# AarambhDevHub/query-engine

Hardware: AMD Instinct MI355X
Metric: rows/sec filter->hash-join->group-by, 1B rows, 1/2/4/8 GPUs; % HBM roofline (higher is better)
Workload: dtype int64/f64

## Files before the change

### query-engine_amd/csrc/k_aggregate.hip

```cpp
#include <algorithm>
#include <cstdlib>
#include <cstring>
#include <string>
#include <memory>
#include <type_traits>

#include "agg.h"
#include "expr_device.h"
#include "fast_tile.h"
#include "ops.h"

namespace qeh {

constexpr int kAggR = 4;
constexpr int kAggTile = kBlock * kAggR;
constexpr size_t kLdsStateBudget = 48 * 1024;
constexpr int kFastTile = kBlock * kFastR;

enum GidMode { GM_ZERO = 0, GM_JOIN = 1, GM_GROUP = 2, GM_LDSHASH = 3 };
enum PredMode { PM_NONE = 0, PM_TERMS = 1, PM_PROG = 2 };

constexpr int64_t kEmptyKey = INT64_MIN;
struct GTable {
    int64_t *keys;
// ... 267 lines not shown
    if (tid < kBpP) pc[tid] = 0, fillp[tid] = kBpChunk, curc[tid] = 0;
    __syncthreads();
    const int64_t n_tiles = (n + kBpTile - 1) / kBpTile;
    const int64_t woff = (int64_t)wave * (64 * kFastR) + 2 * lane;
    FastTile<NTERMS, NACOL, NT> nx;
    if ((int64_t)blockIdx.x < n_tiles && ((int64_t)blockIdx.x + 1) * kBpTile <= n) nx.issue(in, (int64_t)blockIdx.x * kBpTile + woff);
    for (int64_t tile = blockIdx.x; tile < n_tiles; tile += gridDim.x) {
        const int64_t base = tile * kBpTile + woff;
        FastTile<NTERMS, NACOL, NT> ft;
        if ((tile + 1) * kBpTile <= n) {
            ft = nx;
            ft.eval(in, terms);
            const int64_t t2 = tile + gridDim.x;
            if (t2 < n_tiles && (t2 + 1) * kBpTile <= n) nx.issue(in, t2 * kBpTile + woff);
        } else {
            ft.issue_tail(in, base, n);
            ft.eval(in, terms);
            ft.sel &= FastTile<NTERMS, NACOL, NT>::tail_mask(base, n);
        }
        uint32_t part[kFastR], rk[kFastR];
#pragma unroll
        for (int r = 0; r < kFastR; ++r) {
            part[r] = (uint32_t)(hash64((uint64_t)ft.k(r)) >> (64 - kBpPBits));
            rk[r] = ((ft.sel >> r) & 1u) ? atomicAdd(&pc[part[r]], 1u) : 0u;
        }
        bp_barrier();
        if (tid < kBpP) {
            const uint32_t c = pc[tid];
            const uint32_t incl = wave_incl_scan(c);
            tstart[tid] = incl - c;
            if (tid == kBpP - 1) tot_s = incl;
            const uint32_t room = kBpChunk - fillp[tid];
            const uint32_t spill = c > room ? c - room : 0u;
            const uint32_t nnew = (spill + kBpChunk - 1) / kBpChunk;
            uint32_t b = 0;
            if (nnew) {
                b = atomicAdd(nchunk, nnew);
                for (uint32_t i = 0; i < nnew; ++i) tag[b + i] = (uint16_t)tid, ccnt[b + i] = (uint16_t)kBpChunk;
            }
            cbase[tid] = b;
        }
        bp_barrier();
#pragma unroll
        for (int r = 0; r < kFastR; ++r) {
            if (!((ft.sel >> r) & 1u)) continue;
            const uint32_t p = part[r], f = fillp[p], room = kBpChunk - f;
            uint32_t dst;
            if (rk[r] < room) {
                dst = curc[p] * kBpChunk + f + rk[r];
            } else {
                const uint32_t q = rk[r] - room;
                dst = (cbase[p] + q / kBpChunk) * kBpChunk + q % kBpChunk;
            }
            const uint32_t st = tstart[p] + rk[r];
            skey[st] = (uint64_t)ft.k(r);
            if (NACOL > 0) sval[st] = (uint64_t)ft.a(acs, r);
            sdst[st] = dst;
        }
        bp_barrier();
        const uint32_t tot = tot_s;
        for (uint32_t i = tid; i < tot; i += kBpBlock) {
            const uint32_t d = sdst[i];
            okey[d] = skey[i];
            if (NACOL > 0) oval[d] = sval[i];
        }
        if (tid < kBpP) {
            const uint32_t c = pc[tid], f = fillp[tid], room = kBpChunk - f;
            if (c <= room) {
                fillp[tid] = f + c;
            } else {
                const uint32_t q = c - room;
                curc[tid] = cbase[tid] + (q - 1) / kBpChunk;
                fillp[tid] = (q - 1) % kBpChunk + 1;
            }
            pc[tid] = 0;
        }
        bp_barrier();
    }
    if (tid < kBpP && fillp[tid] < kBpChunk) ccnt[curc[tid]] = (uint16_t)fillp[tid];
}

template <int NACOL>
__global__ __launch_bounds__(kBpBlock) void k_bp_probe(AggSpecs specs, FastIn in, HashTable t, int64_t G,
                                                       const uint32_t *__restrict__ sbase, const uint32_t *__restrict__ list,
                                                       const uint64_t *__restrict__ ikey, const uint64_t *__restrict__ ival,
                                                       uint64_t *__restrict__ gstates_all) {
    uint64_t *__restrict__ gstates = shard_states(gstates_all, specs, G);
    extern __shared__ __attribute__((aligned(16))) uint64_t lds[];
    {
        const int64_t words = (int64_t)specs.n_slots * G;
        for (int64_t i = threadIdx.x; i < words; i += blockDim.x) lds[i] = 0;
        __syncthreads();
        for (int a = 0; a < specs.n; ++a) {
            const AggSpec sp = specs.a[a];
            if (sp.kind == AK_MIN || sp.kind == AK_MAX)
                for (int64_t g = threadIdx.x; g < G; g += blockDim.x) lds[(int64_t)sp.val_slot * G + g] = (uint64_t)agg_init_value(sp.kind);
        }
        __syncthreads();
    }
    const int lane = threadIdx.x & 63, wave = threadIdx.x >> 6;
    const int x = blockIdx.x & 7;
    const uint32_t wi = blockIdx.x >> 3, nwg = gridDim.x >> 3;
    constexpr int U = 2;
    for (int p = x; p < kBpP; p += 8) {
        const uint32_t lo = sbase[p], hi = sbase[p + 1];
        const uint32_t stride = nwg * kBpWaves * U;
        uint32_t ent[U];
#pragma unroll
        for (int u = 0; u < U; ++u) {
            const uint32_t e = lo + (wi * kBpWaves + wave) * U + u;
            ent[u] = e < hi ? list[e] : 0xFFFFFFFFu;
        }
        for (uint32_t e0 = lo + (wi * kBpWaves + wave) * U; e0 < hi; e0 += stride) {
            int64_t key[U][4], val[U][4];
            uint32_t cn[U];
#pragma unroll
            for (int u = 0; u < U; ++u) {
                cn[u] = ent[u] == 0xFFFFFFFFu ? 0u : (ent[u] >> 24) + 1u;
                const uint64_t at = (uint64_t)(ent[u] & 0xFFFFFFu) * kBpChunk + lane * 4;
                if (cn[u]) {
                    const v2i64 k0 = __builtin_nontemporal_load((const v2i64 *)(ikey + at));
                    const v2i64 k1 = __builtin_nontemporal_load((const v2i64 *)(ikey + at + 2));
                    key[u][0] = k0[0], key[u][1] = k0[1], key[u][2] = k1[0], key[u][3] = k1[1];
                    if (NACOL > 0) {
                        const v2i64 v0 = __builtin_nontemporal_load((const v2i64 *)(ival + at));
                        const v2i64 v1 = __builtin_nontemporal_load((const v2i64 *)(ival + at + 2));
                        val[u][0] = v0[0], val[u][1] = v0[1], val[u][2] = v1[0], val[u][3] = v1[1];
                    }
                }
            }
#pragma unroll
            for (int u = 0; u < U; ++u) {
                const uint32_t e = e0 + stride + u;
                ent[u] = e < hi ? list[e] : 0xFFFFFFFFu;
            }
            uint32_t gid[U][4];
            uint32_t hit = 0;
#pragma unroll
            for (int u = 0; u < U; ++u)
#pragma unroll
                for (int q = 0; q < 4; ++q) {
                    gid[u][q] = 0;
                    if ((uint32_t)(lane * 4 + q) < cn[u] && probe_unique(t, key[u][q], gid[u][q])) hit |= 1u << (u * 4 + q);
                }
#pragma unroll
            for (int u = 0; u < U; ++u)
#pragma unroll
                for (int q = 0; q < 4; ++q)
                    if ((hit >> (u * 4 + q)) & 1u) atomicAdd((unsigned long long *)&lds[gid[u][q]], 1ull);
            for (int a = 0; a < specs.n; ++a) {
                const AggSpec sp = specs.a[a];
                if (sp.kind == AK_COUNT || in.agg_colslot[a] < 0) continue;
                uint64_t *st = lds + (int64_t)sp.val_slot * G;
#pragma unroll
                for (int u = 0; u < U; ++u)
#pragma unroll
                    for (int q = 0; q < 4; ++q)
                        if ((hit >> (u * 4 + q)) & 1u) {
                            const int64_t v = NACOL > 0 ? val[u][q] : 0;
                            if (sp.kind == AK_SUM_F) atomicAdd((double *)&st[gid[u][q]], as_f64(v));
                            else if (sp.kind == AK_SUM_I) atomicAdd((unsigned long long *)&st[gid[u][q]], (unsigned long long)v);
                            else agg_apply<true>(sp.kind, &st[gid[u][q]], agg_input(sp.kind, sp.in_type, v));
                        }
            }
        }
    }
    __syncthreads();
    for (int64_t g = threadIdx.x; g < G; g += blockDim.x) {
        uint64_t rows = lds[g];
        if (!rows) continue;
        atomicAdd((unsigned long long *)&gstates[g], (unsigned long long)rows);
        for (int a = 0; a < specs.n; ++a) {
            const AggSpec sp = specs.a[a];
            if (sp.kind != AK_COUNT)
                agg_merge_global(sp.kind, &gstates[(int64_t)sp.val_slot * G + g], lds[(int64_t)sp.val_slot * G + g]);
        }
    }
}

constexpr int kSliceBits = 16;
constexpr int kSliceKeys = 1 << kSliceBits;
constexpr int kSliceMaxF = 160;
constexpr int kSliceBlock = 1024;
constexpr int kSliceTile = kSliceBlock * kFastR;
constexpr int kSliceChunk = 32;
constexpr int kMaxSliceGrid = 512;
constexpr int kSliceStateWords = 3584;
constexpr int kGidSliceBits = 12;
constexpr int kGidStateWords = 16384;

__device__ __forceinline__ void lds_barrier() { asm volatile("s_waitcnt lgkmcnt(0)\n\ts_barrier" ::: "memory"); }

struct SliceRegions {
    uint16_t *key;
    int64_t *val;
    int64_t *val2;
    uint32_t *count;
    uint32_t *overflow;
    uint64_t cap;
    int32_t F;
    const uint64_t *rbase;
    int32_t pw;
    int32_t prank;
    int32_t pgrid;
    const uint16_t *okey;
    const int64_t *oval;
    uint64_t ocap;
};
__host__ __device__ __forceinline__ int part_slices(int F, int pw) { return (F + pw - 1) / pw; }
__host__ __device__ __forceinline__ uint64_t part_region(int b, int w, int F, int pw, int grid) {
    return ((uint64_t)(b % pw) * part_slices(F, pw) + (uint64_t)(b / pw)) * grid + w;
}


struct SlicePlan {
    int64_t kmin;
    uint64_t range;
    uint64_t cap;
    int32_t F;
    int32_t ok;
    int64_t src[6];
};
struct SlicePlanIn {
    uint64_t min_bytes;
    uint64_t alloc_items;
    int32_t grid;
    int32_t n_slots;
    int32_t sparse_ok;
    int32_t chunk;
    int32_t world;
};
__host__ __device__ inline SlicePlan plan_slices(const SlicePlanIn &pi, int64_t kmn, int64_t kmx, int64_t kcnt, int64_t gmn,
                                                 int64_t gmx, int64_t gcnt) {
    SlicePlan p{};
    p.src[0] = kmn, p.src[1] = kmx, p.src[2] = kcnt, p.src[3] = gmn, p.src[4] = gmx, p.src[5] = gcnt;
    if (kcnt <= 0) return p;
    const uint64_t gr = gcnt ? (uint64_t)gmx - (uint64_t)gmn + 1ull : 0;
    const int64_t g_bound = (gr == 0 || gr > (1ull << 20)) ? -1 : (int64_t)gr + 1;
    if (g_bound <= 0 || g_bound >= 0xFFFF || (int64_t)pi.n_slots * g_bound > kSliceStateWords) return p;
    const uint64_t range = (uint64_t)kmx - (uint64_t)kmn + 1ull;
    if (!direct_table_ok_with(range, (uint64_t)kcnt, (uint64_t)g_bound, pi.sparse_ok != 0)) return p;
    if (range * 2 < pi.min_bytes) return p;
    const uint64_t F = (range + kSliceKeys - 1) >> kSliceBits;
    if (F == 0 || F > (uint64_t)kSliceMaxF) return p;
    p.kmin = kmn;
    p.range = range;
    p.F = (int32_t)F;
    const uint64_t ch = pi.chunk > 0 ? (uint64_t)pi.chunk : (uint64_t)kSliceChunk;
    const uint64_t Fr = pi.world > 1 ? (F + pi.world - 1) / pi.world * pi.world : F;
    p.cap = pi.alloc_items / ((uint64_t)pi.grid * Fr) / ch * ch;
    p.ok = p.cap >= ch;
    return p;
}
__global__ void k_slice_plan(const MinMax *__restrict__ mm, SlicePlanIn pi, SlicePlan *out) {
    if (threadIdx.x == 0 && blockIdx.x == 0)
        *out = plan_slices(pi, mm[0].mn, mm[0].mx, (int64_t)mm[0].cnt, mm[1].mn, mm[1].mx, (int64_t)mm[1].cnt);
}
__global__ void k_slice_plan_stats(const int64_t *__restrict__ M, int world, int row_len, SlicePlanIn pi, SlicePlan *out) {
    if (threadIdx.x != 0 || blockIdx.x != 0) return;
    int64_t tot = 0, kmn = INT64_MAX, kmx = INT64_MIN, gmn = INT64_MAX, gmx = INT64_MIN, bitmap = 0;
    for (int r = 0; r < world; ++r) {
        const int64_t *m = M + (int64_t)r * row_len;
        bitmap |= m[5];
        if (m[0] <= 0) continue;
        tot += m[0];
        kmn = m[1] < kmn ? m[1] : kmn, kmx = m[2] > kmx ? m[2] : kmx;
        gmn = m[3] < gmn ? m[3] : gmn, gmx = m[4] > gmx ? m[4] : gmx;
    }
    SlicePlan p = plan_slices(pi, kmn, kmx, tot, gmn, gmx, tot);
    if (bitmap || kmn > kmx || gmn > gmx) p.ok = 0;
    *out = p;
}

struct FusedPlan {
    SlicePlan sp;
    int64_t gmin;
    int64_t ngroups;
    uint64_t dcap;
};
struct FusedPro {
    const int64_t *dk;
    ColRef dg;
    int64_t nd;
    uint32_t *ditems;
    uint32_t *dcount;
    uint32_t *status;
    void *gkeys;
    uint32_t *rep;
    int64_t G;
    int32_t as32;
    const FusedPlan *plan;
};
struct DimSlices {
    const uint32_t *items;
    const uint32_t *count;
    uint32_t *dup;
    const FusedPlan *plan;
    int32_t nreg;
    int32_t _pad;
    uint64_t rstride;
    const uint32_t *offs;
};

struct __attribute__((aligned(16))) SliceChunk {
    uint64_t g;
    int32_t soff;
    uint32_t pk;
};

#ifndef QEH_EARLY_PAIRS
#define QEH_EARLY_PAIRS 2
#endif
#ifndef QEH_SLICE_FLUSH_LATE
#define QEH_SLICE_FLUSH_LATE 1
#endif
#ifndef QEH_EARLY_CHUNK
#define QEH_EARLY_CHUNK 64
#endif
template <int NACOL, bool EARLY = false, int NTH = kSliceBlock>
struct SliceShape {
    static constexpr int P = NACOL > 1 ? 2 : (EARLY ? QEH_EARLY_PAIRS : kFastPairs);
    static constexpr int CH = NACOL > 1 ? 16 : (EARLY ? QEH_EARLY_CHUNK : kSliceChunk);
    static constexpr int TILE = NTH * 2 * P;
};

template <int NTH>
__device__ __attribute__((noinline)) void fused_prologue(const FusedPro &fp, int F, int64_t kmin, uint32_t *dcnt) {
    const int tid = threadIdx.x;
    const FusedPlan fpl = *fp.plan;
    for (int i = tid; i < F; i += NTH) dcnt[i] = 0;
    for (int64_t i = (int64_t)blockIdx.x * NTH + tid; i < fp.G; i += (int64_t)gridDim.x * NTH) {
        if (fp.as32) ((int32_t *)fp.gkeys)[i] = (int32_t)(fpl.gmin + i);
        else ((int64_t *)fp.gkeys)[i] = fpl.gmin + i;
        fp.rep[i] = (uint32_t)i;
    }
    __syncthreads();
    const int64_t chunk = (fp.nd + gridDim.x - 1) / gridDim.x;
    const int64_t lo = (int64_t)blockIdx.x * chunk, hi = lo + chunk < fp.nd ? lo + chunk : fp.nd;
    uint32_t *dreg = fp.ditems + (uint64_t)blockIdx.x * F * fpl.dcap;
    bool dovf = false;
    constexpr int DR = 8;
    for (int64_t i0 = lo + tid; i0 < hi; i0 += DR * NTH) {
        int64_t kk[DR], gg[DR];
#pragma unroll
        for (int q = 0; q < DR; ++q) {
            const int64_t i = i0 + (int64_t)q * NTH;
            kk[q] = i < hi ? fp.dk[i] : kmin;
            gg[q] = i < hi ? load_i64(fp.dg, i) : 0;
        }
#pragma unroll
        for (int q = 0; q < DR; ++q) {
            if (i0 + (int64_t)q * NTH >= hi) continue;
            const uint64_t o = (uint64_t)kk[q] - (uint64_t)kmin;
            const uint32_t b = (uint32_t)(o >> kSliceBits);
            const uint32_t r = atomicAdd(&dcnt[b], 1u);
            if (r < fpl.dcap)
                dreg[(uint64_t)b * fpl.dcap + r] =
                    ((uint32_t)(o & (kSliceKeys - 1)) << 16) | ((uint32_t)((uint64_t)gg[q] - (uint64_t)fpl.gmin) + 1u);
            else
                dovf = true;
        }
    }
    __syncthreads();
    if (fp.dcount)
        for (int i = tid; i < F; i += NTH) {
            fp.dcount[(uint64_t)blockIdx.x * F + i] = dcnt[i] < fpl.dcap ? dcnt[i] : (uint32_t)fpl.dcap;
            dovf |= dcnt[i] > fpl.dcap;
        }
    if (dovf) fp.status[1] = 1u;
}

#ifndef QEH_PA_STAMPS
#define QEH_PA_STAMPS 0
#endif
#if QEH_PA_STAMPS
constexpr int kPaStampWords = 16;
__device__ uint64_t qeh_pa_stamps[kMaxSliceGrid * 16 * kPaStampWords];
#define PA_STAMP(i)                                          \
    do {                                                     \
        const uint64_t t_ = __builtin_amdgcn_s_memtime();    \
        pa_acc[i] += t_ - pa_prev;                           \
        pa_prev = t_;                                        \
    } while (0)
#else
#define PA_STAMP(i) \
    do {            \
    } while (0)
#endif

template <int NTERMS, int NACOL, bool NT, int MODE = 0, bool EARLY = false, int NTH = kSliceBlock>
__global__ __launch_bounds__(NTH) void k_slice_partition(FastIn in, PredTerms terms, int64_t kmin, uint64_t range,
                                                                 int64_t n_tiles, SliceRegions rg, HashTable t,
                                                                 const SlicePlan *__restrict__ dplan = nullptr,
                                                                 int64_t tail_rows = 0, FusedPro fp = FusedPro{}) {
    using Shape = SliceShape<NACOL, EARLY, NTH>;
    constexpr int P = Shape::P, R = 2 * P, TILE = Shape::TILE, CH = Shape::CH;
    constexpr int MAXF = kSliceMaxF;
    if (dplan) {
        const SlicePlan pl = *dplan;
        if (!pl.ok) return;
        kmin = pl.kmin, range = pl.range;
        rg.F = pl.F, rg.cap = pl.cap;
    }
    constexpr int SB = MODE ? kGidSliceBits : kSliceBits;
    constexpr int VC = NACOL;
    constexpr int VS = VC > 0 ? VC : 1;
    __shared__ uint32_t cntb[2][MAXF], cnb[2][MAXF], posb[2][MAXF], lofsb[2][MAXF], mpre[MAXF], hd[MAXF];
    __shared__ uint64_t abase[MAXF];
    __shared__ uint32_t s_chunks;
    __shared__ SliceChunk cdesc[TILE / CH + MAXF];
    __shared__ uint16_t st_key[TILE];
    __shared__ int64_t st_v[VS][VC ? TILE : 1];
    __shared__ uint16_t c_key[MAXF * CH];
    __shared__ int64_t c_v[VS][VC ? MAXF * CH : 1];
    __shared__ uint8_t st_b[EARLY ? TILE : 1];
    int64_t *const vout[2] = {rg.val, rg.val2};
    const int F = rg.F;
    const uint64_t cap = rg.cap;
    const int tid = threadIdx.x, lane = tid & 63, wave = tid >> 6;
    const uint64_t region0 = (uint64_t)blockIdx.x * F;
    for (int i = tid; i < MAXF; i += NTH) {
        cntb[0][i] = 0, cntb[1][i] = 0, posb[0][i] = 0, hd[i] = 0, abase[i] = 0;
        if (i < F) {
            const uint64_t st = rg.rbase ? rg.rbase[(uint64_t)i * gridDim.x + blockIdx.x]
                                : rg.pw ? part_region(i, blockIdx.x, F, rg.pw, gridDim.x) * cap
                                        : (region0 + i) * cap;
            hd[i] = (uint32_t)(st % CH);
            abase[i] = st - hd[i];
        }
        cnb[0][i] = hd[i];
    }
    __syncthreads();
    bool ovf = false;
    auto flush = [&](uint32_t M) {
        const uint32_t xl = (tid & (CH / 2 - 1)) * 2;
        for (uint32_t c = tid / (CH / 2); c < M; c += NTH / (CH / 2)) {
            const SliceChunk d = cdesc[c];
            const uint32_t coff = (d.pk & 255u) * CH, clim = (d.pk >> 8) & 127u, lo = (d.pk >> 15) & 127u,
                           hi = (d.pk >> 22) & 127u;
            uint16_t kv[2];
            int64_t vv[VS][2] = {};
#pragma unroll
            for (int q = 0; q < 2; ++q) {
                const uint32_t x = xl + q;
                if (x < clim) {
                    kv[q] = c_key[coff + x];
#pragma unroll
                    for (int u = 0; u < VC; ++u) vv[u][q] = c_v[u][coff + x];
                } else {
                    kv[q] = st_key[d.soff + (int32_t)x];
#pragma unroll
                    for (int u = 0; u < VC; ++u) vv[u][q] = st_v[u][d.soff + (int32_t)x];
                }
            }
            const uint64_t o = d.g + xl;
            if (lo == 0 && hi == (uint32_t)CH) {
                const uint32_t kw = (uint32_t)kv[0] | ((uint32_t)kv[1] << 16);
                if constexpr (EARLY) __builtin_nontemporal_store(kw, (uint32_t *)(rg.key + o));
                else *(uint32_t *)(rg.key + o) = kw;
#pragma unroll
                for (int u = 0; u < VC; ++u) {
                    v2i64 w;
                    w[0] = vv[u][0], w[1] = vv[u][1];
                    __builtin_nontemporal_store(w, (v2i64 *)(vout[u] + o));
                }
            } else {
#pragma unroll
                for (int q = 0; q < 2; ++q) {
                    if (xl + q < lo || xl + q >= hi) continue;
                    rg.key[o + q] = kv[q];
#pragma unroll
                    for (int u = 0; u < VC; ++u) __builtin_nontemporal_store(vv[u][q], vout[u] + o + q);
                }
            }
        }
    };
    auto carry = [&](const uint32_t *cn_o, const uint32_t *cnt_o, const uint32_t *lofs_o, int p0, int stride) {
        if constexpr (EARLY) {
            const uint32_t total = lofs_o[F - 1] + cnt_o[F - 1];
            for (uint32_t si = (uint32_t)p0; si < total; si += (uint32_t)stride) {
                const int b = st_b[si];
                const uint32_t cb = cn_o[b], nb = cnt_o[b], T = cb + nb, L = T % CH, j = si - lofs_o[b];
                int dst = -1;
                if (T < CH) dst = (int)(cb + j);
                else if (j >= nb - L) dst = (int)(j - (nb - L));
                if (dst >= 0) {
                    c_key[b * CH + dst] = st_key[si];
#pragma unroll
                    for (int u = 0; u < VC; ++u) c_v[u][b * CH + dst] = st_v[u][si];
                }
            }
            return;
        }
        for (int p = p0; p < F * CH; p += stride) {
            const int b = p / CH, kx = p % CH;
            const uint32_t cb = cn_o[b], nb = cnt_o[b], T = cb + nb, L = T % CH;
            int src = -1;
            if (T < CH) {
                if (kx >= (int)cb && kx < (int)T) src = (int)(lofs_o[b] + kx - cb);
            } else if (kx < (int)L) {
                src = (int)(lofs_o[b] + nb - L + kx);
            }
            if (src >= 0) {
                c_key[b * CH + kx] = st_key[src];
#pragma unroll
                for (int u = 0; u < VC; ++u) c_v[u][b * CH + kx] = st_v[u][src];
            }
        }
    };
    FastTile<NTERMS, NACOL, NT, P> ft;
    int64_t tile = blockIdx.x;
    int par = 0;
    uint32_t m_prev = 0;
    bool have_prev = false;
    const int64_t n_all = n_tiles + (EARLY && tail_rows > 0 ? 1 : 0), lim = n_tiles * TILE + tail_rows;
    auto issue_tile = [&](int64_t tl) {
        const int64_t b = tl * TILE + (int64_t)wave * (64 * R) + 2 * lane;
        if (!EARLY || tl < n_tiles) ft.issue(in, b);
        else ft.issue_tail(in, b, lim);
    };
    if constexpr (EARLY) {
        __shared__ uint32_t dcnt[MAXF];
        fused_prologue<NTH>(fp, F, kmin, dcnt);
    }
    if (tile < n_all) issue_tile(tile);
#if QEH_PA_STAMPS
    uint64_t pa_acc[10] = {};
    const uint64_t pa_t0 = __builtin_amdgcn_s_memtime(), pa_r0 = __builtin_amdgcn_s_memrealtime();
    uint64_t pa_prev = pa_t0;
#endif
    for (; tile < n_all; tile += gridDim.x) {
        uint32_t *cnt = cntb[par], *cn = cnb[par], *pos = posb[par], *lofs = lofsb[par];
        const int pq = par ^ 1;
        if (!QEH_SLICE_FLUSH_LATE && have_prev) flush(m_prev);
#if QEH_PA_STAMPS
        PA_STAMP(9);
        asm volatile("s_waitcnt vmcnt(0)" ::: "memory");
        PA_STAMP(0);
#endif
        ft.eval(in, terms);
        uint32_t sel = ft.sel, off[R], rk[R];
        if (EARLY && tile >= n_tiles) sel &= decltype(ft)::tail_mask(tile * TILE + (int64_t)wave * (64 * R) + 2 * lane, lim);
        if constexpr (MODE == 1) {
#pragma unroll
            for (int r = 0; r < R; ++r) {
                off[r] = 0;
                if (((sel >> r) & 1) && !probe_unique(t, ft.k(r), off[r])) sel &= ~(1u << r);
            }
#pragma unroll
            for (int r = 0; r < R; ++r) {
                rk[r] = 0;
                if ((sel >> r) & 1) rk[r] = atomicAdd(&cnt[off[r] >> SB], 1u);
            }
        } else {
#pragma unroll
            for (int r = 0; r < R; ++r) {
                const uint64_t o = (uint64_t)ft.k(r) - (uint64_t)kmin;
                off[r] = (uint32_t)o;
                rk[r] = 0;
                if (((sel >> r) & 1) && o < range) rk[r] = atomicAdd(&cnt[(uint32_t)o >> kSliceBits], 1u);
                else sel &= ~(1u << r);
            }
        }
        int64_t vcur[VS][R];
#pragma unroll
        for (int u = 0; u < VS; ++u)
#pragma unroll
            for (int r = 0; r < R; ++r) vcur[u][r] = VC ? ft.a(u, r) : 0;
        PA_STAMP(1);
        if (EARLY && tile + gridDim.x < n_all) issue_tile(tile + gridDim.x);
        if (QEH_SLICE_FLUSH_LATE && have_prev) flush(m_prev);
        PA_STAMP(2);
        lds_barrier();
        PA_STAMP(3);
        if (wave == 0) {
            uint32_t n3[3], m3[3], ns = 0, ms = 0;
#pragma unroll
            for (int q = 0; q < 3; ++q) {
                const int b = lane * 3 + q;
                n3[q] = b < F ? cnt[b] : 0u;
                m3[q] = b < F ? (cn[b] + n3[q]) / CH : 0u;
                ns += n3[q];
                ms += m3[q];
            }
            uint32_t ni = ns, mi = ms;
#pragma unroll
            for (int d = 1; d < 64; d <<= 1) {
                const uint32_t a = __shfl_up(ni, d, 64), c = __shfl_up(mi, d, 64);
                if (lane >= d) ni += a, mi += c;
            }
            uint32_t no = ni - ns, mo = mi - ms;
#pragma unroll
            for (int q = 0; q < 3; ++q) {
                const int b = lane * 3 + q;
                if (b < MAXF) lofs[b] = no, mpre[b] = mo;
                no += n3[q];
                mo += m3[q];
            }
            if (lane == 63) s_chunks = mi;
        } else if (have_prev) {
            carry(cnb[pq], cntb[pq], lofsb[pq], tid - 64, NTH - 64);
        }
        PA_STAMP(4);
        lds_barrier();
        PA_STAMP(5);
#pragma unroll
        for (int r = 0; r < R; ++r) {
            if (!((sel >> r) & 1)) continue;
            const uint32_t s = lofs[off[r] >> SB] + rk[r];
            st_key[s] = (uint16_t)(off[r] & ((1u << SB) - 1u));
            if constexpr (EARLY) st_b[s] = (uint8_t)(off[r] >> SB);
#pragma unroll
            for (int u = 0; u < VC; ++u) st_v[u][s] = vcur[u][r];
        }
        if (tid < F) {
            const uint32_t cb = cn[tid], T = cb + cnt[tid], m = T / CH, m0 = mpre[tid];
            const uint32_t lo0 = lofs[tid];
            const uint64_t p0 = pos[tid], h = hd[tid], gb = abase[tid] + p0;
            for (uint32_t j = 0; j < m; ++j) {
                const uint64_t ds = p0 + (uint64_t)j * CH;
                const uint32_t lo = h > ds ? (uint32_t)std::min<uint64_t>(h - ds, CH) : 0u;
                const uint32_t hi = cap > ds ? (uint32_t)std::min<uint64_t>(cap - ds, CH) : 0u;
                if (hi < (uint32_t)CH) ovf = true;
                const uint32_t clim = j == 0 ? cb : 0u;
                SliceChunk d;
                d.g = gb + (uint64_t)j * CH;
                d.soff = (int32_t)lo0 + (int32_t)(j * CH) - (int32_t)cb;
                d.pk = (uint32_t)tid | (clim << 8) | (lo << 15) | (hi << 22);
                cdesc[m0 + j] = d;
            }
            posb[pq][tid] = (uint32_t)(p0 + (uint64_t)m * CH);
            cnb[pq][tid] = T % CH;
            cntb[pq][tid] = 0;
        }
        if (!EARLY && tile + gridDim.x < n_all) issue_tile(tile + gridDim.x);
        PA_STAMP(6);
        lds_barrier();
        PA_STAMP(7);
        m_prev = s_chunks;
        have_prev = true;
        par = pq;
#if QEH_PA_STAMPS
        pa_acc[8] += 1;
#endif
    }
#if QEH_PA_STAMPS
    if (EARLY && lane == 0) {
        uint64_t *o = qeh_pa_stamps + ((uint64_t)blockIdx.x * (NTH / 64) + wave) * kPaStampWords;
        for (int i = 0; i < 10; ++i) o[i] = pa_acc[i];
        o[10] = __builtin_amdgcn_s_memtime() - pa_t0;
        o[11] = __builtin_amdgcn_s_memrealtime() - pa_r0;
    }
#endif
    if (have_prev) {
        flush(m_prev);
        lds_barrier();
        const int pq = par ^ 1;
        carry(cnb[pq], cntb[pq], lofsb[pq], tid, NTH);
        lds_barrier();
    }
    const uint32_t *cn = cnb[par], *pos = posb[par];
    for (int p = tid; p < F * CH; p += NTH) {
        const int b = p / CH, kx = p % CH;
        if (kx >= (int)cn[b]) continue;
        const uint64_t dst = (uint64_t)pos[b] + kx;
        if (dst < hd[b]) continue;
        if (dst < cap) {
            const uint64_t o = abase[b] + dst;
            rg.key[o] = c_key[b * CH + kx];
#pragma unroll
            for (int u = 0; u < VC; ++u) vout[u][o] = c_v[u][b * CH + kx];
        } else {
            ovf = true;
        }
    }
    if (ovf) *rg.overflow = 1u;
    for (int b = tid; b < F; b += NTH) {
        const uint64_t n = (uint64_t)pos[b] + cn[b];
        rg.count[rg.pw ? part_region(b, blockIdx.x, F, rg.pw, gridDim.x) : region0 + b] =
            (uint32_t)((n < cap ? n : cap) - hd[b]);
    }
}

__device__ __forceinline__ void slice_states_flush(const uint64_t *lst, int64_t stride, int64_t g0, int64_t ng,
                                                   const AggSpecs &specs, int64_t G, uint64_t *__restrict__ gstates) {
    const uint32_t *lcnt = (const uint32_t *)lst;
    for (int64_t i = threadIdx.x; i < ng; i += blockDim.x) {
        const uint64_t rows = lcnt[i];
        if (!rows) continue;
        const int64_t g = g0 + i;
        atomicAdd((unsigned long long *)&gstates[g], (unsigned long long)rows);
        for (int a = 0; a < specs.n; ++a) {
            const AggSpec sp = specs.a[a];
            if (sp.kind != AK_COUNT)
                agg_merge_global(sp.kind, &gstates[(int64_t)sp.val_slot * G + g], lst[(int64_t)sp.val_slot * stride + i]);
        }
    }
}

__device__ __forceinline__ void slice_states_init(uint64_t *lst, int64_t stride, const AggSpecs &specs) {
    const int64_t words = (int64_t)specs.n_slots * stride;
    for (int64_t i = threadIdx.x; i < words; i += blockDim.x) lst[i] = 0;
    __syncthreads();
    for (int a = 0; a < specs.n; ++a) {
        const AggSpec sp = specs.a[a];
        if (sp.kind == AK_MIN || sp.kind == AK_MAX)
            for (int64_t g = threadIdx.x; g < stride; g += blockDim.x)
                lst[(int64_t)sp.val_slot * stride + g] = (uint64_t)agg_init_value(sp.kind);
    }
}

template <int NACOL, bool IDENT = false, bool PF = false, bool PV = false, bool DIM = false>
__global__ __launch_bounds__(kSliceBlock) void k_slice_probe(SliceRegions rg, int nreg, int splits, HashTable t, FastIn in,
                                                             AggSpecs specs, int64_t G, uint64_t *__restrict__ gstates_all,
                                                             DimSlices dim = DimSlices{}) {
    constexpr int VC = NACOL > 0 ? 1 : 0;
    __shared__ __attribute__((aligned(16))) uint16_t tslice[IDENT ? 8 : kSliceKeys];
    __shared__ uint64_t lst[IDENT ? kGidStateWords : kSliceStateWords];
    __shared__ uint32_t rcnt[DIM ? kMaxSliceGrid : 1];
    __shared__ uint32_t rbase[DIM ? kMaxSliceGrid : 1];
    uint32_t *lcnt = (uint32_t *)lst;
    uint64_t dcap = 0;
    int Fg = 0;
    if constexpr (DIM) {
        const FusedPlan pl = *dim.plan;
        if (!pl.sp.ok) return;
        Fg = pl.sp.F;
        rg.F = rg.pw ? part_slices(pl.sp.F, rg.pw) : pl.sp.F, rg.cap = pl.sp.cap;
        dcap = pl.dcap;
    }
    uint64_t *__restrict__ gstates = shard_states(gstates_all, specs, G);
    const int tid = threadIdx.x, lane = tid & 63, wave = tid >> 6;
    constexpr int W = kSliceBlock / 64;
    const int64_t stride = IDENT ? (1 << kGidSliceBits) : G;
    slice_states_init(lst, stride, specs);
    const int F = rg.F;
    const int64_t T = (int64_t)F * nreg;
    const int64_t units = splits ? (int64_t)F * splits : (int64_t)gridDim.x;
    int cur_b = -1;
    for (int64_t u = blockIdx.x; u < units; u += gridDim.x) {
    int64_t s0, s1;
    if (splits) {
        const int64_t ub = u / splits, sp = u % splits;
        s0 = ub * nreg + sp * nreg / splits;
        s1 = ub * nreg + (sp + 1) * nreg / splits;
    } else {
        s0 = u * T / gridDim.x;
        s1 = (u + 1) * T / gridDim.x;
    }
    for (int64_t sb = s0; sb < s1;) {
        const int b = (int)(sb / nreg);
        const int64_t se = std::min<int64_t>(s1, (int64_t)(b + 1) * nreg);
        __syncthreads();
        if (IDENT && b != cur_b) {
            if (cur_b >= 0) {
                const int64_t g0 = (int64_t)cur_b << kGidSliceBits;
                slice_states_flush(lst, stride, g0, std::min<int64_t>(stride, G - g0), specs, G, gstates);
                __syncthreads();
                slice_states_init(lst, stride, specs);
            }
            cur_b = b;
        }
        if (DIM && b != cur_b) {
            cur_b = b;
            uint32_t *tw = (uint32_t *)tslice;
            for (int i = tid; i < kSliceKeys / 2; i += kSliceBlock) tw[i] = 0u;
            const int dn = dim.nreg ? dim.nreg : nreg;
            const int bg = rg.pw ? b * rg.pw + rg.prank : b;
            for (int r = tid; r < dn; r += kSliceBlock) {
                if (bg >= Fg) {
                    rcnt[r] = 0u, rbase[r] = 0u;
                } else if (dim.nreg) {
                    const uint32_t *o = dim.offs + (uint64_t)r * 2 * (kSliceMaxF + 1);
                    rcnt[r] = o[kSliceMaxF + 1 + bg];
                    rbase[r] = (uint32_t)((uint64_t)r * dim.rstride + o[bg]);
                } else {
                    rcnt[r] = dim.count[(uint64_t)r * F + b];
                    rbase[r] = (uint32_t)(((uint64_t)r * F + b) * dcap);
                }
            }
            __syncthreads();
            uint32_t dup = 0;
            for (int r0 = wave * 8; r0 < dn; r0 += W * 8) {
                v4u32 w[8];
                uint32_t cq[8];
#pragma unroll
                for (int q = 0; q < 8; ++q) {
                    const int r = r0 + q;
                    cq[q] = r < dn ? rcnt[r] : 0u;
                    w[q] = (uint32_t)lane * 4 < cq[q] ? *(const v4u32 *)(dim.items + (uint64_t)rbase[r] + lane * 4)
                                                      : v4u32{0u, 0u, 0u, 0u};
                }
#pragma unroll
                for (int q = 0; q < 8; ++q)
#pragma unroll
                    for (int e = 0; e < 4; ++e) {
                        if ((uint32_t)lane * 4 + e >= cq[q]) break;
                        const uint32_t it = w[q][e];
                        const uint32_t off = it >> 16, sh = (off & 1u) * 16u;
                        dup |= (atomicOr(&tw[off >> 1], (it & 0xFFFFu) << sh) >> sh) & 0xFFFFu;
                    }
#pragma unroll
                for (int q = 0; q < 8; ++q) {
                    const int r = r0 + q;
                    const uint32_t c = r < dn ? rcnt[r] : 0u;
                    for (uint32_t i = 256 + (uint32_t)lane * 4; i < c; i += 256) {
                        const v4u32 x = *(const v4u32 *)(dim.items + (uint64_t)rbase[r] + i);
#pragma unroll
                        for (int e = 0; e < 4; ++e) {
                            if (i + e >= c) break;
                            const uint32_t off = x[e] >> 16, sh = (off & 1u) * 16u;
                            dup |= (atomicOr(&tw[off >> 1], (x[e] & 0xFFFFu) << sh) >> sh) & 0xFFFFu;
                        }
                    }
                }
            }
            if (dup) *dim.dup = 1u;
        } else if (!DIM && !IDENT && b != cur_b) {
            cur_b = b;
            const uint64_t k0 = (uint64_t)b << kSliceBits;
            const uint64_t nk = t.range - k0 < (uint64_t)kSliceKeys ? t.range - k0 : (uint64_t)kSliceKeys;
            for (int i = tid * 8; i < kSliceKeys; i += kSliceBlock * 8) {
                v4u32 w = {0u, 0u, 0u, 0u};
                if ((uint64_t)i + 8 <= nk) {
                    w = *(const v4u32 *)(t.payload16 + k0 + i);
                } else {
                    for (int q = 0; q < 8; ++q)
                        if ((uint64_t)(i + q) < nk) w[q >> 1] |= (uint32_t)t.payload16[k0 + i + q] << ((q & 1) * 16);
                }
                *(v4u32 *)&tslice[i] = w;
            }
        }
        __syncthreads();
        for (int64_t s = sb + wave; s < se; s += W) {
            uint64_t reg, rb;
            const uint16_t *kbase = rg.key;
            const int64_t *vbase = rg.val;
            if (rg.pw) {
                const int64_t r = s - (int64_t)b * nreg, q = r / rg.pgrid;
                reg = ((uint64_t)q * F + b) * rg.pgrid + (uint64_t)(r - q * rg.pgrid);
                if (rg.okey && q == rg.prank) {
                    kbase = rg.okey, vbase = rg.oval;
                    rb = reg * rg.ocap;
                } else {
                    rb = rg.rbase[reg];
                }
            } else {
                reg = (uint64_t)(s - (int64_t)b * nreg) * F + b;
                rb = reg * rg.cap;
            }
            const uint32_t n_r = rg.count[reg];
            const uint16_t *kp = kbase + rb;
            const int64_t *vp = VC ? vbase + rb : nullptr;
            const int64_t *vp2 = NACOL > 1 ? rg.val2 + rb : nullptr;
            uint32_t en[8];
            int64_t vn[8], vn2[NACOL > 1 ? 8 : 1];
            auto item = [&](uint32_t i0, int j) -> uint32_t {
                return PV ? i0 + (uint32_t)(j >> 1) * 128 + 2 * lane + (uint32_t)(j & 1) : i0 + (uint32_t)j * 64 + lane;
            };
            auto ld = [&](uint32_t i0) {
                if constexpr (PV) {
#pragma unroll
                    for (int j = 0; j < 4; ++j) {
                        const uint32_t i = item(i0, 2 * j);
                        const uint32_t ii = i < n_r ? i : 0u;
                        const uint32_t kk = __builtin_nontemporal_load((const uint32_t *)(kp + ii));
                        en[2 * j] = kk & 0xFFFFu, en[2 * j + 1] = kk >> 16;
                        if (VC) {
                            const v2i64 w = __builtin_nontemporal_load((const v2i64 *)(vp + ii));
                            vn[2 * j] = w[0], vn[2 * j + 1] = w[1];
                        } else {
                            vn[2 * j] = vn[2 * j + 1] = 0;
                        }
                    }
                } else {
#pragma unroll
                    for (int j = 0; j < 8; ++j) {
                        const uint32_t i = item(i0, j);
                        const uint32_t ii = i < n_r ? i : 0u;
                        en[j] = __builtin_nontemporal_load(kp + ii);
                        vn[j] = VC ? __builtin_nontemporal_load(vp + ii) : 0;
                        if constexpr (NACOL > 1) vn2[j] = __builtin_nontemporal_load(vp2 + ii);
                    }
                }
            };
            if (PF && n_r) ld(0);
            for (uint32_t i0 = 0; i0 < n_r; i0 += 64 * 8) {
                uint32_t e[8];
                int64_t v[8], v2[NACOL > 1 ? 8 : 1];
                if (!PF) ld(i0);
#pragma unroll
                for (int j = 0; j < 8; ++j) e[j] = en[j], v[j] = vn[j];
                if constexpr (NACOL > 1) {
#pragma unroll
                    for (int j = 0; j < 8; ++j) v2[j] = vn2[j];
                }
                if (PF && i0 + 64 * 8 < n_r) ld(i0 + 64 * 8);
#pragma unroll
                for (int j = 0; j < 8; ++j)
                    e[j] = (item(i0, j) < n_r) ? (IDENT ? e[j] + 1u : (uint32_t)tslice[e[j]]) : 0u;

#pragma unroll
                for (int j = 0; j < 8; ++j)
                    if (e[j]) atomicAdd(lcnt + (e[j] - 1u), 1u);
                for (int a = 0; a < specs.n; ++a) {
                    const AggSpec sp = specs.a[a];
                    uint64_t *st = lst + (int64_t)sp.val_slot * stride - 1;
                    const bool second = NACOL > 1 && in.agg_colslot[a] == 1;
                    auto val = [&](int j) -> int64_t {
                        if constexpr (NACOL > 1) return second ? v2[j] : v[j];
                        return v[j];
                    };
                    switch (sp.kind) {
                        case AK_SUM_F:
#pragma unroll
                            for (int j = 0; j < 8; ++j)
                                if (e[j]) atomicAdd((double *)&st[e[j]], as_f64(val(j)));
                            break;
                        case AK_SUM_I:
#pragma unroll
                            for (int j = 0; j < 8; ++j)
                                if (e[j]) atomicAdd((unsigned long long *)&st[e[j]], (unsigned long long)val(j));
                            break;
                        case AK_MIN:
                        case AK_MAX:
#pragma unroll
                            for (int j = 0; j < 8; ++j)
                                if (e[j]) agg_apply<true>(sp.kind, &st[e[j]], agg_input(sp.kind, sp.in_type, val(j)));
                            break;
                        default: break;
                    }
                }
            }
        }
        sb = se;
    }
    }
    __syncthreads();
    if (IDENT) {
        if (cur_b >= 0) {
            const int64_t g0 = (int64_t)cur_b << kGidSliceBits;
            slice_states_flush(lst, stride, g0, std::min<int64_t>(stride, G - g0), specs, G, gstates);
        }
    } else {
        slice_states_flush(lst, stride, 0, G, specs, G, gstates);
    }
}

constexpr int kKeyAggWords = 20480;
template <int NACOL, bool C16 = false>
__global__ __launch_bounds__(kSliceBlock) void k_slice_keyagg(SliceRegions rg, int nreg, HashTable t, AggSpecs specs,
                                                              int64_t G, uint64_t *__restrict__ gstates_all, int nw, int ws,
                                                              int full, int tparts) {
    __shared__ uint64_t lbuf[kKeyAggWords];
    uint32_t *lcnt = (uint32_t *)lbuf;
    uint64_t *lval = lbuf + (C16 ? ((uint32_t)ws + 3u) / 4u : ((uint32_t)ws + 1u) / 2u);
    bool ovf = false;
    uint64_t *__restrict__ gstates = shard_states(gstates_all, specs, G);
    const int tid = threadIdx.x, lane = tid & 63, wave = tid >> 6;
    constexpr int W = kSliceBlock / 64;
    const int gpx = (int)gridDim.x / 8 / nw;
    const int xcd = (int)blockIdx.x & 7, x = (int)blockIdx.x >> 3;
    const int grp = xcd * gpx + x / nw, ngrp = 8 * gpx;
    const uint32_t lo = (uint32_t)(x % nw) * (uint32_t)ws;
    auto init = [&]() {
        for (int i = tid; i < (C16 ? (ws + 1) / 2 : ws); i += kSliceBlock) lcnt[i] = 0u;
        for (int a = 0; a < specs.n; ++a) {
            const AggSpec sp = specs.a[a];
            if (sp.kind == AK_COUNT) continue;
            const uint64_t v0 = (uint64_t)agg_init_value(sp.kind);
            for (int i = tid; i < ws; i += kSliceBlock) lval[(int64_t)(sp.val_slot - 1) * ws + i] = v0;
        }
    };
    init();
    const int units = full + (rg.F - full) * tparts;
    for (int u = grp; u < units; u += ngrp) {
        const int tu = u - full;
        const int b = tu < 0 ? u : full + tu / tparts, parts = tu < 0 ? 1 : tparts, part = tu < 0 ? 0 : tu % tparts;
        const int r0 = part * nreg / parts, r1 = (part + 1) * nreg / parts;
        __syncthreads();
        for (int r = r0 + wave; r < r1; r += W) {
            const uint64_t reg = (uint64_t)r * rg.F + b;
            const uint32_t n_r = rg.count[reg];
            const uint16_t *kp = rg.key + reg * rg.cap;
            const int64_t *vp = NACOL ? rg.val + reg * rg.cap : nullptr;
            for (uint32_t i0 = 0; i0 < n_r; i0 += 64 * 8) {
                uint32_t e[8];
                int64_t v[8];
#pragma unroll
                for (int j = 0; j < 8; ++j) {
                    const uint32_t i = i0 + (uint32_t)j * 64 + lane;
                    const uint32_t ii = i < n_r ? i : 0u;
                    const uint32_t k = (uint32_t)kp[ii] - lo;
                    v[j] = NACOL ? vp[ii] : 0;
                    e[j] = (i < n_r && k < (uint32_t)ws) ? k + 1u : 0u;
                }
#pragma unroll
                for (int j = 0; j < 8; ++j) {
                    if (!e[j]) continue;
                    if constexpr (C16) {
                        const uint32_t sh = ((e[j] - 1u) & 1u) * 16u;
                        const uint32_t old = atomicAdd(lcnt + ((e[j] - 1u) >> 1), 1u << sh);
                        ovf |= ((old >> sh) & 0xFFFFu) == 0xFFFFu;
                    } else {
                        atomicAdd(lcnt + (e[j] - 1u), 1u);
                    }
                }
                for (int a = 0; a < specs.n; ++a) {
                    const AggSpec sp = specs.a[a];
                    if (sp.kind == AK_COUNT) continue;
                    uint64_t *st = lval + (int64_t)(sp.val_slot - 1) * ws - 1;
                    switch (sp.kind) {
                        case AK_SUM_F:
#pragma unroll
                            for (int j = 0; j < 8; ++j)
                                if (e[j]) atomicAdd((double *)&st[e[j]], as_f64(v[j]));
                            break;
                        case AK_SUM_I:
#pragma unroll
                            for (int j = 0; j < 8; ++j)
                                if (e[j]) atomicAdd((unsigned long long *)&st[e[j]], (unsigned long long)v[j]);
                            break;
                        default:
#pragma unroll
                            for (int j = 0; j < 8; ++j)
                                if (e[j]) agg_apply<true>(sp.kind, &st[e[j]], agg_input(sp.kind, sp.in_type, v[j]));
                            break;
                    }
                }
            }
        }
        __syncthreads();
        const uint64_t k0 = ((uint64_t)b << kSliceBits) + lo;
        for (int i = tid; i < ws; i += kSliceBlock) {
            const uint64_t rows = C16 ? (lcnt[i >> 1] >> ((i & 1) * 16)) & 0xFFFFu : lcnt[i];
            if (!rows || k0 + i >= t.range) continue;
            const uint32_t ent = t.payload16 ? (uint32_t)t.payload16[k0 + i] : t.payload[k0 + i];
            if (!ent) continue;
            const int64_t g = (int64_t)ent - 1;
            atomicAdd((unsigned long long *)&gstates[g], (unsigned long long)rows);
            for (int a = 0; a < specs.n; ++a) {
                const AggSpec sp = specs.a[a];
                if (sp.kind != AK_COUNT)
                    agg_merge_global(sp.kind, &gstates[(int64_t)sp.val_slot * G + g], lval[(int64_t)(sp.val_slot - 1) * ws + i]);
            }
        }
        __syncthreads();
        init();
    }
    if (C16 && ovf) *rg.overflow = 1u;
}

__global__ __launch_bounds__(1024) void k_fused_plan(const MinMax *__restrict__ part, int nb, SlicePlanIn pi, int64_t g_cap,
                                                     int64_t nd, uint64_t dim_items, FusedPlan *out, uint32_t *__restrict__ st,
                                                     uint64_t *__restrict__ states, int64_t G, AggSpecs specs) {
    const int64_t words = (int64_t)specs.shards * specs.n_slots * G;
    for (int64_t i = (int64_t)blockIdx.x * blockDim.x + threadIdx.x; i < words; i += (int64_t)gridDim.x * blockDim.x) {
        const int64_t slot = (i / G) % specs.n_slots;
        uint64_t v = 0;
        for (int a = 0; a < specs.n; ++a)
            if (specs.a[a].val_slot == slot) v = (uint64_t)agg_init_value(specs.a[a].kind);
        states[i] = v;
    }
    if (blockIdx.x != 0) return;
    __shared__ MinMax sm[2][16];
    const int lane = threadIdx.x & 63, wave = threadIdx.x >> 6;
    for (int c = 0; c < 2; ++c) {
        int64_t mn = INT64_MAX, mx = INT64_MIN;
        uint64_t cnt = 0;
        uint32_t bad = 0;
        for (int i = threadIdx.x; i < nb; i += blockDim.x) {
            const MinMax q = part[(int64_t)c * nb + i];
            mn = q.mn < mn ? q.mn : mn;
            mx = q.mx > mx ? q.mx : mx;
            cnt += q.cnt;
            bad |= q.bad;
        }
#pragma unroll
        for (int d = 32; d >= 1; d >>= 1) {
            const int64_t a = __shfl_xor(mn, d, 64), b2 = __shfl_xor(mx, d, 64);
            const uint64_t cc = __shfl_xor(cnt, d, 64);
            const uint32_t bb = __shfl_xor(bad, d, 64);
            mn = a < mn ? a : mn;
            mx = b2 > mx ? b2 : mx;
            cnt += cc;
            bad |= bb;
        }
        if (lane == 0) sm[c][wave] = MinMax{mn, mx, cnt, bad};
    }
    __syncthreads();
    if (threadIdx.x != 0) return;
    MinMax mm[2];
    for (int c = 0; c < 2; ++c) {
        mm[c] = sm[c][0];
        for (int w = 1; w < (int)(blockDim.x >> 6); ++w) {
            const MinMax q = sm[c][w];
            mm[c].mn = q.mn < mm[c].mn ? q.mn : mm[c].mn;
            mm[c].mx = q.mx > mm[c].mx ? q.mx : mm[c].mx;
            mm[c].cnt += q.cnt;
            mm[c].bad |= q.bad;
        }
    }
    FusedPlan p{};
    p.sp = plan_slices(pi, mm[0].mn, mm[0].mx, (int64_t)mm[0].cnt, mm[1].mn, mm[1].mx, (int64_t)mm[1].cnt);
    const bool full = (int64_t)mm[0].cnt == nd && (int64_t)mm[1].cnt == nd && !mm[0].bad && !mm[1].bad;
    p.gmin = mm[1].mn;
    p.ngroups = full ? (int64_t)((uint64_t)mm[1].mx - (uint64_t)mm[1].mn + 1ull) : 0;
    p.dcap = p.sp.F > 0 ? dim_items / ((uint64_t)pi.grid * p.sp.F) / 4 * 4 : 0;
    p.sp.ok = p.sp.ok && full && p.ngroups >= 1 && p.ngroups <= g_cap && p.ngroups < 0xFFFF && p.dcap >= 4;
    *out = p;
    for (int i = 0; i < 8; ++i) st[i] = 0u;
    st[5] = p.sp.ok ? 1u : 0u;
}

__device__ __forceinline__ void emit_matches(const uint32_t *e, const int64_t *v, const bool *live, int64_t amin,
                                             uint64_t *base, int64_t *__restrict__ out_v, int64_t *__restrict__ out_a) {
    uint64_t b = *base;
#pragma unroll
    for (int j = 0; j < 8; ++j) {
        const bool m = live[j] && e[j] != 0u;
        const uint64_t mask = __ballot(m);
        if (m) {
            const uint64_t pos = b + mbcnt(mask);
            out_v[pos] = v[j];
            out_a[pos] = (int64_t)(e[j] - 1u) + amin;
        }
        b += popc64(mask);
    }
    *base = b;
}

__device__ __forceinline__ void load_slice(uint16_t *tslice, const HashTable &t, int b, int tid) {
    const uint64_t k0 = (uint64_t)b << kSliceBits;
    const uint64_t nk = t.range - k0 < (uint64_t)kSliceKeys ? t.range - k0 : (uint64_t)kSliceKeys;
    for (int i = tid * 8; i < kSliceKeys; i += kSliceBlock * 8) {
        v4u32 w = {0u, 0u, 0u, 0u};
        if ((uint64_t)i + 8 <= nk) {
            w = *(const v4u32 *)(t.payload16 + k0 + i);
        } else {
            for (int q = 0; q < 8; ++q)
                if ((uint64_t)(i + q) < nk) w[q >> 1] |= (uint32_t)t.payload16[k0 + i + q] << ((q & 1) * 16);
        }
        *(v4u32 *)&tslice[i] = w;
    }
}

template <bool EMIT>
__global__ __launch_bounds__(kSliceBlock) void k_slice_join_b(SliceRegions rg, int nreg, HashTable t, int64_t amin,
                                                              uint32_t *__restrict__ counts, const uint64_t *__restrict__ bases,
                                                              int64_t *__restrict__ out_v, int64_t *__restrict__ out_a) {
    __shared__ __attribute__((aligned(16))) uint16_t tslice[kSliceKeys];
    const int tid = threadIdx.x, lane = tid & 63, wave = tid >> 6;
    constexpr int W = kSliceBlock / 64;
    const int F = rg.F;
    const int64_t T = (int64_t)F * nreg;
    const int64_t s0 = (int64_t)blockIdx.x * T / gridDim.x, s1 = (int64_t)(blockIdx.x + 1) * T / gridDim.x;
    for (int64_t sb = s0; sb < s1;) {
        const int b = (int)(sb / nreg);
        const int64_t se = std::min<int64_t>(s1, (int64_t)(b + 1) * nreg);
        __syncthreads();
        load_slice(tslice, t, b, tid);
        __syncthreads();
        for (int64_t s = sb + wave; s < se; s += W) {
            const uint64_t reg = (uint64_t)(s - (int64_t)b * nreg) * F + b;
            const uint32_t n_r = rg.count[reg];
            const uint64_t rb = rg.rbase ? rg.rbase[s] : reg * rg.cap;
            const uint16_t *kp = rg.key + rb;
            const int64_t *vp = rg.val + rb;
            uint64_t base = EMIT ? bases[s] : 0;
            uint32_t matches = 0;
            for (uint32_t i0 = 0; i0 < n_r; i0 += 64 * 8) {
                uint32_t e[8];
                int64_t v[8];
                bool live[8];
#pragma unroll
                for (int j = 0; j < 8; ++j) {
                    const uint32_t i = i0 + j * 64 + lane;
                    live[j] = i < n_r;
                    const uint32_t ii = live[j] ? i : 0u;
                    e[j] = __builtin_nontemporal_load(kp + ii);
                    v[j] = EMIT ? __builtin_nontemporal_load(vp + ii) : 0;
                }
#pragma unroll
                for (int j = 0; j < 8; ++j) e[j] = live[j] ? (uint32_t)tslice[e[j]] : 0u;
                if (EMIT) {
                    emit_matches(e, v, live, amin, &base, out_v, out_a);
                } else {
#pragma unroll
                    for (int j = 0; j < 8; ++j) matches += (uint32_t)popc64(__ballot(live[j] && e[j] != 0u));
                }
            }
            if (!EMIT && lane == 0) counts[s] = matches;
        }
        sb = se;
    }
}

__global__ __launch_bounds__(kSliceBlock) void k_slice_count(const int64_t *__restrict__ key, int64_t kmin, uint64_t range,
                                                             int64_t n_tiles, int F, uint32_t *__restrict__ counts) {
    constexpr int W = kSliceBlock / 64;
    __shared__ uint32_t cnt[W][kSliceMaxF];
    const int tid = threadIdx.x, wave = tid >> 6;
    for (int i = tid; i < W * kSliceMaxF; i += kSliceBlock) (&cnt[0][0])[i] = 0;
    __syncthreads();
    for (int64_t tile = blockIdx.x; tile < n_tiles; tile += gridDim.x) {
        const int64_t base = tile * kSliceTile;
        v2i64 kk[kSliceTile / (2 * kSliceBlock)];
#pragma unroll
        for (int q = 0; q < kSliceTile / (2 * kSliceBlock); ++q)
            kk[q] = __builtin_nontemporal_load((const v2i64 *)(key + base + 2 * ((int64_t)q * kSliceBlock + tid)));
#pragma unroll
        for (int q = 0; q < kSliceTile / (2 * kSliceBlock); ++q)
#pragma unroll
            for (int x = 0; x < 2; ++x) {
                const uint64_t o = (uint64_t)kk[q][x] - (uint64_t)kmin;
                if (o < range) atomicAdd(&cnt[wave][(uint32_t)(o >> kSliceBits)], 1u);
            }
    }
    __syncthreads();
    for (int b = tid; b < F; b += kSliceBlock) {
        uint32_t c = 0;
#pragma unroll
        for (int w = 0; w < W; ++w) c += cnt[w][b];
        counts[(uint64_t)b * gridDim.x + blockIdx.x] = c;
    }
}

__global__ __launch_bounds__(kSliceBlock) void k_slice_join_inplace(SliceRegions rg, int nreg, HashTable t, int64_t amin,
                                                                    int64_t *__restrict__ out_a,
                                                                    unsigned long long *__restrict__ misses) {
    __shared__ __attribute__((aligned(16))) uint16_t tslice[kSliceKeys];
    const int tid = threadIdx.x, lane = tid & 63, wave = tid >> 6;
    constexpr int W = kSliceBlock / 64;
    const int F = rg.F;
    const int64_t T = (int64_t)F * nreg;
    const int64_t s0 = (int64_t)blockIdx.x * T / gridDim.x, s1 = (int64_t)(blockIdx.x + 1) * T / gridDim.x;
    uint32_t miss = 0;
    for (int64_t sb = s0; sb < s1;) {
        const int b = (int)(sb / nreg);
        const int64_t se = std::min<int64_t>(s1, (int64_t)(b + 1) * nreg);
        __syncthreads();
        load_slice(tslice, t, b, tid);
        __syncthreads();
        for (int64_t s = sb + wave; s < se; s += W) {
            const uint64_t reg = (uint64_t)(s - (int64_t)b * nreg) * F + b;
            const uint32_t n_r = rg.count[reg];
            const uint64_t rb = rg.rbase[s];
            const uint16_t *kp = rg.key + rb;
            int64_t *ap = out_a + rb;
            uint32_t e[16];
#pragma unroll
            for (int j = 0; j < 16; ++j) {
                const uint32_t i = j * 64 + lane;
                e[j] = __builtin_nontemporal_load(kp + (i < n_r ? i : 0u));
            }
            for (uint32_t i0 = 0; i0 < n_r; i0 += 64 * 16) {
                uint32_t en[16];
                const uint32_t i1 = i0 + 64 * 16;
#pragma unroll
                for (int j = 0; j < 16; ++j) {
                    const uint32_t i = i1 + j * 64 + lane;
                    en[j] = __builtin_nontemporal_load(kp + (i < n_r ? i : 0u));
                }
#pragma unroll
                for (int j = 0; j < 16; ++j) {
                    const uint32_t i = i0 + j * 64 + lane;
                    if (i < n_r) {
                        const uint32_t x = tslice[e[j]];
                        miss += x == 0u;
                        __builtin_nontemporal_store((int64_t)(x - 1u) + amin, ap + i);
                    }
                }
#pragma unroll
                for (int j = 0; j < 16; ++j) e[j] = en[j];
            }
        }
        sb = se;
    }
    const uint64_t m = wave_sum_u64(miss);
    if (lane == 0 && m) atomicAdd(misses, (unsigned long long)m);
}

__global__ __launch_bounds__(kBlock) void k_slice_join_tail(const int64_t *__restrict__ key, const int64_t *__restrict__ val,
                                                            int64_t n, HashTable t, int64_t amin, int64_t *__restrict__ out_v,
                                                            int64_t *__restrict__ out_a, unsigned long long *counter) {
    const int lane = threadIdx.x & 63;
    for (int64_t i0 = (int64_t)blockIdx.x * blockDim.x * 8 + (threadIdx.x & ~63) * 8; i0 < n;
         i0 += (int64_t)gridDim.x * blockDim.x * 8) {
        uint32_t e[8];
        int64_t v[8];
        bool live[8];
        uint32_t total = 0;
#pragma unroll
        for (int j = 0; j < 8; ++j) {
            const int64_t i = i0 + j * 64 + lane;
            live[j] = i < n;
            e[j] = 0u;
            v[j] = 0;
            if (live[j]) {
                const uint64_t o = (uint64_t)key[i] - (uint64_t)t.kmin;
                if (o < t.range) e[j] = t.payload16[o];
                v[j] = val[i];
            }
            total += (uint32_t)popc64(__ballot(live[j] && e[j] != 0u));
        }
        unsigned long long b = 0;
        if (lane == 0 && total) b = atomicAdd(counter, (unsigned long long)total);
        uint64_t base = __shfl(b, 0, 64);
        emit_matches(e, v, live, amin, &base, out_v, out_a);
    }
}

__device__ __forceinline__ int64_t gt_slot(const GTable &g, int64_t key) {
    uint64_t h = hash64((uint64_t)key) & g.mask;
    for (uint64_t p = 0; p <= g.mask; ++p) {
        const long long cur = __hip_atomic_load((long long *)&g.keys[h], __ATOMIC_RELAXED, __HIP_MEMORY_SCOPE_AGENT);
        if (cur == key) return (int64_t)h;
        if (cur == kEmptyKey) {
            const unsigned long long old =
                atomicCAS((unsigned long long *)&g.keys[h], (unsigned long long)kEmptyKey, (unsigned long long)key);
            if ((long long)old == kEmptyKey || (long long)old == key) return (int64_t)h;
        }
        if (p > 4096) break;
        h = (h + 1) & g.mask;
    }
    *g.overflow = 1u;
    return -1;
}

template <int PM>
__global__ __launch_bounds__(kBlock) void k_groupby_lds(ColSet cols, int64_t n, PredTerms terms, DevProgram prog,
                                                        int key_col, GidSource src, AggSpecs specs, int64_t G,
                                                        uint64_t *__restrict__ gstates_all, uint32_t *__restrict__ errp) {
    uint64_t *__restrict__ gstates = shard_states(gstates_all, specs, G);
    extern __shared__ __attribute__((aligned(16))) uint64_t lds[];
    const int lcap = src.lcap;
    int64_t *lkeys = (int64_t *)lds;
    uint64_t *lst = lds + lcap;
    for (int i = threadIdx.x; i < lcap; i += blockDim.x) lkeys[i] = kEmptyKey;
    for (int64_t i = threadIdx.x; i < (int64_t)specs.n_slots * lcap; i += blockDim.x) lst[i] = 0;
    __syncthreads();
    for (int a = 0; a < specs.n; ++a) {
        const AggSpec sp = specs.a[a];
        if (sp.kind == AK_MIN || sp.kind == AK_MAX)
            for (int i = threadIdx.x; i < lcap; i += blockDim.x) lst[(int64_t)sp.val_slot * lcap + i] = (uint64_t)agg_init_value(sp.kind);
    }
    __syncthreads();
    const int64_t gcap = (int64_t)src.gt.mask + 1;
    const int lane = threadIdx.x & 63, wave = threadIdx.x >> 6;
    uint32_t err = 0;
    const int64_t ntiles = (n + kAggTile - 1) / kAggTile;
    for (int64_t tile = blockIdx.x; tile < ntiles; tile += gridDim.x) {
        const int64_t row0 = tile * kAggTile + (int64_t)wave * 64 * kAggR + lane;
        uint32_t sel;
        if (PM == PM_TERMS) {
            sel = eval_terms<kAggR>(terms, cols, row0, 64, n);
        } else if (PM == PM_PROG) {
            ExprRegs<kAggR> X;
            run_program<kAggR>(prog, cols, row0, 64, n, X, err);
            sel = program_true_mask<kAggR>(X);
        } else {
            sel = 0;
#pragma unroll
            for (int r = 0; r < kAggR; ++r)
                if (row0 + r * 64 < n) sel |= 1u << r;
        }
        int64_t kv[kAggR];
        uint32_t kvalid;
        load_rows<kAggR>(cols.c[key_col], row0, 64, n, kv, kvalid);
#pragma unroll
        for (int r = 0; r < kAggR; ++r) {
            if (!((sel >> r) & 1)) continue;
            const int64_t row = row0 + r * 64;
            const int64_t key = kv[r];
            uint64_t *st;
            int64_t stride, idx;
            bool local = false;
            int lslot = -1;
            if (((kvalid >> r) & 1) && key != kEmptyKey) {
                int h = (int)(hash64((uint64_t)key) & (uint64_t)(lcap - 1));
                for (int p = 0; p < 32; ++p) {
                    const int64_t cur = lkeys[h];
                    if (cur == key) { lslot = h; break; }
                    if (cur == kEmptyKey) {
                        const unsigned long long old = atomicCAS((unsigned long long *)&lkeys[h],
                                                                 (unsigned long long)kEmptyKey, (unsigned long long)key);
                        if ((long long)old == kEmptyKey || (long long)old == key) { lslot = h; break; }
                    }
                    h = (h + 1) & (lcap - 1);
                }
            }
            if (lslot >= 0) {
                local = true;
                st = lst;
                stride = lcap;
                idx = lslot;
            } else {
                st = gstates;
                stride = G;
                if (!((kvalid >> r) & 1)) idx = gcap;
                else if (key == kEmptyKey) idx = gcap + 1;
                else idx = gt_slot(src.gt, key);
                if (idx < 0) continue;
            }
            atomicAdd((unsigned long long *)&st[idx], 1ull);
            for (int a = 0; a < specs.n; ++a) {
                const AggSpec sp = specs.a[a];
                const ColRef &c = cols.c[sp.col];
                if (!col_valid(c, row)) continue;
                if (sp.cnt_slot) atomicAdd((unsigned long long *)&st[(int64_t)sp.cnt_slot * stride + idx], 1ull);
                if (sp.kind != AK_COUNT) {
                    const int64_t x = agg_input(sp.kind, sp.in_type, load_i64(c, row));
                    if (local) agg_apply<true>(sp.kind, &st[(int64_t)sp.val_slot * stride + idx], x);
                    else agg_apply<false>(sp.kind, &st[(int64_t)sp.val_slot * stride + idx], x);
                }
            }
        }
    }
    if (err) atomicOr(errp, err);
    __syncthreads();
    for (int i = threadIdx.x; i < lcap; i += blockDim.x) {
        const int64_t key = lkeys[i];
        if (key == kEmptyKey) continue;
        const int64_t g = gt_slot(src.gt, key);
        if (g < 0) continue;
        atomicAdd((unsigned long long *)&gstates[g], (unsigned long long)lst[i]);
        for (int a = 0; a < specs.n; ++a) {
            const AggSpec sp = specs.a[a];
            if (sp.cnt_slot) {
                const uint64_t c = lst[(int64_t)sp.cnt_slot * lcap + i];
                if (c) atomicAdd((unsigned long long *)&gstates[(int64_t)sp.cnt_slot * G + g], (unsigned long long)c);
            }
            if (sp.kind != AK_COUNT)
                agg_merge_global(sp.kind, &gstates[(int64_t)sp.val_slot * G + g], lst[(int64_t)sp.val_slot * lcap + i]);
        }
    }
}

__device__ __forceinline__ uint32_t lds_hash(int64_t key) {
    const uint32_t x = (uint32_t)key ^ (uint32_t)((uint64_t)key >> 32);
    return (x * 0x9E3779B1u) ^ ((x * 0x9E3779B1u) >> 15);
}

template <int NTERMS, int NACOL, bool NT, int BLOCK = kBlock>
__global__ __launch_bounds__(BLOCK) void k_group_agg_fast(FastIn in, PredTerms terms, AggSpecs specs, GTable gt,
                                                           int lcap, int64_t G, int64_t n_tiles,
                                                           uint64_t *__restrict__ gstates_all) {
    uint64_t *__restrict__ gstates = shard_states(gstates_all, specs, G);
    extern __shared__ __attribute__((aligned(16))) uint64_t lds[];
    int64_t *lkeys = (int64_t *)lds;
    uint64_t *lst = lds + lcap;
    for (int i = threadIdx.x; i < lcap; i += blockDim.x) lkeys[i] = kEmptyKey;
    for (int64_t i = threadIdx.x; i < (int64_t)specs.n_slots * lcap; i += blockDim.x) lst[i] = 0;
    __syncthreads();
    for (int a = 0; a < specs.n; ++a) {
        const AggSpec sp = specs.a[a];
        if (sp.kind == AK_MIN || sp.kind == AK_MAX)
            for (int i = threadIdx.x; i < lcap; i += blockDim.x) lst[(int64_t)sp.val_slot * lcap + i] = (uint64_t)agg_init_value(sp.kind);
    }
    __syncthreads();
    const int64_t gcap = (int64_t)gt.mask + 1;
    const int lane = threadIdx.x & 63, wave = threadIdx.x >> 6;
    for (int64_t tile = blockIdx.x; tile < n_tiles; tile += gridDim.x) {
        const int64_t base = tile * (BLOCK * kFastR) + (int64_t)wave * (64 * kFastR) + 2 * lane;
        FastTile<NTERMS, NACOL, NT> ft;
        ft.load(in, terms, base);
        const uint32_t sel = ft.sel;
        int slot[kFastR], h0[kFastR];
        int64_t first[kFastR];
#pragma unroll
        for (int r = 0; r < kFastR; ++r) {
            h0[r] = (int)(lds_hash(ft.k(r)) & (uint32_t)(lcap - 1));
            first[r] = lkeys[h0[r]];
        }
#pragma unroll
        for (int r = 0; r < kFastR; ++r) {
            const int64_t key = ft.k(r);
            slot[r] = (first[r] == key && key != kEmptyKey) ? h0[r] : -1;
            if (slot[r] >= 0 || !((sel >> r) & 1) || key == kEmptyKey) continue;
            int h = h0[r];
            for (int p = 0; p < 32; ++p) {
                const int64_t cur = lkeys[h];
                if (cur == key) { slot[r] = h; break; }
                if (cur == kEmptyKey) {
                    const unsigned long long old = atomicCAS((unsigned long long *)&lkeys[h], (unsigned long long)kEmptyKey,
                                                             (unsigned long long)key);
                    if ((long long)old == kEmptyKey || (long long)old == key) { slot[r] = h; break; }
                }
                h = (h + 1) & (lcap - 1);
            }
        }
        uint32_t in_lds = 0;
#pragma unroll
        for (int r = 0; r < kFastR; ++r) in_lds |= (((sel >> r) & 1) && slot[r] >= 0) ? 1u << r : 0u;
        lds_apply_rows(lst, lcap, specs, in, ft, in_lds, slot);
#pragma unroll
        for (int r = 0; r < kFastR; ++r) {
            if (!((sel >> r) & 1)) continue;
            if (slot[r] < 0) {
                const int64_t key = ft.k(r);
                const int64_t g = key == kEmptyKey ? gcap + 1 : gt_slot(gt, key);
                if (g < 0) continue;
                atomicAdd((unsigned long long *)&gstates[g], 1ull);
                for (int a = 0; a < specs.n; ++a) {
                    const AggSpec sp = specs.a[a];
                    if (sp.kind == AK_COUNT) continue;
                    agg_apply<false>(sp.kind, &gstates[(int64_t)sp.val_slot * G + g],
                                     agg_input(sp.kind, sp.in_type, ft.a(in.agg_colslot[a], r)));
                }
            }
        }
    }
    __syncthreads();
    for (int i = threadIdx.x; i < lcap; i += blockDim.x) {
        const int64_t key = lkeys[i];
        if (key == kEmptyKey) continue;
        const int64_t g = gt_slot(gt, key);
        if (g < 0) continue;
        atomicAdd((unsigned long long *)&gstates[g], (unsigned long long)lst[i]);
        for (int a = 0; a < specs.n; ++a) {
            const AggSpec sp = specs.a[a];
            if (sp.kind != AK_COUNT)
                agg_merge_global(sp.kind, &gstates[(int64_t)sp.val_slot * G + g], lst[(int64_t)sp.val_slot * lcap + i]);
        }
    }
}

__global__ void k_fill_i64(int64_t *p, int64_t n, int64_t v) {
    for (int64_t i = (int64_t)blockIdx.x * blockDim.x + threadIdx.x; i < n; i += (int64_t)gridDim.x * blockDim.x) p[i] = v;
}

__global__ void k_iota(uint32_t *p, int64_t n) {
    for (int64_t i = (int64_t)blockIdx.x * blockDim.x + threadIdx.x; i < n; i += (int64_t)gridDim.x * blockDim.x)
        p[i] = (uint32_t)i;
}

__global__ void k_states_init(uint64_t *states, int64_t G, AggSpecs specs) {
    const int64_t words = (int64_t)specs.shards * specs.n_slots * G;
    for (int64_t i = (int64_t)blockIdx.x * blockDim.x + threadIdx.x; i < words; i += (int64_t)gridDim.x * blockDim.x) {
        int64_t slot = (i / G) % specs.n_slots;
        uint64_t v = 0;
        for (int a = 0; a < specs.n; ++a)
            if (specs.a[a].val_slot == slot) v = (uint64_t)agg_init_value(specs.a[a].kind);
        states[i] = v;
    }
}

__global__ void k_states_reduce(uint64_t *states, int64_t G, AggSpecs specs) {
    const int64_t words = (int64_t)specs.n_slots * G;
    const int64_t stride = words;
    for (int64_t i = (int64_t)blockIdx.x * blockDim.x + threadIdx.x; i < words; i += (int64_t)gridDim.x * blockDim.x) {
        const int64_t slot = i / G;
        int kind = -1;
        for (int a = 0; a < specs.n; ++a)
            if (specs.a[a].val_slot == slot) kind = specs.a[a].kind;
        uint64_t acc = states[i];
        for (int sh = 1; sh < specs.shards; ++sh) {
            const uint64_t v = states[i + sh * stride];
            switch (kind) {
                case AK_SUM_F: acc = __builtin_bit_cast(uint64_t, as_f64(acc) + as_f64(v)); break;
                case AK_MIN: acc = (int64_t)v < (int64_t)acc ? v : acc; break;
                case AK_MAX: acc = (int64_t)v > (int64_t)acc ? v : acc; break;
                default: acc += v; break;
            }
        }
        states[i] = acc;
    }
}

__global__ __launch_bounds__(256) void k_states_fold(uint64_t *__restrict__ states, int64_t Gs, AggSpecs specs) {
    const int64_t words = (int64_t)specs.n_slots * Gs;
    const int64_t i = (int64_t)blockIdx.x * blockDim.x + threadIdx.x;
    if (i >= words) return;
    const int64_t slot = i / Gs;
    int kind = -1;
    for (int a = 0; a < specs.n; ++a)
        if (specs.a[a].val_slot == slot) kind = specs.a[a].kind;
    uint64_t acc = states[i];
    constexpr int B = 16;
    for (int sh0 = 1; sh0 < specs.shards; sh0 += B) {
        uint64_t v[B];
#pragma unroll
        for (int q = 0; q < B; ++q) v[q] = sh0 + q < specs.shards ? states[i + (sh0 + q) * words] : 0ull;
#pragma unroll
        for (int q = 0; q < B; ++q) {
            if (sh0 + q >= specs.shards) break;
            switch (kind) {
                case AK_SUM_F: acc = __builtin_bit_cast(uint64_t, as_f64(acc) + as_f64(v[q])); break;
                case AK_MIN: acc = (int64_t)v[q] < (int64_t)acc ? v[q] : acc; break;
                case AK_MAX: acc = (int64_t)v[q] > (int64_t)acc ? v[q] : acc; break;
                default: acc += v[q]; break;
            }
        }
    }
    states[i] = acc;
}

__global__ __launch_bounds__(256) void k_states_lanes(const uint64_t *__restrict__ states, int64_t Gs, int64_t G,
                                                      AggSpecs specs, double *__restrict__ lanes,
                                                      const uint32_t *__restrict__ status, int fused = 0) {
    const int64_t e = (int64_t)blockIdx.x * blockDim.x + threadIdx.x;
    if (e == 0 && status)
        lanes[(int64_t)(1 + specs.n) * G] =
            (status[0] | status[1] | (fused ? (status[4] | (status[5] ? 0u : 1u)) : 0u)) ? 1.0 : 0.0;
    if (e >= (int64_t)(1 + specs.n) * G) return;
    const int j = (int)(e / G) - 1;
    const int64_t g = e % G;
    const bool fsum = j >= 0 && specs.a[j].kind == AK_SUM_F;
    const int slot = j < 0 ? 0 : (fsum ? specs.a[j].val_slot : specs.a[j].cnt_slot);
    const int64_t words = (int64_t)specs.n_slots * Gs;
    const uint64_t *p = states + (int64_t)slot * Gs + g;
    constexpr int B = 16;
    double fv = 0.0;
    uint64_t uv = 0;
    for (int q0 = 0; q0 < specs.shards; q0 += B) {
        uint64_t v[B];
#pragma unroll
        for (int q = 0; q < B; ++q) v[q] = q0 + q < specs.shards ? p[(int64_t)(q0 + q) * words] : 0ull;
#pragma unroll
        for (int q = 0; q < B; ++q) {
            if (q0 + q >= specs.shards) break;
            if (fsum) fv += as_f64((int64_t)v[q]);
            else uv += v[q];
        }
    }
    lanes[e] = fsum ? fv : (double)uv;
}

constexpr int kCompactSmallG = 16384;
__global__ __launch_bounds__(1024) void k_states_compact_small(uint64_t *__restrict__ states, int64_t Gs, int64_t G,
                                                              AggSpecs specs, uint64_t *__restrict__ pos,
                                                              uint64_t *__restrict__ total) {
    __shared__ uint32_t wsum[16];
    const int t = threadIdx.x, lane = t & 63, wave = t >> 6;
    if (specs.shards > 1) {
        const int64_t words = (int64_t)specs.n_slots * Gs;
        for (int64_t i = t; i < words; i += 1024) {
            const int64_t slot = i / Gs;
            int kind = -1;
            for (int a = 0; a < specs.n; ++a)
                if (specs.a[a].val_slot == slot) kind = specs.a[a].kind;
            uint64_t acc = states[i];
            constexpr int B = 16;
            for (int sh0 = 1; sh0 < specs.shards; sh0 += B) {
                uint64_t v[B];
#pragma unroll
                for (int q = 0; q < B; ++q) v[q] = sh0 + q < specs.shards ? states[i + (sh0 + q) * words] : 0ull;
#pragma unroll
                for (int q = 0; q < B; ++q) {
                    if (sh0 + q >= specs.shards) break;
                    switch (kind) {
                        case AK_SUM_F: acc = __builtin_bit_cast(uint64_t, as_f64(acc) + as_f64(v[q])); break;
                        case AK_MIN: acc = (int64_t)v[q] < (int64_t)acc ? v[q] : acc; break;
                        case AK_MAX: acc = (int64_t)v[q] > (int64_t)acc ? v[q] : acc; break;
                        default: acc += v[q]; break;
                    }
                }
            }
            states[i] = acc;
        }
        __syncthreads();
    }
    const int64_t per = (G + 1023) / 1024, g0 = (int64_t)t * per, g1 = g0 + per < G ? g0 + per : G;
    uint32_t c = 0;
    for (int64_t g = g0; g < g1; ++g) c += states[g] != 0;
    const uint32_t incl = wave_incl_scan(c);
    if (lane == 63) wsum[wave] = incl;
    __syncthreads();
    uint32_t base = incl - c, all = 0;
    for (int w = 0; w < 16; ++w) {
        base += w < wave ? wsum[w] : 0u;
        all += wsum[w];
    }
    for (int64_t g = g0; g < g1; ++g) {
        pos[g] = base;
        base += states[g] != 0;
    }
    if (t == 0) *total = all;
}

__global__ void k_group_nonempty(const uint64_t *states, int64_t G, uint32_t *flags) {
    for (int64_t g = (int64_t)blockIdx.x * blockDim.x + threadIdx.x; g < G; g += (int64_t)gridDim.x * blockDim.x)
        flags[g] = states[g] != 0;
}

struct OutCol {
    void *values;
    uint32_t *validity;
    int32_t dtype;
    int32_t _pad;
};
struct OutCols {
    OutCol c[kMaxGroupKeys + kMaxAggs];
};

__device__ __forceinline__ void write_value(const OutCol &o, int64_t p, int64_t payload, bool valid) {
    if (o.validity && valid) atomicOr(&o.validity[p >> 5], 1u << (p & 31));
    switch (o.dtype) {
        case QEH_DT_BOOL:
            if (payload & 1) atomicOr(&((uint32_t *)o.values)[p >> 5], 1u << (p & 31));
            break;
        case QEH_DT_INT32: ((int32_t *)o.values)[p] = (int32_t)payload; break;
        case QEH_DT_FLOAT32: ((float *)o.values)[p] = (float)as_f64(payload); break;
        default: ((int64_t *)o.values)[p] = payload; break;
    }
}

__global__ void k_finalize(const uint64_t *__restrict__ states, int64_t G, const uint64_t *__restrict__ pos,
                           KeyCols keys, const uint32_t *__restrict__ rep_row, AggSpecs specs, OutCols outs) {
    for (int64_t g = (int64_t)blockIdx.x * blockDim.x + threadIdx.x; g < G; g += (int64_t)gridDim.x * blockDim.x) {
        const uint64_t rows = states[g];
        int64_t p;
        if (pos) {
            if (!rows) continue;
            p = (int64_t)pos[g];
        } else {
            p = g;
        }
        for (int k = 0; k < keys.n; ++k) {
            const int64_t r = rep_row[g];
            write_value(outs.c[k], p, load_i64(keys.c[k], r), col_valid(keys.c[k], r));
        }
        for (int a = 0; a < specs.n; ++a) {
            const AggSpec sp = specs.a[a];
            const uint64_t cnt = sp.cnt_slot ? states[(int64_t)sp.cnt_slot * G + g] : rows;
            const int64_t v = sp.kind == AK_COUNT ? 0 : (int64_t)states[(int64_t)sp.val_slot * G + g];
            const OutCol &o = outs.c[keys.n + a];
            const bool i32 = sp.in_type == QEH_DT_INT32;
            const bool flt = sp.in_type == QEH_DT_FLOAT32 || sp.in_type == QEH_DT_FLOAT64;
            switch (sp.func) {
                case QEH_AGG_COUNT: write_value(o, p, (int64_t)cnt, true); break;
                case QEH_AGG_SUM:
                    write_value(o, p, i32 ? (int64_t)(int32_t)v : v, cnt != 0);
                    break;
                case QEH_AGG_AVG: {
                    double s = flt ? as_f64(v) : (double)(i32 ? (int64_t)(int32_t)v : v);
                    write_value(o, p, f64_bits(cnt ? s / (double)cnt : 0.0), cnt != 0);
                    break;
                }
                default: {
                    int64_t out = flt ? f64_bits(f64_from_order_key(v)) : v;
                    write_value(o, p, out, cnt != 0);
                    break;
                }
            }
        }
    }
}

__global__ __launch_bounds__(1024) void k_fused_finish(const uint64_t *__restrict__ states, int64_t G, KeyCols keys,
                                                       const uint32_t *__restrict__ rep, AggSpecs specs, OutCols outs,
                                                       uint64_t *__restrict__ total) {
    __shared__ uint32_t pos[kSliceStateWords];
    __shared__ uint32_t vbits[kMaxGroupKeys + kMaxAggs][kSliceStateWords / 32];
    __shared__ uint32_t wsum[16];
    const int t = threadIdx.x, lane = t & 63, wave = t >> 6;
    const int nout = keys.n + specs.n;
    const int64_t vwords = (G + 31) / 32;
    for (int c = 0; c < nout; ++c)
        for (int64_t w = t; w < vwords; w += blockDim.x) vbits[c][w] = 0u;
    const int64_t per = (G + 1023) / 1024, g0 = (int64_t)t * per, g1 = g0 + per < G ? g0 + per : G;
    uint32_t c = 0;
    for (int64_t g = g0; g < g1; ++g) c += states[g] != 0;
    const uint32_t incl = wave_incl_scan(c);
    if (lane == 63) wsum[wave] = incl;
    __syncthreads();
    uint32_t base = incl - c, all = 0;
    for (int w = 0; w < 16; ++w) {
        base += w < wave ? wsum[w] : 0u;
        all += wsum[w];
    }
    for (int64_t g = g0; g < g1; ++g) {
        pos[g] = base;
        base += states[g] != 0;
    }
    if (t == 0) *total = all;
    __syncthreads();
    auto put = [&](int c, int64_t p, int64_t payload, bool valid) {
        OutCol o = outs.c[c];
        if (o.validity && valid) atomicOr(&vbits[c][p >> 5], 1u << (p & 31));
        o.validity = nullptr;
        write_value(o, p, payload, true);
    };
    for (int64_t g = t; g < G; g += blockDim.x) {
        const uint64_t rows = states[g];
        if (!rows) continue;
        const int64_t p = pos[g];
        for (int k = 0; k < keys.n; ++k) {
            const int64_t r = rep[g];
            put(k, p, load_i64(keys.c[k], r), col_valid(keys.c[k], r));
        }
        for (int a = 0; a < specs.n; ++a) {
            const AggSpec sp = specs.a[a];
            const uint64_t cnt = sp.cnt_slot ? states[(int64_t)sp.cnt_slot * G + g] : rows;
            const int64_t v = sp.kind == AK_COUNT ? 0 : (int64_t)states[(int64_t)sp.val_slot * G + g];
            const int o = keys.n + a;
            const bool i32 = sp.in_type == QEH_DT_INT32;
            const bool flt = sp.in_type == QEH_DT_FLOAT32 || sp.in_type == QEH_DT_FLOAT64;
            switch (sp.func) {
                case QEH_AGG_COUNT: put(o, p, (int64_t)cnt, true); break;
                case QEH_AGG_SUM: put(o, p, i32 ? (int64_t)(int32_t)v : v, cnt != 0); break;
                case QEH_AGG_AVG: {
                    double sm = flt ? as_f64(v) : (double)(i32 ? (int64_t)(int32_t)v : v);
                    put(o, p, f64_bits(cnt ? sm / (double)cnt : 0.0), cnt != 0);
                    break;
                }
                default: put(o, p, flt ? f64_bits(f64_from_order_key(v)) : v, cnt != 0); break;
            }
        }
    }
    __syncthreads();
    for (int c = 0; c < nout; ++c)
        if (outs.c[c].validity)
            for (int64_t w = t; w < vwords; w += blockDim.x) outs.c[c].validity[w] = vbits[c][w];
}

static int agg_output_type(int func, int in_type) {
    switch (func) {
        case QEH_AGG_COUNT: return QEH_DT_INT64;
        case QEH_AGG_SUM: return (in_type == QEH_DT_FLOAT32 || in_type == QEH_DT_FLOAT64) ? QEH_DT_FLOAT64 : QEH_DT_INT64;
        case QEH_AGG_AVG: return QEH_DT_FLOAT64;
        default: return in_type;
    }
}

static int plan_aggs(const qeh_agg *aggs, int n_aggs, const qeh_column *inputs, int n_inputs,
                     const int *colset_index, AggSpecs *out) {
    if (n_aggs > kMaxAggs) return fail(QEH_E_UNSUPPORTED, "too many aggregates for one device operator (max 8)");
    std::memset(out, 0, sizeof(*out));
    out->n = n_aggs;
    out->shards = 1;
    int slot = 1;
    for (int i = 0; i < n_aggs; ++i) {
        const qeh_agg &a = aggs[i];
        if (a.column < 0 || a.column >= n_inputs) return fail(QEH_E_INVALID, "aggregate input index out of range");
        const qeh_column &c = inputs[a.column];
        int t = c.dtype;
        AggSpec &s = out->a[i];
        s.func = a.func;
        s.col = colset_index[a.column];
        s.in_type = t;
        const bool numeric = t == QEH_DT_INT32 || t == QEH_DT_INT64 || t == QEH_DT_FLOAT32 || t == QEH_DT_FLOAT64;
        const bool flt = t == QEH_DT_FLOAT32 || t == QEH_DT_FLOAT64;
        switch (a.func) {
            case QEH_AGG_COUNT: s.kind = AK_COUNT; break;
            case QEH_AGG_SUM:
                if (!numeric) return fail(QEH_E_TYPE, "Unsupported type for SUM");
                s.kind = flt ? AK_SUM_F : AK_SUM_I;
                break;
            case QEH_AGG_AVG:
                if (!numeric) return fail(QEH_E_TYPE, "Unsupported type for AVG");
                s.kind = flt ? AK_SUM_F : AK_SUM_I;
                break;
            case QEH_AGG_MIN:
                if (!numeric) return fail(QEH_E_TYPE, "Unsupported type for MIN");
                s.kind = AK_MIN;
                break;
            case QEH_AGG_MAX:
                if (!numeric) return fail(QEH_E_TYPE, "Unsupported type for MAX");
                s.kind = AK_MAX;
                break;
            default: return fail(QEH_E_INVALID, "unknown aggregate function");
        }
        s.val_slot = s.kind == AK_COUNT ? -1 : slot++;
        const bool has_nulls = c.validity != nullptr && c.null_count != 0;
        s.cnt_slot = has_nulls ? slot++ : 0;
    }
    out->n_slots = slot;
    return QEH_OK;
}

struct PredPlan {
    int mode = PM_NONE;
    PredTerms terms{};
    DevProgram prog{};
};

static int plan_predicate(const qeh_expr *pred, const int32_t *dtypes, int n_cols, PredPlan *pp) {
    pp->mode = PM_NONE;
    if (!pred || pred->n_nodes == 0) return QEH_OK;
    QEH_TRY(compile_expr(pred, dtypes, n_cols, &pp->prog));
    if (pp->prog.result_type != QEH_DT_BOOL)
        return fail(QEH_E_TYPE, "Filter predicate must return boolean");
    pp->mode = lower_to_terms(pred, dtypes, n_cols, &pp->terms) ? PM_TERMS : PM_PROG;
    return QEH_OK;
}

template <int GM>
static void launch_agg_rows(qeh_ctx *ctx, int pm, bool lds, int grid, size_t shmem, const ColSet &cols, int64_t n,
                            const PredPlan &pp, const GidSource &src, const AggSpecs &specs, int64_t G,
                            uint64_t *states, uint32_t *err) {
#define QEH_LAUNCH(PMV, LDSV)                                                                                  \
    hipLaunchKernelGGL((k_agg_rows<GM, PMV, LDSV>), dim3(grid), dim3(kBlock), shmem, ctx->stream, cols, n, pp.terms, \
                       pp.prog, src, specs, G, states, err)
    if (pm == PM_NONE) { if (lds) QEH_LAUNCH(PM_NONE, true); else QEH_LAUNCH(PM_NONE, false); }
    else if (pm == PM_TERMS) { if (lds) QEH_LAUNCH(PM_TERMS, true); else QEH_LAUNCH(PM_TERMS, false); }
    else { if (lds) QEH_LAUNCH(PM_PROG, true); else QEH_LAUNCH(PM_PROG, false); }
#undef QEH_LAUNCH
}

static ColRef advance(ColRef c, int64_t rows) {
    size_t es = dtype_size(c.dtype);
    if (c.dtype != QEH_DT_BOOL && es) c.values = (const char *)c.values + (size_t)rows * es;
    c.vbit0 += rows;
    return c;
}

static bool fast_col_ok(const ColRef &c) {
    return (c.dtype == QEH_DT_INT64 || c.dtype == QEH_DT_FLOAT64) && c.validity == nullptr &&
           ((uintptr_t)c.values & 15) == 0;
}

static int fast_nt_mode() {
    static int m = -1;
    if (m < 0) {
        const char *e = std::getenv("QEH_NT_LOADS");
        m = (e && e[0] == '0') ? 0 : 1;
    }
    return m;
}

static bool fast_cols_eligible(const ColSet &cols, const PredPlan &pp, int key_col, const AggSpecs &specs,
                               FastIn *inp, int *nterms_out, int *nacol_out) {
    if (pp.mode == PM_PROG || (pp.mode == PM_TERMS && pp.terms.n > 2)) return false;
    if (!fast_col_ok(cols.c[key_col])) return false;
    FastIn &in = *inp;
    in = FastIn{};
    in.key = (const int64_t *)cols.c[key_col].values;
    const int nterms = pp.mode == PM_TERMS ? pp.terms.n : 0;
    for (int i = 0; i < nterms; ++i) {
        const ColRef &c = cols.c[pp.terms.t[i].col];
        if (!fast_col_ok(c)) return false;
        in.term[i] = (const int64_t *)c.values;
        in.term_dt[i] = c.dtype;
    }
    int nacol = 0;
    int acol_idx[2] = {-1, -1};
    for (int a = 0; a < specs.n; ++a) {
        const AggSpec &sp = specs.a[a];
        if (sp.cnt_slot != 0) return false;
        in.agg_colslot[a] = -1;
        if (sp.kind == AK_COUNT) continue;
        int slot = -1;
        for (int c = 0; c < nacol; ++c)
            if (acol_idx[c] == sp.col) slot = c;
        if (slot < 0) {
            if (nacol == 2) return false;
            if (!fast_col_ok(cols.c[sp.col])) return false;
            acol_idx[nacol] = sp.col;
            in.acol[nacol] = (const int64_t *)cols.c[sp.col].values;
            slot = nacol++;
        }
        in.agg_colslot[a] = slot;
    }
    *nterms_out = nterms;
    *nacol_out = nacol;
    return true;
}

static bool fast_eligible(const ColSet &cols, const PredPlan &pp, const GidSource &src, const AggSpecs &specs,
                          FastIn *inp, int *nterms_out, int *nacol_out) {
    if (!src.jt.unique) return false;
    if (cols.c[src.key_col].dtype != QEH_DT_INT64) return false;
    return fast_cols_eligible(cols, pp, src.key_col, specs, inp, nterms_out, nacol_out);
}

static void launch_tail(qeh_ctx *ctx, const ColSet &cols, int64_t n, int64_t done, const PredPlan &pp,
                        const GidSource &src, const AggSpecs &specs, int64_t G, uint64_t *states, uint32_t *err,
                        size_t lds_bytes) {
    if (done >= n) return;
    ColSet tail = cols;
    for (int i = 0; i < cols.n; ++i) tail.c[i] = advance(cols.c[i], done);
    const int grid = (int)std::min<int64_t>(16, (n - done + kAggTile - 1) / kAggTile);
    launch_agg_rows<GM_JOIN>(ctx, pp.mode, true, std::max(grid, 1), lds_bytes, tail, n - done, pp, src, specs, G, states,
                             err);
}

static uint64_t table_bytes(const HashTable &t);

static bool try_bucket_parts(qeh_ctx *ctx, const FastIn &in, const PredPlan &pp, int nterms, int nacol,
                             const AggSpecs &specs, const HashTable &t, int64_t G, int64_t n, uint64_t *states,
                             size_t lds_bytes) {
    if (t.kind != TK_BUCKET || nacol > 1 || !std::getenv("QEH_BUCKET_PARTS")) return false;
    if (lds_bytes > 64 * 1024) return false;
    const int cus = ctx->props.multiProcessorCount;
    const int64_t n_tiles = (n + kBpTile - 1) / kBpTile;
    const int grid1 = (int)std::max<int64_t>(1, std::min<int64_t>(2 * (int64_t)cus, n_tiles));
    const uint64_t max_chunks = (uint64_t)(n + kBpChunk - 1) / kBpChunk + (uint64_t)grid1 * kBpP;
    if (max_chunks >= (1ull << 24)) return false;
    DevBuf keys, vals, tags, cnts, lists, ctr;
    if (keys.alloc(ctx, max_chunks * kBpChunk * 8) != QEH_OK || (nacol && vals.alloc(ctx, max_chunks * kBpChunk * 8) != QEH_OK) ||
        tags.alloc(ctx, max_chunks * 2) != QEH_OK || cnts.alloc(ctx, max_chunks * 2) != QEH_OK ||
        lists.alloc(ctx, max_chunks * 4 + (kBpP + 1) * 4 + chunk_lists_work_words(kBpP) * 4) != QEH_OK ||
        ctr.alloc(ctx, 4) != QEH_OK)
        return false;
    if (hipMemsetAsync(tags.p, 0xFF, max_chunks * 2, ctx->stream) != hipSuccess ||
        hipMemsetAsync(ctr.p, 0, 4, ctx->stream) != hipSuccess)
        return false;
    const int acs = nacol ? 0 : -1;
    KernelTimer kt(ctx, "bucket_parts");
    const bool nt = fast_nt_mode() == 1;
#define QEH_BP(NTV, NAV, NTB)                                                                                            \
    hipLaunchKernelGGL((k_bp_part<NTV, NAV, NTB>), dim3(grid1), dim3(kBpBlock), 0, ctx->stream, in, pp.terms, n, acs,   \
                       keys.as<uint64_t>(), vals.as<uint64_t>(), tags.as<uint16_t>(), cnts.as<uint16_t>(), ctr.as<uint32_t>())
#define QEH_BP_NA(NTV, NTB)                  \
    if (nacol == 0) QEH_BP(NTV, 0, NTB);     \
    else QEH_BP(NTV, 1, NTB);
#define QEH_BP_NT(NTB)                           \
    if (nterms == 0) { QEH_BP_NA(0, NTB) }       \
    else if (nterms == 1) { QEH_BP_NA(1, NTB) }  \
    else { QEH_BP_NA(2, NTB) }
    if (nt) { QEH_BP_NT(true) } else { QEH_BP_NT(false) }
#undef QEH_BP_NT
#undef QEH_BP_NA
#undef QEH_BP
    uint32_t *sbase = lists.as<uint32_t>() + max_chunks;
    if (chunk_lists(ctx, tags.as<uint16_t>(), cnts.as<uint16_t>(), max_chunks, kBpP, sbase, lists.as<uint32_t>(),
                    sbase + kBpP + 1) != QEH_OK)
        return false;
    const int grid2 = std::max(8, (2 * cus + 7) / 8 * 8);
    if (nacol)
        hipLaunchKernelGGL(k_bp_probe<1>, dim3(grid2), dim3(kBpBlock), lds_bytes, ctx->stream, specs, in, t, G, sbase,
                           lists.as<uint32_t>(), keys.as<uint64_t>(), vals.as<uint64_t>(), states);
    else
        hipLaunchKernelGGL(k_bp_probe<0>, dim3(grid2), dim3(kBpBlock), lds_bytes, ctx->stream, specs, in, t, G, sbase,
                           lists.as<uint32_t>(), keys.as<uint64_t>(), vals.as<uint64_t>(), states);
    return hipStreamSynchronize(ctx->stream) == hipSuccess;
}

static bool try_fast_join(qeh_ctx *ctx, const ColSet &cols, int64_t n, const PredPlan &pp, const GidSource &src,
                          const AggSpecs &specs, int64_t G, uint64_t *states, uint32_t *err, size_t lds_bytes,
                          int per_cu) {
    if (std::getenv("QEH_NO_FAST")) return false;
    FastIn in;
    int nterms, nacol;
    if (!fast_eligible(cols, pp, src, specs, &in, &nterms, &nacol)) return false;
    if (try_bucket_parts(ctx, in, pp, nterms, nacol, specs, src.jt, G, n, states, lds_bytes)) return true;
    const int64_t n_tiles = n / kFastTile;
    if (n_tiles > 0) {
        const int grid = grid_for(ctx, n_tiles * kFastTile, kFastTile, per_cu);
        const bool nt = fast_nt_mode() == 1;
#define QEH_FAST(NTV, NAV, NTB)                                                                                    \
    hipLaunchKernelGGL((k_join_agg_fast<NTV, NAV, NTB>), dim3(grid), dim3(kBlock), lds_bytes, ctx->stream, in, pp.terms, \
                       specs, src.jt, G, n_tiles, states)
#define QEH_FAST_NA(NTV, NTB)                       \
    if (nacol == 0) QEH_FAST(NTV, 0, NTB);          \
    else if (nacol == 1) QEH_FAST(NTV, 1, NTB);     \
    else QEH_FAST(NTV, 2, NTB);
#define QEH_FAST_NT(NTB)                            \
    if (nterms == 0) { QEH_FAST_NA(0, NTB) }        \
    else if (nterms == 1) { QEH_FAST_NA(1, NTB) }   \
    else { QEH_FAST_NA(2, NTB) }
        if (nt) { QEH_FAST_NT(true) } else { QEH_FAST_NT(false) }
#undef QEH_FAST_NT
#undef QEH_FAST_NA
#undef QEH_FAST
    }
    launch_tail(ctx, cols, n, n_tiles * kFastTile, pp, src, specs, G, states, err, lds_bytes);
    return true;
}

static uint64_t table_bytes(const HashTable &t) {
    if (t.kind == TK_DIRECT) return t.range * (t.payload16 ? 2 : 4);
    if (t.kind == TK_PACKED) return (t.mask + 1) * 8;
    if (t.kind == TK_BUCKET) return t.nbkt * 64;
    return (t.mask + 1) * 16;
}

struct SlicePre {
    bool launched = false;
    int64_t kmin = 0;
    uint64_t range = 0;
    int grid = 0;
    int64_t n_tiles = 0;
    DevBuf kbuf, vbuf, cbuf, planbuf, vbuf2;
    SliceRegions rg{};
    hipEvent_t done = nullptr;
    bool dev_planned = false;
    hipEvent_t plan_copied = nullptr;
    ~SlicePre() {
        if (done) {
            (void)hipEventSynchronize(done);
            (void)hipEventDestroy(done);
        }
        if (plan_copied) {
            (void)hipEventSynchronize(plan_copied);
            (void)hipEventDestroy(plan_copied);
        }
    }
};

struct BuildRanges {
    int64_t mn[2], mx[2], cnt[2];
    bool operator==(const BuildRanges &o) const {
        return std::memcmp(mn, o.mn, sizeof mn) == 0 && std::memcmp(mx, o.mx, sizeof mx) == 0 &&
               std::memcmp(cnt, o.cnt, sizeof cnt) == 0;
    }
};

struct PendingSlice {
    SlicePre pre;
    std::vector<const void *> vals;
    std::vector<int64_t> offs, lens;
    std::vector<int32_t> dtypes;
    int key_idx = -1;
    std::vector<uint8_t> pred;
    std::vector<int32_t> agg_fc;
    BuildRanges br{};
    static std::vector<uint8_t> serialise(const qeh_expr *e);
    static std::vector<int32_t> agg_list(const qeh_agg *aggs, int n_aggs) {
        std::vector<int32_t> v;
        for (int i = 0; i < n_aggs; ++i) v.push_back(aggs[i].func), v.push_back(aggs[i].column);
        return v;
    }
    bool matches(const qeh_column *cols, int n_cols, int key, const qeh_expr *predicate, const qeh_agg *aggs,
                 int n_aggs) const {
        if (n_cols != (int)vals.size() || key != key_idx) return false;
// ... 1256 lines not shown
    if (probe_key_idx < 0 || probe_key_idx >= n_probe_cols) return fail(QEH_E_INVALID, "probe key index out of range");
    DeviceGuard dg(ctx->device);
    ctx->pending_slice.reset();
    if (n_aggs == 0 || std::getenv("QEH_NO_SLICES") || std::getenv("QEH_NO_OVERLAP") || slice_chunk_tiles() > 0) return QEH_OK;
    const int64_t n = probe_cols[0].length;
    for (int i = 0; i < n_probe_cols; ++i)
        if (probe_cols[i].length != n) return fail(QEH_E_INVALID, "probe columns have different lengths");
    if (probe_cols[probe_key_idx].dtype != QEH_DT_INT64) return QEH_OK;
    ColSet cols;
    QEH_TRY(make_colset(probe_cols, n_probe_cols, &cols));
    std::vector<int32_t> dts(n_probe_cols);
    std::vector<int> idx(n_probe_cols);
    for (int i = 0; i < n_probe_cols; ++i) {
        dts[i] = probe_cols[i].dtype;
        idx[i] = i;
    }
    PredPlan pp;
    QEH_TRY(plan_predicate(predicate, dts.data(), n_probe_cols, &pp));
    AggSpecs specs;
    QEH_TRY(plan_aggs(aggs, n_aggs, probe_cols, n_probe_cols, idx.data(), &specs));
    auto p = std::make_shared<PendingSlice>();
    SlicePlanIn pi;
    bool launched = false;
    QEH_TRY(slice_launch_dev(
        ctx, cols, n, pp, specs, probe_key_idx, &pi, &p->pre,
        [&](const SlicePlanIn &q, SlicePlan *out) {
            hipLaunchKernelGGL(k_slice_plan_stats, dim3(1), dim3(64), 0, ctx->stream, stats, world, row_len, q, out);
        },
        &launched));
    if (!launched) return QEH_OK;
    for (int i = 0; i < n_probe_cols; ++i) {
        p->vals.push_back(probe_cols[i].values);
        p->offs.push_back(probe_cols[i].offset);
        p->lens.push_back(probe_cols[i].length);
        p->dtypes.push_back(probe_cols[i].dtype);
    }
    p->key_idx = probe_key_idx;
    p->pred = PendingSlice::serialise(predicate);
    p->agg_fc = PendingSlice::agg_list(aggs, n_aggs);
    ctx->pending_slice = p;
    return QEH_OK;
}

struct DenseCols {
    const void *vals[kMaxAggs];
    int32_t dt[kMaxAggs];
    int32_t n;
};

__global__ void k_dense_scatter(ColRef key, int64_t n, DenseCols dc, int64_t kmin, int64_t range,
                                double *__restrict__ out) {
    for (int64_t i = (int64_t)blockIdx.x * blockDim.x + threadIdx.x; i < n; i += (int64_t)gridDim.x * blockDim.x) {
        const uint64_t o = (uint64_t)load_i64(key, i) - (uint64_t)kmin;
        if (o >= (uint64_t)range) continue;
        out[o] = 1.0;
        for (int j = 0; j < dc.n; ++j) {
            double v;
            if (dc.dt[j] == QEH_DT_FLOAT64) v = ((const double *)dc.vals[j])[i];
            else if (dc.dt[j] == QEH_DT_INT32) v = (double)((const int32_t *)dc.vals[j])[i];
            else v = (double)((const int64_t *)dc.vals[j])[i];
            out[(int64_t)(j + 1) * range + (int64_t)o] = v;
        }
    }
}

__global__ __launch_bounds__(1024) void k_dense_take(const double *__restrict__ in, int64_t kmin, int64_t range, int world,
                                                     int rank, int32_t key_dt, void *__restrict__ okeys, DenseCols oc,
                                                     int64_t *__restrict__ total, int with_status = 0) {
    __shared__ uint32_t wsum[16];
    const int t = threadIdx.x, lane = t & 63, wave = t >> 6;
    const int64_t owned = range > rank ? (range - rank + world - 1) / world : 0;
    const int64_t per = (owned + 1023) / 1024, q0 = (int64_t)t * per, q1 = q0 + per < owned ? q0 + per : owned;
    uint32_t c = 0;
    for (int64_t q = q0; q < q1; ++q) c += in[rank + q * world] > 0.0;
    const uint32_t incl = wave_incl_scan(c);
    if (lane == 63) wsum[wave] = incl;
    __syncthreads();
    uint32_t base = incl - c, all = 0;
    for (int w = 0; w < 16; ++w) {
        base += w < wave ? wsum[w] : 0u;
        all += wsum[w];
    }
    for (int64_t q = q0; q < q1; ++q) {
        const int64_t o = rank + q * world;
        if (!(in[o] > 0.0)) continue;
        const int64_t key = kmin + o;
        if (key_dt == QEH_DT_INT32) ((int32_t *)okeys)[base] = (int32_t)key;
        else ((int64_t *)okeys)[base] = key;
        for (int j = 0; j < oc.n; ++j) {
            const double v = in[(int64_t)(j + 1) * range + o];
            if (oc.dt[j] == QEH_DT_FLOAT64) ((double *)oc.vals[j])[base] = v;
            else ((int64_t *)oc.vals[j])[base] = (int64_t)v;
        }
        ++base;
    }
    if (t == 0) {
        total[0] = all;
        if (with_status) total[1] = __builtin_bit_cast(int64_t, in[(int64_t)(1 + oc.n) * range]);
    }
}

extern "C" int qeh_dense_states_f64(qeh_ctx *ctx, const qeh_column *keys, const qeh_column *vals, int n_vals,
                                    int64_t key_min, int64_t range, double *out) {
    if (!ctx || !keys || !out || n_vals < 0 || n_vals > kMaxAggs || (n_vals > 0 && !vals) || range <= 0)
        return fail(QEH_E_INVALID, "qeh_dense_states_f64: bad argument");
    QEH_TRY(check_column(*keys, "dense state key"));
    if (keys->dtype != QEH_DT_INT64 && keys->dtype != QEH_DT_INT32) return fail(QEH_E_UNSUPPORTED, "dense state keys must be Int32 / Int64");
    if (keys->validity && keys->null_count != 0) return fail(QEH_E_UNSUPPORTED, "dense state keys must be non-null");
    DenseCols dc{};
    dc.n = n_vals;
    for (int j = 0; j < n_vals; ++j) {
        QEH_TRY(check_column(vals[j], "dense state value"));
        if (vals[j].length != keys->length) return fail(QEH_E_INVALID, "dense state columns have different lengths");
        if ((vals[j].dtype != QEH_DT_INT64 && vals[j].dtype != QEH_DT_FLOAT64 && vals[j].dtype != QEH_DT_INT32) ||
            (vals[j].validity && vals[j].null_count != 0))
            return fail(QEH_E_UNSUPPORTED, "dense state values must be non-null Int32 / Int64 / Float64");
        dc.vals[j] = (const char *)vals[j].values + (size_t)vals[j].offset * dtype_size(vals[j].dtype);
        dc.dt[j] = vals[j].dtype;
    }
    DeviceGuard dg(ctx->device);
    const int64_t n = keys->length;
    if (n > 0)
        hipLaunchKernelGGL(k_dense_scatter, dim3(grid_for(ctx, n, kBlock, 8)), dim3(kBlock), 0, ctx->stream, make_colref(*keys),
                           n, dc, key_min, range, out);
    QEH_HIP(hipGetLastError());
    return QEH_OK;
}

static int dense_states_take(qeh_ctx *ctx, const double *in, int n_vals, int64_t key_min, int64_t range, int world,
                             int rank, int32_t key_dtype, const int32_t *out_dtypes, qeh_column *out_keys,
                             qeh_column *out_vals, int64_t *out_groups, double *status) {
    if (!ctx || !in || !out_keys || !out_groups || n_vals < 0 || n_vals > kMaxAggs || (n_vals > 0 && (!out_vals || !out_dtypes)) ||
        range <= 0 || world < 1 || rank < 0 || rank >= world || (key_dtype != QEH_DT_INT64 && key_dtype != QEH_DT_INT32))
        return fail(QEH_E_INVALID, "qeh_dense_states_take: bad argument");
    for (int j = 0; j < n_vals; ++j)
        if (out_dtypes[j] != QEH_DT_INT64 && out_dtypes[j] != QEH_DT_FLOAT64)
            return fail(QEH_E_UNSUPPORTED, "dense state outputs are Int64 / Float64");
    DeviceGuard dg(ctx->device);
    *out_groups = 0;
    const int64_t cap = std::max<int64_t>((range + world - 1) / world, 1);
    QEH_TRY(alloc_column(ctx, key_dtype, cap, false, out_keys));
    DenseCols oc{};
    oc.n = n_vals;
    int made = 0, s = QEH_OK;
    for (; made < n_vals; ++made) {
        if ((s = alloc_column(ctx, out_dtypes[made], cap, false, &out_vals[made])) != QEH_OK) break;
        oc.vals[made] = out_vals[made].values;
        oc.dt[made] = out_dtypes[made];
    }
    DevBuf tot;
    if (s == QEH_OK) s = tot.alloc(ctx, 16);
    int64_t g = 0, gs[2] = {0, 0};
    if (s == QEH_OK) {
        hipLaunchKernelGGL(k_dense_take, dim3(1), dim3(1024), 0, ctx->stream, in, key_min, range, world, rank, key_dtype,
                           out_keys->values, oc, tot.as<int64_t>(), status ? 1 : 0);
        s = hipGetLastError() == hipSuccess ? read_small(ctx, gs, tot.p, status ? 16 : 8)
                                            : fail(QEH_E_HIP, "dense take launch failed");
        g = gs[0];
        if (status) *status = __builtin_bit_cast(double, gs[1]);
    }
    if (s != QEH_OK) {
        qeh_column_release(ctx, out_keys);
        for (int j = 0; j < made; ++j) qeh_column_release(ctx, &out_vals[j]);
        return s;
    }
    out_keys->length = g;
    for (int j = 0; j < n_vals; ++j) out_vals[j].length = g;
    *out_groups = g;
    return QEH_OK;
}

extern "C" int qeh_dense_states_take(qeh_ctx *ctx, const double *in, int n_vals, int64_t key_min, int64_t range, int world,
                                     int rank, int32_t key_dtype, const int32_t *out_dtypes, qeh_column *out_keys,
                                     qeh_column *out_vals, int64_t *out_groups) {
    return dense_states_take(ctx, in, n_vals, key_min, range, world, rank, key_dtype, out_dtypes, out_keys, out_vals,
                             out_groups, nullptr);
}

extern "C" int qeh_dense_states_take_status(qeh_ctx *ctx, const double *in, int n_vals, int64_t key_min, int64_t range,
                                            int world, int rank, int32_t key_dtype, const int32_t *out_dtypes,
                                            qeh_column *out_keys, qeh_column *out_vals, int64_t *out_groups,
                                            double *status) {
    if (!status) return fail(QEH_E_INVALID, "qeh_dense_states_take_status: bad argument");
    return dense_states_take(ctx, in, n_vals, key_min, range, world, rank, key_dtype, out_dtypes, out_keys, out_vals,
                             out_groups, status);
}

__global__ void k_seq_i64(int64_t *p, int64_t n, int64_t base, int as32) {
    for (int64_t i = (int64_t)blockIdx.x * blockDim.x + threadIdx.x; i < n; i += (int64_t)gridDim.x * blockDim.x) {
        if (as32) ((int32_t *)p)[i] = (int32_t)(base + i);
        else p[i] = base + i;
    }
}

static int join_filter_aggregate_table(qeh_ctx *ctx, const qeh_column *probe_cols, int n_probe_cols, int probe_key_idx,
                                       const qeh_expr *predicate, const uint16_t *table, int64_t key_min,
                                       uint64_t key_range, int64_t group_min, int64_t n_groups, int32_t group_dtype,
                                       const qeh_agg *aggs, int n_aggs, qeh_column *out_keys, qeh_column *out_aggs,
                                       int64_t *out_groups, double *lanes, uint32_t *dev_status = nullptr) {
    if (!ctx || !out_groups || !table || key_range == 0 || key_range >= (1ull << 32) || n_groups < 1 ||
        n_groups >= 0xFFFE || (group_dtype != QEH_DT_INT64 && group_dtype != QEH_DT_INT32))
        return fail(QEH_E_INVALID, "qeh_join_filter_aggregate_table: bad argument");
    *out_groups = 0;
    if (n_aggs == 0) return QEH_OK;
    if (probe_key_idx < 0 || probe_key_idx >= n_probe_cols) return fail(QEH_E_INVALID, "probe key index out of range");
    const int64_t n = probe_cols[0].length;
    for (int i = 0; i < n_probe_cols; ++i)
        if (probe_cols[i].length != n) return fail(QEH_E_INVALID, "probe columns have different lengths");
    DeviceGuard dg(ctx->device);
    ColSet cols;
    QEH_TRY(make_colset(probe_cols, n_probe_cols, &cols));
    std::vector<int32_t> dts(n_probe_cols);
    std::vector<int> idx(n_probe_cols);
    for (int i = 0; i < n_probe_cols; ++i) {
        dts[i] = probe_cols[i].dtype;
        idx[i] = i;
    }
    PredPlan pp;
    QEH_TRY(plan_predicate(predicate, dts.data(), n_probe_cols, &pp));
    AggSpecs specs;
    QEH_TRY(plan_aggs(aggs, n_aggs, probe_cols, n_probe_cols, idx.data(), &specs));
    if (probe_cols[probe_key_idx].dtype != QEH_DT_INT64 && probe_cols[probe_key_idx].dtype != QEH_DT_INT32)
        return fail(QEH_E_UNSUPPORTED, "hash join keys must be Int32/Int64 on the device");
    SlicePre pre;
    std::shared_ptr<PendingSlice> pend = std::static_pointer_cast<PendingSlice>(ctx->pending_slice);
    ctx->pending_slice.reset();
    if (pend && pend->matches(probe_cols, n_probe_cols, probe_key_idx, predicate, aggs, n_aggs)) {
        if (pend->pre.dev_planned) QEH_TRY(resolve_dev_plan(ctx, &pend->pre, &pend->br));
        pend->take(&pre);
    }
    pend.reset();
    DevBuf gkeys, rep;
    QEH_TRY(gkeys.alloc(ctx, (size_t)n_groups * 8));
    QEH_TRY(rep.alloc(ctx, (size_t)n_groups * 4));
    const int g = grid_for(ctx, n_groups, kBlock, 1);
    hipLaunchKernelGGL(k_seq_i64, dim3(g), dim3(kBlock), 0, ctx->stream, gkeys.as<int64_t>(), n_groups, group_min,
                       group_dtype == QEH_DT_INT32 ? 1 : 0);
    hipLaunchKernelGGL(k_iota, dim3(g), dim3(kBlock), 0, ctx->stream, rep.as<uint32_t>(), n_groups);
    QEH_HIP(hipGetLastError());
    qeh_column kc{};
    kc.dtype = group_dtype;
    kc.length = n_groups;
    kc.values = gkeys.p;
    KeyCols keys{};
    keys.n = 1;
    keys.c[0] = make_colref(kc);
    GidSource src{};
    src.jt.kind = TK_DIRECT;
    src.jt.payload16 = const_cast<uint16_t *>(table);
    src.jt.kmin = key_min;
    src.jt.kmax = (int64_t)((uint64_t)key_min + key_range - 1ull);
    src.jt.range = key_range;
    src.jt.unique = 1;
    src.key_col = probe_key_idx;
    const int32_t kd = group_dtype;
    if (lanes)
        for (int a = 0; a < specs.n; ++a)
            if (!((specs.a[a].kind == AK_SUM_F && specs.a[a].func == QEH_AGG_SUM && specs.a[a].cnt_slot == 0) ||
                  (specs.a[a].kind == AK_COUNT && specs.a[a].func == QEH_AGG_COUNT)))
                return fail(QEH_E_UNSUPPORTED, "dense lanes carry COUNT and non-null float SUM aggregates only");
    return aggregate_rows(ctx, GM_JOIN, cols, n, pp, src, specs, n_groups, keys, &kd, rep.as<uint32_t>(), true,
                          "join_filter_aggregate", out_keys, out_aggs, out_groups, &pre, lanes, dev_status);
}

extern "C" int qeh_join_filter_aggregate_table(qeh_ctx *ctx, const qeh_column *probe_cols, int n_probe_cols,
                                               int probe_key_idx, const qeh_expr *predicate, const uint16_t *table,
                                               int64_t key_min, uint64_t key_range, int64_t group_min, int64_t n_groups,
                                               int32_t group_dtype, const qeh_agg *aggs, int n_aggs, qeh_column *out_keys,
                                               qeh_column *out_aggs, int64_t *out_groups) {
    return join_filter_aggregate_table(ctx, probe_cols, n_probe_cols, probe_key_idx, predicate, table, key_min, key_range,
                                       group_min, n_groups, group_dtype, aggs, n_aggs, out_keys, out_aggs, out_groups,
                                       nullptr);
}

extern "C" int qeh_join_filter_aggregate_table_lanes(qeh_ctx *ctx, const qeh_column *probe_cols, int n_probe_cols,
                                                     int probe_key_idx, const qeh_expr *predicate, const uint16_t *table,
                                                     int64_t key_min, uint64_t key_range, int64_t n_groups,
                                                     const qeh_agg *aggs, int n_aggs, double *lanes) {
    if (!lanes) return fail(QEH_E_INVALID, "qeh_join_filter_aggregate_table_lanes: bad argument");
    if (n_aggs == 0) return fail(QEH_E_INVALID, "qeh_join_filter_aggregate_table_lanes: no aggregates");
    int64_t g = 0;
    return join_filter_aggregate_table(ctx, probe_cols, n_probe_cols, probe_key_idx, predicate, table, key_min, key_range,
                                       0, n_groups, QEH_DT_INT64, aggs, n_aggs, nullptr, nullptr, &g, lanes);
}

extern "C" int qeh_join_filter_aggregate_table_lanes_async(qeh_ctx *ctx, const qeh_column *probe_cols, int n_probe_cols,
                                                           int probe_key_idx, const qeh_expr *predicate,
                                                           const uint16_t *table, int64_t key_min, uint64_t key_range,
                                                           int64_t n_groups, const qeh_agg *aggs, int n_aggs, double *lanes,
                                                           uint32_t *dev_status) {
    if (!lanes || !dev_status) return fail(QEH_E_INVALID, "qeh_join_filter_aggregate_table_lanes_async: bad argument");
    if (n_aggs == 0) return fail(QEH_E_INVALID, "qeh_join_filter_aggregate_table_lanes_async: no aggregates");
    int64_t g = 0;
    return join_filter_aggregate_table(ctx, probe_cols, n_probe_cols, probe_key_idx, predicate, table, key_min, key_range,
                                       0, n_groups, QEH_DT_INT64, aggs, n_aggs, nullptr, nullptr, &g, lanes, dev_status);
}

constexpr int kFusedNotEligible = -4;

static void launch_slice_partition_early(qeh_ctx *ctx, const FastIn &in, const PredPlan &pp, int nterms, int nacol,
                                         int64_t n_tiles, int64_t tail_rows, int grid, const SliceRegions &rg,
                                         const SlicePlan *dplan, const FusedPro &fp) {
    const bool nt = fast_nt_mode() == 1;
    KernelTimer kta(ctx, "slice_partition");
    const HashTable t{};
#define QEH_SE(NTV, NAV, NTB)                                                                                            \
    hipLaunchKernelGGL((k_slice_partition<NTV, NAV, NTB, 0, true>), dim3(grid), dim3(kSliceBlock), 0, ctx->stream, in,   \
                       pp.terms, 0, 0, n_tiles, rg, t, dplan, tail_rows, fp)
#define QEH_SE_NA(NTV, NTB)                      \
    if (nacol == 0) { QEH_SE(NTV, 0, NTB); }      \
    else if (nacol == 1) { QEH_SE(NTV, 1, NTB); } \
    else { QEH_SE(NTV, 2, NTB); }
#define QEH_SE_NT(NTB)                          \
    if (nterms == 0) { QEH_SE_NA(0, NTB) }      \
    else if (nterms == 1) { QEH_SE_NA(1, NTB) } \
    else { QEH_SE_NA(2, NTB) }
    if (nt) { QEH_SE_NT(true) } else { QEH_SE_NT(false) }
#undef QEH_SE_NT
#undef QEH_SE_NA
#undef QEH_SE
}

static int fused_join_filter_aggregate(qeh_ctx *ctx, const ColSet &cols, int64_t n, const PredPlan &pp,
                                       const AggSpecs &specs_in, int key_col, const qeh_column &bk, const qeh_column &gk,
                                       qeh_column *out_keys, qeh_column *out_aggs, int64_t *out_groups) {
    if (std::getenv("QEH_NO_FUSED") || std::getenv("QEH_NO_SLICES")) return kFusedNotEligible;
    const size_t timing_mark = ctx->timing_pending.size();
    const bool bk_nulls = bk.validity && bk.null_count != 0, gk_nulls = gk.validity && gk.null_count != 0;
    if (bk.dtype != QEH_DT_INT64 || bk_nulls || (gk.dtype != QEH_DT_INT64 && gk.dtype != QEH_DT_INT32) || gk_nulls)
        return kFusedNotEligible;
    const int64_t nd = bk.length;
    if (nd <= 0 || nd >= ((int64_t)1 << 32) || gk.length != nd) return kFusedNotEligible;
    FastIn in;
    int nterms, nacol;
    if (!fast_cols_eligible(cols, pp, key_col, specs_in, &in, &nterms, &nacol) || nacol > 2 ||
        (nacol == 2 && std::getenv("QEH_NO_FUSED_AGG2")))
        return kFusedNotEligible;
    const int64_t tile_rows = nacol == 2 ? (int64_t)SliceShape<2, true>::TILE
                                         : (nacol ? SliceShape<1, true>::TILE : SliceShape<0, true>::TILE);
    const int chunk = nacol == 2 ? SliceShape<2, true>::CH : (nacol ? SliceShape<1, true>::CH : SliceShape<0, true>::CH);
    const int64_t n_tiles = n / tile_rows, tail = n - n_tiles * tile_rows;
    if (n_tiles == 0) return kFusedNotEligible;
    AggSpecs specs = specs_in;
    const int64_t g_cap = std::min<int64_t>(kSliceStateWords / std::max(specs.n_slots, 1), 0xFFFE);
    const int64_t Gs = g_cap;
    specs.shards = 1;
    if (std::getenv("QEH_FUSED_SHARDS"))
        while (specs.shards < 64 && (size_t)specs.n_slots * Gs * 8 * specs.shards * 2 <= (8u << 20)) specs.shards *= 2;
    const int64_t n_all = n_tiles + (tail ? 1 : 0);
    const int grid = (int)std::min<int64_t>({(int64_t)ctx->props.multiProcessorCount, n_all,
                                             (int64_t)kMaxSliceGrid});
    const uint64_t tiles_per_wg = (uint64_t)((n_all + grid - 1) / grid);

    DevBuf mm, plan, ditems, dcount, kbuf, vbuf, vbuf2, cbuf, states, errw, gkeys, rep;
    SlicePlanIn pi{};
    pi.min_bytes = 6ull << 20;
    if (const char *e = std::getenv("QEH_SLICE_MIN_BYTES")) pi.min_bytes = std::strtoull(e, nullptr, 10);
    pi.grid = grid;
    pi.n_slots = specs.n_slots;
    pi.sparse_ok = direct_sparse_allowed() ? 1 : 0;
    pi.chunk = chunk;
    pi.alloc_items = tiles_per_wg * grid * (uint64_t)tile_rows * 5 / 4 + (uint64_t)grid * kSliceMaxF * (256 + 2 * chunk);
    const uint64_t dim_items = (uint64_t)nd * 5 / 4 + (uint64_t)grid * kSliceMaxF * 64;
    if (dim_items >= (1ull << 32)) return kFusedNotEligible;
    const uint64_t nreg_max = (uint64_t)grid * kSliceMaxF;
    QEH_TRY(mm.alloc(ctx, sizeof(MinMax) * 2 * (size_t)minmax_partials_max_blocks(ctx) + 16));
    QEH_TRY(plan.alloc(ctx, sizeof(FusedPlan)));
    QEH_TRY(ditems.alloc(ctx, dim_items * 4 + 64));
    QEH_TRY(dcount.alloc(ctx, nreg_max * 4 + 64));
    QEH_TRY(kbuf.alloc(ctx, pi.alloc_items * 2 + 64));
    if (nacol) QEH_TRY(vbuf.alloc(ctx, pi.alloc_items * 8 + 64));
    if (nacol > 1) QEH_TRY(vbuf2.alloc(ctx, pi.alloc_items * 8 + 64));
    QEH_TRY(cbuf.alloc(ctx, nreg_max * 4 + 64));
    QEH_TRY(states.alloc(ctx, (size_t)specs.shards * specs.n_slots * Gs * 8));
    QEH_TRY(errw.alloc(ctx, 32));
    QEH_TRY(gkeys.alloc(ctx, (size_t)Gs * 8));
    QEH_TRY(rep.alloc(ctx, (size_t)Gs * 4));
    uint32_t *st = errw.as<uint32_t>();
    SliceRegions rg{};
    rg.key = kbuf.as<uint16_t>();
    rg.val = nacol ? vbuf.as<int64_t>() : nullptr;
    rg.val2 = nacol > 1 ? vbuf2.as<int64_t>() : nullptr;
    rg.count = cbuf.as<uint32_t>();
    rg.overflow = st + 1;
    FusedPlan *dplan = plan.as<FusedPlan>();
    {
        KernelTimer kt(ctx, "fused_build");
        const qeh_column both[2] = {bk, gk};
        int nb = 0;
        QEH_TRY(columns_minmax_partials(ctx, both, 2, mm.as<MinMax>(), &nb));
        const int gp = (int)std::max<int64_t>(1, std::min<int64_t>(ctx->props.multiProcessorCount,
                                                                   (specs.shards * specs.n_slots * Gs + 4095) / 4096));
        hipLaunchKernelGGL(k_fused_plan, dim3(gp), dim3(1024), 0, ctx->stream, mm.as<MinMax>(), nb, pi, g_cap, nd, dim_items,
                           dplan, st, states.as<uint64_t>(), Gs, specs);
    }
    QEH_HIP(hipGetLastError());
    FusedPro fp{};
    fp.dk = (const int64_t *)bk.values + bk.offset;
    fp.dg = make_colref(gk);
    fp.nd = nd;
    fp.ditems = ditems.as<uint32_t>();
    fp.dcount = dcount.as<uint32_t>();
    fp.status = st;
    fp.gkeys = gkeys.p;
    fp.rep = rep.as<uint32_t>();
    fp.G = Gs;
    fp.as32 = gk.dtype == QEH_DT_INT32 ? 1 : 0;
    fp.plan = dplan;
    launch_slice_partition_early(ctx, in, pp, nterms, nacol, n_tiles, tail, grid, rg, &dplan->sp, fp);
    {
        KernelTimer ktb(ctx, "slice_probe");
        DimSlices dim{ditems.as<uint32_t>(), dcount.as<uint32_t>(), st + 4, dplan};
        const bool pf = slice_probe_prefetch();
        const int gridB = ctx->props.multiProcessorCount;
        const HashTable t{};
        static const bool pv = !(std::getenv("QEH_FUSED_PV") && std::atoi(std::getenv("QEH_FUSED_PV")) == 0);
#define QEH_SD(NAV, PFV, PVV)                                                                                              \
    hipLaunchKernelGGL((k_slice_probe<NAV, false, PFV, PVV, true>), dim3(gridB), dim3(kSliceBlock), 0, ctx->stream, rg,   \
                       grid, 0, t, in, specs, Gs, states.as<uint64_t>(), dim)
        if (nacol == 0) {
            if (pf) QEH_SD(0, true, false);
            else QEH_SD(0, false, false);
        } else if (nacol == 2) {
            if (pf) QEH_SD(2, true, false);
            else QEH_SD(2, false, false);
        } else if (pv) {
            if (pf) QEH_SD(1, true, true);
            else QEH_SD(1, false, true);
        } else {
            if (pf) QEH_SD(1, true, false);
            else QEH_SD(1, false, false);
        }
#undef QEH_SD
    }
    QEH_HIP(hipGetLastError());
    if (specs.shards > 1) {
        const int64_t words = (int64_t)specs.n_slots * Gs;
        hipLaunchKernelGGL(k_states_fold, dim3((unsigned)((words + 255) / 256)), dim3(256), 0, ctx->stream,
                           states.as<uint64_t>(), Gs, specs);
    }
    QEH_HIP(hipGetLastError());
    qeh_column kc{};
    kc.dtype = gk.dtype;
    kc.length = Gs;
    kc.values = gkeys.p;
    KeyCols keys{};
    keys.n = 1;
    keys.c[0] = make_colref(kc);
    OutCols oc{};
    int made = 0;
    auto cleanup = [&]() {
        for (int i = 0; i < made; ++i) qeh_column_release(ctx, i == 0 ? &out_keys[0] : &out_aggs[i - 1]);
        made = 0;
    };
    for (int i = 0; i < 1 + specs.n; ++i) {
        qeh_column *c = i == 0 ? &out_keys[0] : &out_aggs[i - 1];
        int dt;
        bool nullable;
        if (i == 0) {
            dt = gk.dtype;
            nullable = false;
        } else {
            const AggSpec &sp = specs.a[i - 1];
            dt = agg_output_type(sp.func, sp.in_type);
            nullable = sp.func != QEH_AGG_COUNT;
        }
        const int s = alloc_column(ctx, dt, Gs, nullable, c);
        if (s != QEH_OK) {
            cleanup();
            return s;
        }
        ++made;
        oc.c[i].values = c->values;
        oc.c[i].validity = (uint32_t *)c->validity;
        oc.c[i].dtype = dt;
    }
    {
        KernelTimer kt(ctx, "aggregate_finalize");
        hipLaunchKernelGGL(k_fused_finish, dim3(1), dim3(1024), 0, ctx->stream, states.as<uint64_t>(), Gs, keys,
                           rep.as<uint32_t>(), specs, oc, (uint64_t *)(st + 2));
    }
    uint32_t sw[8];
    int s = hipGetLastError() == hipSuccess ? QEH_OK : fail(QEH_E_HIP, "fused join-aggregate: launch failed");
    if (s == QEH_OK) s = read_small(ctx, sw, errw.p, 32);
    if (s == QEH_OK && !sw[0] && (!sw[5] || sw[1] || sw[4])) s = kFusedNotEligible;
    if (s == kFusedNotEligible && !sw[5]) {
        for (size_t i = timing_mark; i < ctx->timing_pending.size(); ++i) ctx->timing_pending[i].name += "_declined";
    }
    if (s == QEH_OK) s = kernel_error_status(sw[0], "aggregate");
    if (s != QEH_OK) {
        cleanup();
        return s;
    }
    const int64_t out_n = (int64_t)((uint64_t)sw[2] | ((uint64_t)sw[3] << 32));
    for (int i = 0; i < 1 + specs.n; ++i) {
        qeh_column *c = i == 0 ? &out_keys[0] : &out_aggs[i - 1];
        c->length = out_n;
        c->null_count = c->validity ? -1 : 0;
    }
    *out_groups = out_n;
    return QEH_OK;
}


__global__ __launch_bounds__(1024) void k_fused_plan_stats(const int64_t *__restrict__ M, int world, int row_len,
                                                           SlicePlanIn pi, int64_t g_cap, FusedPlan *out,
                                                           uint32_t *__restrict__ st, uint64_t *__restrict__ states,
                                                           int64_t G, AggSpecs specs) {
    const int64_t words = (int64_t)specs.shards * specs.n_slots * G;
    for (int64_t i = (int64_t)blockIdx.x * blockDim.x + threadIdx.x; i < words; i += (int64_t)gridDim.x * blockDim.x) {
        const int64_t slot = (i / G) % specs.n_slots;
        uint64_t v = 0;
        for (int a = 0; a < specs.n; ++a)
            if (specs.a[a].val_slot == slot) v = (uint64_t)agg_init_value(specs.a[a].kind);
        states[i] = v;
    }
    if (blockIdx.x != 0 || threadIdx.x != 0) return;
    int64_t tot = 0, kmn = INT64_MAX, kmx = INT64_MIN, gmn = INT64_MAX, gmx = INT64_MIN, bitmap = 0;
    for (int r = 0; r < world; ++r) {
        const int64_t *m = M + (int64_t)r * row_len;
        bitmap |= m[5];
        if (m[0] <= 0) continue;
        tot += m[0];
        kmn = m[1] < kmn ? m[1] : kmn, kmx = m[2] > kmx ? m[2] : kmx;
        gmn = m[3] < gmn ? m[3] : gmn, gmx = m[4] > gmx ? m[4] : gmx;
    }
    FusedPlan p{};
    p.sp = plan_slices(pi, kmn, kmx, tot, gmn, gmx, tot);
    const bool live = !bitmap && tot > 0 && kmn <= kmx && gmn <= gmx;
    p.gmin = gmn;
    p.ngroups = live ? (int64_t)((uint64_t)gmx - (uint64_t)gmn + 1ull) : 0;
    p.dcap = 0;
    p.sp.ok = p.sp.ok && live && p.ngroups >= 1 && p.ngroups <= g_cap && p.ngroups < 0xFFFF;
    *out = p;
    for (int i = 0; i < 8; ++i) st[i] = 0u;
    st[5] = p.sp.ok ? 1u : 0u;
}

__device__ __forceinline__ uint32_t dim_item(const FusedPlan &pl, int64_t k, int64_t g, uint32_t &it) {
    const uint64_t o = (uint64_t)k - (uint64_t)pl.sp.kmin;
    const uint64_t gs = (uint64_t)g - (uint64_t)pl.gmin;
    if (o >= pl.sp.range || gs >= (uint64_t)pl.ngroups) return 0xFFFFFFFFu;
    it = ((uint32_t)(o & (kSliceKeys - 1)) << 16) | ((uint32_t)gs + 1u);
    return (uint32_t)(o >> kSliceBits);
}
__global__ __launch_bounds__(1024) void k_dim_items(const int64_t *__restrict__ dk, ColRef dg, int64_t nd, uint64_t span,
                                                    const FusedPlan *__restrict__ plan, uint32_t *__restrict__ items,
                                                    uint32_t *__restrict__ offs, uint32_t *__restrict__ st) {
    constexpr int DR = 8, S = kSliceMaxF;
    __shared__ uint32_t lc[S], ls[S];
    const int tid = threadIdx.x;
    const FusedPlan pl = *plan;
    for (int i = tid; i < S; i += 1024) lc[i] = 0u;
    __syncthreads();
    const int64_t per = (nd + gridDim.x - 1) / gridDim.x;
    const int64_t lo = (int64_t)blockIdx.x * per, hi = lo + per < nd ? lo + per : nd;
    bool bad = false;
    auto pass = [&](bool place) {
        for (int64_t c0 = lo; c0 < hi; c0 += 1024 * DR) {
            int64_t kk[DR], gg[DR];
#pragma unroll
            for (int q = 0; q < DR; ++q) {
                const int64_t i = c0 + (int64_t)q * 1024 + tid;
                kk[q] = i < hi ? dk[i] : 0;
                gg[q] = i < hi ? load_i64(dg, i) : 0;
            }
#pragma unroll
            for (int q = 0; q < DR; ++q) {
                if (c0 + (int64_t)q * 1024 + tid >= hi) continue;
                uint32_t it;
                const uint32_t b = dim_item(pl, kk[q], gg[q], it);
                if (b == 0xFFFFFFFFu) bad = true;
                else if (place) items[(uint64_t)blockIdx.x * span + atomicAdd(&ls[b], 1u)] = it;
                else atomicAdd(&lc[b], 1u);
            }
        }
    };
    if (pl.sp.ok) pass(false);
    __syncthreads();
    uint32_t *o = offs + (uint64_t)blockIdx.x * 2 * (S + 1);
    if (tid < 64) {
        const int lane = tid;
        uint32_t c3[3], t = 0;
#pragma unroll
        for (int q = 0; q < 3; ++q) {
            const int b = lane * 3 + q;
            c3[q] = b < S ? (lc[b] + 3u) & ~3u : 0u;
            t += c3[q];
        }
        uint32_t incl = t;
#pragma unroll
        for (int d = 1; d < 64; d <<= 1) {
            const uint32_t a = __shfl_up(incl, d, 64);
            if (lane >= d) incl += a;
        }
        uint32_t run = incl - t;
#pragma unroll
        for (int q = 0; q < 3; ++q) {
            const int b = lane * 3 + q;
            if (b < S) ls[b] = run;
            run += c3[q];
        }
        if (lane == 63) o[S] = incl;
    }
    __syncthreads();
    for (int b = tid; b < S; b += 1024) o[b] = ls[b], o[S + 1 + b] = lc[b];
    __syncthreads();
    if (pl.sp.ok) pass(true);
    if (bad) st[1] = 1u;
}

struct FusedItems {
    DevBuf plan, kbuf, vbuf, cbuf, states, errw;
    SliceRegions rg{};
    FastIn in{};
    AggSpecs specs{};
    int nacol = 0, grid = 0;
    int64_t Gs = 0;
    int pw = 0, prank = 0, S = 0;
    uint64_t blockcap = 0, cap = 0;
    DevBuf pkey, pval, pcnt, prb, ptot, rrb, roff;
};

static int fused_items_begin(qeh_ctx *ctx, const qeh_column *probe_cols, int n_probe_cols, int probe_key_idx,
                             const qeh_expr *predicate, const qeh_agg *aggs, int n_aggs, const int64_t *stats_dev,
                             int world, int row_len, void **handle, bool check_only, int pw = 0, int prank = 0) {
    if (!ctx || (!check_only && (!handle || !stats_dev || world < 1 || row_len < 6)) || n_aggs < 1 || n_probe_cols < 1 ||
        probe_key_idx < 0 || probe_key_idx >= n_probe_cols)
        return fail(QEH_E_INVALID, "qeh_fused_items_begin: bad argument");
    if (handle) *handle = nullptr;
    DeviceGuard dg(ctx->device);
    const int64_t n = probe_cols[0].length;
    for (int i = 0; i < n_probe_cols; ++i)
        if (probe_cols[i].length != n) return fail(QEH_E_INVALID, "probe columns have different lengths");
    ColSet cols;
    QEH_TRY(make_colset(probe_cols, n_probe_cols, &cols));
    std::vector<int32_t> dts(n_probe_cols);
    std::vector<int> idx(n_probe_cols);
    for (int i = 0; i < n_probe_cols; ++i) dts[i] = probe_cols[i].dtype, idx[i] = i;
    PredPlan pp;
    QEH_TRY(plan_predicate(predicate, dts.data(), n_probe_cols, &pp));
    auto fi = std::make_unique<FusedItems>();
    QEH_TRY(plan_aggs(aggs, n_aggs, probe_cols, n_probe_cols, idx.data(), &fi->specs));
    for (int a = 0; a < fi->specs.n; ++a)
        if (!((fi->specs.a[a].kind == AK_SUM_F && fi->specs.a[a].func == QEH_AGG_SUM && fi->specs.a[a].cnt_slot == 0) ||
              (fi->specs.a[a].kind == AK_COUNT && fi->specs.a[a].func == QEH_AGG_COUNT)))
            return fail(QEH_E_UNSUPPORTED, "qeh_fused_items_begin: COUNT and non-null float SUM aggregates only");
    int nterms = 0;
    if (!fast_cols_eligible(cols, pp, probe_key_idx, fi->specs, &fi->in, &nterms, &fi->nacol) || fi->nacol > 1)
        return fail(QEH_E_UNSUPPORTED, "qeh_fused_items_begin: probe columns outside the fused pipeline's shapes");
    if (check_only) return QEH_OK;
    const int64_t tile_rows = fi->nacol ? SliceShape<1, true>::TILE : SliceShape<0, true>::TILE;
    const int chunk = fi->nacol ? SliceShape<1, true>::CH : SliceShape<0, true>::CH;
    const int64_t n_tiles = n / tile_rows, tail = n - n_tiles * tile_rows, n_all = n_tiles + (tail ? 1 : 0);
    AggSpecs &specs = fi->specs;
    specs.shards = 1;
    fi->Gs = std::min<int64_t>(kSliceStateWords / std::max(specs.n_slots, 1), 0xFFFE);
    fi->grid = pw > 1 ? (int)std::min<int64_t>(ctx->props.multiProcessorCount, kMaxSliceGrid)
                      : (int)std::max<int64_t>(1, std::min<int64_t>({(int64_t)ctx->props.multiProcessorCount, n_all,
                                                                     (int64_t)kMaxSliceGrid}));
    const uint64_t tiles_per_wg = (uint64_t)((n_all + fi->grid - 1) / fi->grid);
    SlicePlanIn pi{};
    pi.min_bytes = 6ull << 20;
    if (const char *e = std::getenv("QEH_SLICE_MIN_BYTES")) pi.min_bytes = std::strtoull(e, nullptr, 10);
    pi.grid = fi->grid;
    pi.n_slots = specs.n_slots;
    pi.sparse_ok = direct_sparse_allowed() ? 1 : 0;
    pi.chunk = chunk;
    pi.alloc_items = tiles_per_wg * fi->grid * (uint64_t)tile_rows * 5 / 4 + (uint64_t)fi->grid * kSliceMaxF * (256 + 2 * chunk);
    pi.world = pw;
    const uint64_t nreg_max = (uint64_t)fi->grid * (kSliceMaxF + (pw > 1 ? pw : 0));
    fi->pw = pw, fi->prank = prank;
    fi->rg.pw = pw, fi->rg.prank = prank;
    QEH_TRY(fi->plan.alloc(ctx, sizeof(FusedPlan)));
    QEH_TRY(fi->kbuf.alloc(ctx, pi.alloc_items * 2 + 64));
    if (fi->nacol) QEH_TRY(fi->vbuf.alloc(ctx, pi.alloc_items * 8 + 64));
    QEH_TRY(fi->cbuf.alloc(ctx, nreg_max * 4 + 64));
    QEH_TRY(fi->states.alloc(ctx, (size_t)specs.n_slots * fi->Gs * 8));
    QEH_TRY(fi->errw.alloc(ctx, 32));
    uint32_t *st = fi->errw.as<uint32_t>();
    fi->rg.key = fi->kbuf.as<uint16_t>();
    fi->rg.val = fi->nacol ? fi->vbuf.as<int64_t>() : nullptr;
    fi->rg.count = fi->cbuf.as<uint32_t>();
    fi->rg.overflow = st + 1;
    FusedPlan *dplan = fi->plan.as<FusedPlan>();
    {
        KernelTimer kt(ctx, "fused_build");
        const int gp = (int)std::max<int64_t>(1, std::min<int64_t>(ctx->props.multiProcessorCount,
                                                                   (specs.n_slots * fi->Gs + 4095) / 4096));
        hipLaunchKernelGGL(k_fused_plan_stats, dim3(gp), dim3(1024), 0, ctx->stream, stats_dev, world, row_len, pi, fi->Gs,
                           dplan, st, fi->states.as<uint64_t>(), fi->Gs, specs);
    }
    QEH_HIP(hipGetLastError());
    FusedPro fp{};
    fp.status = st;
    fp.plan = dplan;
    if (n_tiles > 0 || tail > 0)
        launch_slice_partition_early(ctx, fi->in, pp, nterms, fi->nacol, n_tiles, tail, fi->grid, fi->rg, &dplan->sp, fp);
    else
        QEH_HIP(hipMemsetAsync(fi->cbuf.p, 0, nreg_max * 4, ctx->stream));
    QEH_HIP(hipGetLastError());
    *handle = fi.release();
    return QEH_OK;
}

extern "C" int qeh_fused_items_begin(qeh_ctx *ctx, const qeh_column *probe_cols, int n_probe_cols, int probe_key_idx,
                                     const qeh_expr *predicate, const qeh_agg *aggs, int n_aggs, const int64_t *stats_dev,
                                     int world, int row_len, void **handle) {
    return fused_items_begin(ctx, probe_cols, n_probe_cols, probe_key_idx, predicate, aggs, n_aggs, stats_dev, world, row_len,
                             handle, false);
}

extern "C" int qeh_fused_items_check(qeh_ctx *ctx, const qeh_column *probe_cols, int n_probe_cols, int probe_key_idx,
                                     const qeh_expr *predicate, const qeh_agg *aggs, int n_aggs) {
    return fused_items_begin(ctx, probe_cols, n_probe_cols, probe_key_idx, predicate, aggs, n_aggs, nullptr, 0, 0, nullptr,
                             true);
}

extern "C" int qeh_fused_items_build(qeh_ctx *ctx, void *handle, const qeh_column *build_key, const qeh_column *group_key,
                                     int n_blocks, uint64_t span, uint32_t *items, uint32_t *offs) {
    if (!ctx || !handle || !build_key || !group_key || !offs || !items || n_blocks < 1 || n_blocks > kMaxSliceGrid ||
        (span & 3))
        return fail(QEH_E_INVALID, "qeh_fused_items_build: bad argument (1..512 blocks, span a multiple of 4)");
    FusedItems *fi = (FusedItems *)handle;
    DeviceGuard dg(ctx->device);
    if (build_key->dtype != QEH_DT_INT64 || (build_key->validity && build_key->null_count != 0) ||
        (group_key->dtype != QEH_DT_INT64 && group_key->dtype != QEH_DT_INT32) ||
        (group_key->validity && group_key->null_count != 0) || group_key->length != build_key->length)
        return fail(QEH_E_UNSUPPORTED, "qeh_fused_items_build: one non-null Int64 key and one non-null integer group key");
    const int64_t nd = build_key->length;
    if ((uint64_t)((nd + n_blocks - 1) / n_blocks) + 4ull * kSliceMaxF > span)
        return fail(QEH_E_INVALID, "qeh_fused_items_build: span below ceil(rows / n_blocks) + 640");
    KernelTimer kt(ctx, "fused_build");
    hipLaunchKernelGGL(k_dim_items, dim3(n_blocks), dim3(1024), 0, ctx->stream,
                       (const int64_t *)build_key->values + build_key->offset, make_colref(*group_key), nd, span,
                       fi->plan.as<FusedPlan>(), items, offs, fi->errw.as<uint32_t>());
    QEH_HIP(hipGetLastError());
    return QEH_OK;
}

extern "C" int qeh_fused_items_finish(qeh_ctx *ctx, void *handle, const uint32_t *items, uint64_t span,
                                      const uint32_t *offs, int n_regions, int64_t n_groups, double *lanes) {
    const int world = n_regions;
    if (!ctx || !handle || !offs || !lanes || world < 1 || world > kMaxSliceGrid || n_groups < 1 || (span & 3) ||
        (uint64_t)world * span >= (1ull << 32))
        return fail(QEH_E_INVALID, "qeh_fused_items_finish: bad argument");
    std::unique_ptr<FusedItems> fi((FusedItems *)handle);
    DeviceGuard dg(ctx->device);
    if (n_groups > fi->Gs) return fail(QEH_E_UNSUPPORTED, "qeh_fused_items_finish: more groups than the states hold");
    uint32_t *st = fi->errw.as<uint32_t>();
    {
        KernelTimer ktb(ctx, "slice_probe");
        DimSlices dim{items, nullptr, st + 4, fi->plan.as<FusedPlan>(), world, 0, span, offs};
        const int gridB = ctx->props.multiProcessorCount;
        const HashTable t{};
        const bool pf = slice_probe_prefetch();
        if (fi->nacol == 0) {
            if (pf) hipLaunchKernelGGL((k_slice_probe<0, false, true, false, true>), dim3(gridB), dim3(kSliceBlock), 0, ctx->stream,
                                       fi->rg, fi->grid, 0, t, fi->in, fi->specs, fi->Gs, fi->states.as<uint64_t>(), dim);
            else hipLaunchKernelGGL((k_slice_probe<0, false, false, false, true>), dim3(gridB), dim3(kSliceBlock), 0, ctx->stream,
                                    fi->rg, fi->grid, 0, t, fi->in, fi->specs, fi->Gs, fi->states.as<uint64_t>(), dim);
        } else {
            if (pf) hipLaunchKernelGGL((k_slice_probe<1, false, true, true, true>), dim3(gridB), dim3(kSliceBlock), 0, ctx->stream,
                                       fi->rg, fi->grid, 0, t, fi->in, fi->specs, fi->Gs, fi->states.as<uint64_t>(), dim);
            else hipLaunchKernelGGL((k_slice_probe<1, false, false, true, true>), dim3(gridB), dim3(kSliceBlock), 0, ctx->stream,
                                    fi->rg, fi->grid, 0, t, fi->in, fi->specs, fi->Gs, fi->states.as<uint64_t>(), dim);
        }
    }
    QEH_HIP(hipGetLastError());
    const int64_t ne = (int64_t)(1 + fi->specs.n) * n_groups;
    hipLaunchKernelGGL(k_states_lanes, dim3((unsigned)((ne + 255) / 256)), dim3(256), 0, ctx->stream,
                       (const uint64_t *)fi->states.as<uint64_t>(), fi->Gs, n_groups, fi->specs, lanes, (const uint32_t *)st, 1);
    QEH_HIP(hipGetLastError());
    return QEH_OK;
}

extern "C" int qeh_fused_items_abort(qeh_ctx *ctx, void *handle) {
    if (!ctx || !handle) return QEH_OK;
    DeviceGuard dg(ctx->device);
    std::unique_ptr<FusedItems> fi((FusedItems *)handle);
    QEH_HIP(hipStreamSynchronize(ctx->stream));
    return QEH_OK;
}


__global__ __launch_bounds__(1024) void k_region_scan(const uint32_t *__restrict__ cnt, int64_t E, const int64_t *bases,
                                                      uint64_t blockcap, int F, int pw, int grid,
// ... 278 lines not shown
```

### query-engine_amd/csrc/qeh_internal.h

```cpp
#pragma once

#include <hip/hip_runtime.h>

#include <cstdint>
#include <cstring>
#include <map>
#include <memory>
#include <mutex>
#include <string>
#include <unordered_map>
#include <vector>

#include "../../include/qeh.h"

namespace qeh {

void set_error(const std::string &msg);
int fail(int status, const std::string &msg);

#define QEH_HIP(expr)                                                                       \
    do {                                                                                    \
        hipError_t _e = (expr);                                                             \
        if (_e != hipSuccess)                                                               \
            return ::qeh::fail(QEH_E_HIP, std::string(#expr) + ": " + hipGetErrorString(_e)); \
    } while (0)

#define QEH_TRY(expr)               \
    do {                            \
        int _s = (expr);            \
        if (_s != QEH_OK) return _s; \
    } while (0)

class DevicePool {
  public:
    explicit DevicePool(int device) : device_(device) {}
    int device() const { return device_; }
    ~DevicePool();
    int alloc(size_t bytes, void **out);
    int free(void *p);
    void trim();
    size_t bytes_in_use() const { return in_use_; }

  private:
    static size_t size_class(size_t bytes);
    int device_;
    std::mutex mu_;
    std::multimap<size_t, void *> free_;
    std::unordered_map<void *, size_t> live_;
    size_t in_use_ = 0;
};

struct TimingRecord {
    std::string name;
    hipEvent_t start, stop;
};

}

namespace qeh {
struct SourceCache;
}

struct qeh_ctx {
    int device = 0;
    hipStream_t own_stream = nullptr;
    hipStream_t stream = nullptr;
    hipStream_t aux_stream = nullptr;
    qeh::DevicePool *pool = nullptr;
    hipDeviceProp_t props{};
    void *scratch = nullptr;
    size_t scratch_bytes = 0;
    void *pinned = nullptr;
    size_t pinned_bytes = 0;
    void *pinned_plan = nullptr;
    bool timing = false;
    std::vector<qeh::TimingRecord> timing_pending;
    std::vector<hipEvent_t> event_free;
    std::map<std::string, std::pair<double, int64_t>> timing_done;
    std::shared_ptr<qeh::SourceCache> source_cache;
    struct MinMaxMemoEntry {
        const void *values, *validity;
        int64_t offset, length;
        int32_t dtype;
        int64_t mn, mx, cnt;
    };
    bool mm_memo_on = false;
    int mm_memo_n = 0;
    MinMaxMemoEntry mm_memo[4];
    int64_t build_beside_rows = 0;
    std::shared_ptr<void> pending_slice;
};

namespace qeh {

struct DeviceGuard {
    int prev = -1;
    explicit DeviceGuard(int dev) {
        (void)hipGetDevice(&prev);
        if (prev != dev) (void)hipSetDevice(dev);
    }
    ~DeviceGuard() {
        int cur = -1;
        (void)hipGetDevice(&cur);
        if (prev >= 0 && cur != prev) (void)hipSetDevice(prev);
    }
};

struct MinMaxMemoScope {
    qeh_ctx *c;
    explicit MinMaxMemoScope(qeh_ctx *ctx) : c(ctx) { c->mm_memo_on = true, c->mm_memo_n = 0; }
    ~MinMaxMemoScope() { c->mm_memo_on = false, c->mm_memo_n = 0; }
};

struct DevBuf {
    qeh_ctx *ctx = nullptr;
    void *p = nullptr;
    size_t n = 0;
    DevBuf() = default;
    DevBuf(const DevBuf &) = delete;
    DevBuf &operator=(const DevBuf &) = delete;
    ~DevBuf() { reset(); }
    int alloc(qeh_ctx *c, size_t bytes) {
        reset();
        ctx = c;
        n = bytes;
        return c->pool->alloc(bytes ? bytes : 1, &p);
    }
    void reset() {
        if (p && ctx) ctx->pool->free(p);
        p = nullptr;
        n = 0;
    }
    void *release() {
        void *r = p;
        p = nullptr;
        return r;
    }
    template <class T>
    T *as() const { return reinterpret_cast<T *>(p); }
};

struct KernelTimer {
    qeh_ctx *ctx;
    const char *name;
    hipStream_t stream;
    hipEvent_t a = nullptr, b = nullptr;
    KernelTimer(qeh_ctx *c, const char *n, hipStream_t s = nullptr);
    ~KernelTimer();
};

hipStream_t aux_stream(qeh_ctx *ctx);

int read_small(qeh_ctx *ctx, void *host_dst, const void *dev_src, size_t bytes);
int scratch_zeroed(qeh_ctx *ctx, size_t bytes, void **out);

inline int grid_for(qeh_ctx *ctx, int64_t work_items, int items_per_block, int per_cu = 8) {
    int64_t want = (work_items + items_per_block - 1) / items_per_block;
    int64_t cap = (int64_t)ctx->props.multiProcessorCount * per_cu;
    if (want > cap) want = cap;
    if (want < 1) want = 1;
    return (int)want;
}

inline bool is_temporal(int dt) { return dt >= QEH_DT_DATE32 && dt <= QEH_DT_TIMESTAMP_NS; }
inline int physical_dtype(int dt) {
    if (dt == QEH_DT_DATE32) return QEH_DT_INT32;
    return is_temporal(dt) ? QEH_DT_INT64 : dt;
}
inline qeh_column physical_view(const qeh_column &c) {
    qeh_column v = c;
    v.dtype = physical_dtype(c.dtype);
    v.owned = 0;
    return v;
}

size_t dtype_size(int dt);
int alloc_column(qeh_ctx *ctx, int dtype, int64_t length, bool with_validity, qeh_column *out);

}
```

### query-engine_amd/csrc/runtime.cpp

```cpp
#include "qeh_internal.h"

#include <cstdio>

namespace qeh {

static thread_local std::string g_last_error;

void set_error(const std::string &msg) { g_last_error = msg; }

int fail(int status, const std::string &msg) {
    g_last_error = msg;
    return status;
}

size_t DevicePool::size_class(size_t bytes) {
    if (bytes <= 256) return 256;
    if (bytes >= (size_t(1) << 30)) return (bytes + 0xFFFFF) & ~size_t(0xFFFFF);
    size_t c = 256;
    while (c < bytes) c <<= 1;
    return c;
}

DevicePool::~DevicePool() { trim(); }

int DevicePool::alloc(size_t bytes, void **out) {
    size_t cls = size_class(bytes);
    {
        std::lock_guard<std::mutex> g(mu_);
        auto it = free_.find(cls);
        if (it != free_.end()) {
            void *p = it->second;
            free_.erase(it);
            live_[p] = cls;
            in_use_ += cls;
            *out = p;
            return QEH_OK;
        }
    }
    void *p = nullptr;
    hipError_t e = hipMalloc(&p, cls);
    if (e != hipSuccess) {
        (void)hipGetLastError();
        trim();
        e = hipMalloc(&p, cls);
        if (e != hipSuccess) {
            (void)hipGetLastError();
            return fail(QEH_E_OOM, "device allocation of " + std::to_string(bytes) + " bytes failed");
        }
    }
    std::lock_guard<std::mutex> g(mu_);
    live_[p] = cls;
    in_use_ += cls;
    *out = p;
    return QEH_OK;
}

int DevicePool::free(void *p) {
    if (!p) return QEH_OK;
    std::lock_guard<std::mutex> g(mu_);
    auto it = live_.find(p);
    if (it == live_.end()) return fail(QEH_E_INVALID, "qeh_device_free: pointer not owned by this context");
    free_.emplace(it->second, p);
    in_use_ -= it->second;
    live_.erase(it);
    return QEH_OK;
}

void DevicePool::trim() {
    std::lock_guard<std::mutex> g(mu_);
    for (auto &kv : free_) hipFree(kv.second);
    free_.clear();
}

static hipEvent_t take_event(qeh_ctx *ctx) {
    if (!ctx->event_free.empty()) {
        hipEvent_t e = ctx->event_free.back();
        ctx->event_free.pop_back();
        return e;
    }
    hipEvent_t e = nullptr;
    hipEventCreate(&e);
    return e;
}

KernelTimer::KernelTimer(qeh_ctx *c, const char *n, hipStream_t s) : ctx(c), name(n), stream(s ? s : c->stream) {
    if (!ctx->timing) return;
    a = take_event(ctx);
    b = take_event(ctx);
    hipEventRecord(a, stream);
}

KernelTimer::~KernelTimer() {
    if (!ctx->timing || !a) return;
    hipEventRecord(b, stream);
    ctx->timing_pending.push_back({name, a, b});
}

hipStream_t aux_stream(qeh_ctx *ctx) {
    if (!ctx->aux_stream) (void)hipStreamCreateWithFlags(&ctx->aux_stream, hipStreamNonBlocking);
    return ctx->aux_stream;
}

static void drain_timing(qeh_ctx *ctx) {
    for (auto &r : ctx->timing_pending) {
        hipEventSynchronize(r.stop);
        float ms = 0.f;
        hipEventElapsedTime(&ms, r.start, r.stop);
        auto &slot = ctx->timing_done[r.name];
        slot.first += ms;
        slot.second += 1;
        ctx->event_free.push_back(r.start);
        ctx->event_free.push_back(r.stop);
    }
    ctx->timing_pending.clear();
}

int read_small(qeh_ctx *ctx, void *host_dst, const void *dev_src, size_t bytes) {
    if (bytes == 0) return QEH_OK;
    if (bytes > ctx->pinned_bytes) {
        if (ctx->pinned) hipHostFree(ctx->pinned);
        ctx->pinned = nullptr;
        size_t n = bytes < 65536 ? 65536 : bytes;
        QEH_HIP(hipHostMalloc(&ctx->pinned, n, hipHostMallocDefault));
        ctx->pinned_bytes = n;
    }
    QEH_HIP(hipMemcpyAsync(ctx->pinned, dev_src, bytes, hipMemcpyDeviceToHost, ctx->stream));
    QEH_HIP(hipStreamSynchronize(ctx->stream));
    std::memcpy(host_dst, ctx->pinned, bytes);
    return QEH_OK;
}

int scratch_zeroed(qeh_ctx *ctx, size_t bytes, void **out) {
    bytes = (bytes + 255) & ~size_t(255);
    if (bytes > ctx->scratch_bytes) {
        if (ctx->scratch) ctx->pool->free(ctx->scratch);
        ctx->scratch = nullptr;
        size_t n = bytes < (1 << 20) ? (1 << 20) : bytes;
        QEH_TRY(ctx->pool->alloc(n, &ctx->scratch));
        ctx->scratch_bytes = n;
    }
    QEH_HIP(hipMemsetAsync(ctx->scratch, 0, bytes, ctx->stream));
    *out = ctx->scratch;
    return QEH_OK;
}

size_t dtype_size(int dt) {
    switch (physical_dtype(dt)) {
        case QEH_DT_INT32: return 4;
        case QEH_DT_UINT32: return 4;
        case QEH_DT_FLOAT32: return 4;
        case QEH_DT_INT64: return 8;
        case QEH_DT_FLOAT64: return 8;
        default: return 0;
    }
}

int alloc_column(qeh_ctx *ctx, int dtype, int64_t length, bool with_validity, qeh_column *out) {
    std::memset(out, 0, sizeof(*out));
    out->dtype = dtype;
    out->owned = 1;
    out->length = length;
    out->null_count = with_validity ? -1 : 0;
    size_t bytes;
    if (dtype == QEH_DT_BOOL) bytes = (size_t)((length + 63) / 64) * 8;
    else bytes = (size_t)length * dtype_size(dtype);
    if (bytes == 0) bytes = 8;
    QEH_TRY(ctx->pool->alloc(bytes, &out->values));
    if (with_validity) {
        size_t vb = (size_t)((length + 63) / 64) * 8;
        if (vb == 0) vb = 8;
        void *v = nullptr;
        int s = ctx->pool->alloc(vb, &v);
        if (s != QEH_OK) {
            ctx->pool->free(out->values);
            out->values = nullptr;
            return s;
        }
        out->validity = (uint8_t *)v;
    }
    return QEH_OK;
}

}

using namespace qeh;

extern "C" {

int qeh_abi_version(void) { return QEH_ABI_VERSION; }

const char *qeh_last_error(void) { return g_last_error.c_str(); }

int qeh_init(int device, qeh_ctx **out) {
    if (!out) return fail(QEH_E_INVALID, "qeh_init: out is NULL");
    *out = nullptr;
    int n = 0;
    hipError_t e = hipGetDeviceCount(&n);
    if (e != hipSuccess || n == 0)
        return fail(QEH_E_HIP, "qeh_init: no HIP device available (" +
                                   std::string(hipGetErrorString(e)) + ")");
    if (device < 0 || device >= n) return fail(QEH_E_INVALID, "qeh_init: device out of range");
    QEH_HIP(hipSetDevice(device));
    qeh_ctx *ctx = new qeh_ctx();
    ctx->device = device;
    if (hipGetDeviceProperties(&ctx->props, device) != hipSuccess) {
        delete ctx;
        return fail(QEH_E_HIP, "qeh_init: hipGetDeviceProperties failed");
    }
    if (hipStreamCreateWithFlags(&ctx->own_stream, hipStreamNonBlocking) != hipSuccess) {
        delete ctx;
        return fail(QEH_E_HIP, "qeh_init: stream creation failed");
    }
    ctx->stream = ctx->own_stream;
    ctx->pool = new DevicePool(device);
    *out = ctx;
    return QEH_OK;
}

int qeh_shutdown(qeh_ctx *ctx) {
    if (!ctx) return QEH_OK;
    DeviceGuard dg(ctx->device);
    hipStreamSynchronize(ctx->stream);
    for (auto &r : ctx->timing_pending) {
        hipEventDestroy(r.start);
        hipEventDestroy(r.stop);
    }
    for (auto e : ctx->event_free) hipEventDestroy(e);
    if (ctx->scratch) ctx->pool->free(ctx->scratch);
    ctx->pending_slice.reset();
    if (ctx->aux_stream) hipStreamSynchronize(ctx->aux_stream);
    if (ctx->pinned_plan) hipHostFree(ctx->pinned_plan);
    if (ctx->pinned) hipHostFree(ctx->pinned);
    ctx->source_cache.reset();
    delete ctx->pool;
    if (ctx->own_stream) hipStreamDestroy(ctx->own_stream);
    if (ctx->aux_stream) {
        hipStreamSynchronize(ctx->aux_stream);
        hipStreamDestroy(ctx->aux_stream);
    }
    delete ctx;
    return QEH_OK;
}

int qeh_set_stream(qeh_ctx *ctx, void *hip_stream) {
    if (!ctx) return fail(QEH_E_INVALID, "null context");
    ctx->stream = hip_stream ? (hipStream_t)hip_stream : ctx->own_stream;
    return QEH_OK;
}

void *qeh_get_stream(qeh_ctx *ctx) { return ctx ? (void *)ctx->stream : nullptr; }

int qeh_synchronize(qeh_ctx *ctx) {
    if (!ctx) return fail(QEH_E_INVALID, "null context");
    DeviceGuard dg(ctx->device);
    QEH_HIP(hipStreamSynchronize(ctx->stream));
    return QEH_OK;
}

int qeh_device_alloc(qeh_ctx *ctx, size_t bytes, void **out) {
    if (!ctx || !out) return fail(QEH_E_INVALID, "qeh_device_alloc: bad argument");
    DeviceGuard dg(ctx->device);
    return ctx->pool->alloc(bytes, out);
}

int qeh_device_free(qeh_ctx *ctx, void *ptr) {
    if (!ctx) return fail(QEH_E_INVALID, "null context");
    return ctx->pool->free(ptr);
}

int qeh_pool_trim(qeh_ctx *ctx) {
    if (!ctx) return fail(QEH_E_INVALID, "null context");
    DeviceGuard dg(ctx->device);
    hipStreamSynchronize(ctx->stream);
    ctx->pool->trim();
    return QEH_OK;
}

int qeh_memcpy_h2d(qeh_ctx *ctx, void *dst, const void *src, size_t bytes) {
    if (!ctx) return fail(QEH_E_INVALID, "null context");
    if (!bytes) return QEH_OK;
    DeviceGuard dg(ctx->device);
    QEH_HIP(hipMemcpyAsync(dst, src, bytes, hipMemcpyHostToDevice, ctx->stream));
    QEH_HIP(hipStreamSynchronize(ctx->stream));
    return QEH_OK;
}

int qeh_memcpy_d2h(qeh_ctx *ctx, void *dst, const void *src, size_t bytes) {
    if (!ctx) return fail(QEH_E_INVALID, "null context");
    if (!bytes) return QEH_OK;
    DeviceGuard dg(ctx->device);
    QEH_HIP(hipMemcpyAsync(dst, src, bytes, hipMemcpyDeviceToHost, ctx->stream));
    QEH_HIP(hipStreamSynchronize(ctx->stream));
    return QEH_OK;
}

int qeh_memcpy_d2d(qeh_ctx *ctx, void *dst, const void *src, size_t bytes) {
    if (!ctx) return fail(QEH_E_INVALID, "null context");
    if (!bytes) return QEH_OK;
    DeviceGuard dg(ctx->device);
    QEH_HIP(hipMemcpyAsync(dst, src, bytes, hipMemcpyDeviceToDevice, ctx->stream));
    return QEH_OK;
}

int qeh_memset(qeh_ctx *ctx, void *dst, int value, size_t bytes) {
    if (!ctx) return fail(QEH_E_INVALID, "null context");
    DeviceGuard dg(ctx->device);
    QEH_HIP(hipMemsetAsync(dst, value, bytes, ctx->stream));
    return QEH_OK;
}

int qeh_column_release(qeh_ctx *ctx, qeh_column *col) {
    if (!ctx || !col) return fail(QEH_E_INVALID, "qeh_column_release: bad argument");
    if (col->owned) {
        if (col->values) ctx->pool->free(col->values);
        if (col->validity) ctx->pool->free(col->validity);
        if (col->offsets) ctx->pool->free(col->offsets);
    }
    std::memset(col, 0, sizeof(*col));
    return QEH_OK;
}

int qeh_timing_enable(qeh_ctx *ctx, int enable) {
    if (!ctx) return fail(QEH_E_INVALID, "null context");
    ctx->timing = enable != 0;
    return QEH_OK;
}

int qeh_timing_reset(qeh_ctx *ctx) {
    if (!ctx) return fail(QEH_E_INVALID, "null context");
    DeviceGuard dg(ctx->device);
    drain_timing(ctx);
    ctx->timing_done.clear();
    return QEH_OK;
}

int qeh_kernel_time(qeh_ctx *ctx, const char *name, double *total_ms, int64_t *launches) {
    if (!ctx || !name) return fail(QEH_E_INVALID, "qeh_kernel_time: bad argument");
    DeviceGuard dg(ctx->device);
    drain_timing(ctx);
    auto it = ctx->timing_done.find(name);
    if (total_ms) *total_ms = it == ctx->timing_done.end() ? 0.0 : it->second.first;
    if (launches) *launches = it == ctx->timing_done.end() ? 0 : it->second.second;
    return QEH_OK;
}

}
```

Baseline: 171.9 billion.

## Fuse stats into plan kernel and finalize into last probe block via tickets

Replaces the separate min/max partial-stats pass plus single-block plan kernel with a grid-wide stats+plan kernel that reduces through device atomics and a last-block ticket. The fused probe kernel now runs the group finalize in whichever block arrives last, writing status into mapped pinned host memory so the host can skip a separate finish launch and a device-to-host copy. The intent is fewer kernel launches and host round-trips per query. The cost is serialized finalize work in one block at the tail of the probe and reliance on correct atomic ordering and visibility across blocks.

```diff
diff --git a/query-engine_amd/csrc/k_aggregate.hip b/query-engine_amd/csrc/k_aggregate.hip
--- a/query-engine_amd/csrc/k_aggregate.hip
+++ b/query-engine_amd/csrc/k_aggregate.hip
@@ -593,6 +593,31 @@
     const uint32_t *offs;
 };
 
+struct OutCol {
+    void *values;
+    uint32_t *validity;
+    int32_t dtype;
+    int32_t _pad;
+};
+struct OutCols {
+    OutCol c[kMaxGroupKeys + kMaxAggs];
+};
+
+struct FusedFin {
+    uint32_t *ticket;
+    const uint32_t *rep;
+    uint32_t *st;
+    uint32_t *host_st;
+    KeyCols keys;
+    OutCols outs;
+};
+constexpr int kFinishVWords = 3584 / 32;
+template <bool AGENT>
+__device__ __forceinline__ uint32_t fused_finish_body(const uint64_t *__restrict__ states, int64_t G, const KeyCols &keys,
+                                                      const uint32_t *__restrict__ rep, const AggSpecs &specs,
+                                                      const OutCols &outs, uint64_t *__restrict__ total, uint32_t *pos,
+                                                      uint32_t (*vbits)[kFinishVWords], uint32_t *wsum);
+
 struct __attribute__((aligned(16))) SliceChunk {
     uint64_t g;
     int32_t soff;
@@ -1004,7 +1029,7 @@
 template <int NACOL, bool IDENT = false, bool PF = false, bool PV = false, bool DIM = false>
 __global__ __launch_bounds__(kSliceBlock) void k_slice_probe(SliceRegions rg, int nreg, int splits, HashTable t, FastIn in,
                                                              AggSpecs specs, int64_t G, uint64_t *__restrict__ gstates_all,
-                                                             DimSlices dim = DimSlices{}) {
+                                                             DimSlices dim = DimSlices{}, FusedFin fin = FusedFin{}) {
     constexpr int VC = NACOL > 0 ? 1 : 0;
     __shared__ __attribute__((aligned(16))) uint16_t tslice[IDENT ? 8 : kSliceKeys];
     __shared__ uint64_t lst[IDENT ? kGidStateWords : kSliceStateWords];
@@ -1106,7 +1131,7 @@
                     }
                 }
             }
-            if (dup) *dim.dup = 1u;
+            if (dup) atomicOr(dim.dup, 1u);
         } else if (!DIM && !IDENT && b != cur_b) {
             cur_b = b;
             const uint64_t k0 = (uint64_t)b << kSliceBits;
@@ -1235,6 +1260,25 @@
         }
     } else {
         slice_states_flush(lst, stride, 0, G, specs, G, gstates);
+    }
+    if constexpr (DIM) {
+        if (!fin.ticket) return;
+        asm volatile("s_waitcnt vmcnt(0)" ::: "memory");
+        __syncthreads();
+        if (tid == 0) rcnt[0] = atomicAdd(fin.ticket, 1u) == gridDim.x - 1 ? 1u : 0u;
+        __syncthreads();
+        if (!rcnt[0]) return;
+        __syncthreads();
+        const uint32_t groups = fused_finish_body<true>(gstates, G, fin.keys, fin.rep, specs, fin.outs, (uint64_t *)(fin.st + 2),
+                                                        (uint32_t *)lst, (uint32_t(*)[kFinishVWords])tslice, rcnt);
+        if (tid == 0) {
+            uint32_t sw[8];
+            for (int i = 0; i < 8; ++i) sw[i] = __hip_atomic_load(fin.st + i, __ATOMIC_RELAXED, __HIP_MEMORY_SCOPE_AGENT);
+            sw[2] = groups, sw[3] = 0u;
+            for (int i = 0; i < 8; ++i) fin.host_st[i] = sw[i];
+            __threadfence_system();
+            __hip_atomic_store(fin.ticket, 0u, __ATOMIC_RELAXED, __HIP_MEMORY_SCOPE_AGENT);
+        }
     }
 }
 
@@ -1342,9 +1386,49 @@
     if (C16 && ovf) *rg.overflow = 1u;
 }
 
-__global__ __launch_bounds__(1024) void k_fused_plan(const MinMax *__restrict__ part, int nb, SlicePlanIn pi, int64_t g_cap,
-                                                     int64_t nd, uint64_t dim_items, FusedPlan *out, uint32_t *__restrict__ st,
-                                                     uint64_t *__restrict__ states, int64_t G, AggSpecs specs) {
+constexpr int kStatsBlock = 1024;
+__device__ __forceinline__ void stats_minmax_col(const ColRef &key, int64_t n, int64_t &mn, int64_t &mx, uint32_t &invalid) {
+    const int64_t t0 = (int64_t)blockIdx.x * kStatsBlock + threadIdx.x, stride = (int64_t)gridDim.x * kStatsBlock;
+    if (key.validity == nullptr && key.dtype == QEH_DT_INT64 && ((uintptr_t)key.values & 15) == 0) {
+        typedef long long v2 __attribute__((ext_vector_type(2)));
+        const v2 *kv = (const v2 *)key.values;
+        const int64_t pairs = n / 2;
+        for (int64_t i = t0; i < pairs; i += 4 * stride) {
+            v2 q[4];
+#pragma unroll
+            for (int u = 0; u < 4; ++u)
+                q[u] = __builtin_nontemporal_load(kv + (i + u * stride < pairs ? i + u * stride : i));
+#pragma unroll
+            for (int u = 0; u < 4; ++u) {
+                const int64_t a = q[u].x, b = q[u].y;
+                mn = a < mn ? a : mn;
+                mx = a > mx ? a : mx;
+                mn = b < mn ? b : mn;
+                mx = b > mx ? b : mx;
+            }
+        }
+        if ((n & 1) && t0 == 0) {
+            const int64_t k = ((const int64_t *)key.values)[n - 1];
+            mn = k < mn ? k : mn;
+            mx = k > mx ? k : mx;
+        }
+    } else {
+        for (int64_t i = t0; i < n; i += stride) {
+            if (!col_valid(key, i)) {
+                invalid = 1u;
+                continue;
+            }
+            const int64_t k = load_i64(key, i);
+            mn = k < mn ? k : mn;
+            mx = k > mx ? k : mx;
+        }
+    }
+}
+
+__global__ __launch_bounds__(kStatsBlock) void k_fused_stats_plan(ColRef bk, ColRef gk, int64_t nd, SlicePlanIn pi, int64_t g_cap,
+                                                                  uint64_t dim_items, FusedPlan *out, uint32_t *__restrict__ st,
+                                                                  uint32_t *__restrict__ host_st, FusedSync *sync,
+                                                                  uint64_t *__restrict__ states, int64_t G, AggSpecs specs) {
     const int64_t words = (int64_t)specs.shards * specs.n_slots * G;
     for (int64_t i = (int64_t)blockIdx.x * blockDim.x + threadIdx.x; i < words; i += (int64_t)gridDim.x * blockDim.x) {
         const int64_t slot = (i / G) % specs.n_slots;
@@ -1353,55 +1437,70 @@
             if (specs.a[a].val_slot == slot) v = (uint64_t)agg_init_value(specs.a[a].kind);
         states[i] = v;
     }
-    if (blockIdx.x != 0) return;
-    __shared__ MinMax sm[2][16];
+    __shared__ int64_t sm[4][kStatsBlock / 64];
+    __shared__ uint32_t sbad[kStatsBlock / 64];
     const int lane = threadIdx.x & 63, wave = threadIdx.x >> 6;
+    uint32_t invalid = 0;
     for (int c = 0; c < 2; ++c) {
         int64_t mn = INT64_MAX, mx = INT64_MIN;
-        uint64_t cnt = 0;
-        uint32_t bad = 0;
-        for (int i = threadIdx.x; i < nb; i += blockDim.x) {
-            const MinMax q = part[(int64_t)c * nb + i];
-            mn = q.mn < mn ? q.mn : mn;
-            mx = q.mx > mx ? q.mx : mx;
-            cnt += q.cnt;
-            bad |= q.bad;
-        }
+        stats_minmax_col(c ? gk : bk, nd, mn, mx, invalid);
 #pragma unroll
         for (int d = 32; d >= 1; d >>= 1) {
             const int64_t a = __shfl_xor(mn, d, 64), b2 = __shfl_xor(mx, d, 64);
-            const uint64_t cc = __shfl_xor(cnt, d, 64);
-            const uint32_t bb = __shfl_xor(bad, d, 64);
             mn = a < mn ? a : mn;
             mx = b2 > mx ? b2 : mx;
-            cnt += cc;
-            bad |= bb;
-        }
-        if (lane == 0) sm[c][wave] = MinMax{mn, mx, cnt, bad};
-    }
+        }
+        if (lane == 0) sm[2 * c][wave] = mn, sm[2 * c + 1][wave] = mx;
+    }
+    invalid = __ballot(invalid != 0) != 0;
+    if (lane == 0) sbad[wave] = invalid;
     __syncthreads();
-    if (threadIdx.x != 0) return;
-    MinMax mm[2];
-    for (int c = 0; c < 2; ++c) {
-        mm[c] = sm[c][0];
-        for (int w = 1; w < (int)(blockDim.x >> 6); ++w) {
-            const MinMax q = sm[c][w];
-            mm[c].mn = q.mn < mm[c].mn ? q.mn : mm[c].mn;
-            mm[c].mx = q.mx > mm[c].mx ? q.mx : mm[c].mx;
-            mm[c].cnt += q.cnt;
-            mm[c].bad |= q.bad;
-        }
-    }
+    if (wave != 0) return;
+    if (lane < 4) {
+        int64_t v = sm[lane][0];
+        for (int w = 1; w < kStatsBlock / 64; ++w) {
+            const int64_t q = sm[lane][w];
+            v = (lane & 1) ? (q > v ? q : v) : (q < v ? q : v);
+        }
+        if (lane & 1) {
+            if (v != INT64_MIN) __hip_atomic_fetch_max(&sync->mm[lane].v, v, __ATOMIC_RELAXED, __HIP_MEMORY_SCOPE_AGENT);
+        } else {
+            if (v != INT64_MAX) __hip_atomic_fetch_min(&sync->mm[lane].v, v, __ATOMIC_RELAXED, __HIP_MEMORY_SCOPE_AGENT);
+        }
+    } else if (lane == 4) {
+        uint32_t bad = 0;
+        for (int w = 0; w < kStatsBlock / 64; ++w) bad |= sbad[w];
+        if (bad) __hip_atomic_fetch_or(&sync->invalid.v, (int64_t)1, __ATOMIC_RELAXED, __HIP_MEMORY_SCOPE_AGENT);
+    }
+    asm volatile("s_waitcnt vmcnt(0)" ::: "memory");
+    uint32_t ticket = 0;
+    if (lane == 0)
+        ticket = (uint32_t)__hip_atomic_fetch_add(&sync->ticket_a.v, (int64_t)1, __ATOMIC_RELAXED, __HIP_MEMORY_SCOPE_AGENT);
+    ticket = __shfl(ticket, 0, 64);
+    if (ticket != gridDim.x - 1) return;
+    int64_t w = 0;
+    if (lane < 5) w = __hip_atomic_load(lane < 4 ? &sync->mm[lane].v : &sync->invalid.v, __ATOMIC_RELAXED, __HIP_MEMORY_SCOPE_AGENT);
+    const int64_t kmn = __shfl(w, 0, 64), kmx = __shfl(w, 1, 64), gmn = __shfl(w, 2, 64), gmx = __shfl(w, 3, 64);
+    const bool bad = __shfl(w, 4, 64) != 0;
+    if (lane < 5)
+        __hip_atomic_store(lane < 4 ? &sync->mm[lane].v : &sync->invalid.v,
+                           lane == 4 ? (int64_t)0 : ((lane & 1) ? INT64_MIN : INT64_MAX), __ATOMIC_RELAXED,
+                           __HIP_MEMORY_SCOPE_AGENT);
+    if (lane != 0) return;
+    __hip_atomic_store(&sync->ticket_a.v, (int64_t)0, __ATOMIC_RELAXED, __HIP_MEMORY_SCOPE_AGENT);
+    const int64_t cnt = (nd > 0 && kmn <= kmx && gmn <= gmx) ? nd : 0;
     FusedPlan p{};
-    p.sp = plan_slices(pi, mm[0].mn, mm[0].mx, (int64_t)mm[0].cnt, mm[1].mn, mm[1].mx, (int64_t)mm[1].cnt);
-    const bool full = (int64_t)mm[0].cnt == nd && (int64_t)mm[1].cnt == nd && !mm[0].bad && !mm[1].bad;
-    p.gmin = mm[1].mn;
-    p.ngroups = full ? (int64_t)((uint64_t)mm[1].mx - (uint64_t)mm[1].mn + 1ull) : 0;
+    p.sp = plan_slices(pi, kmn, kmx, cnt, gmn, gmx, cnt);
+    const bool full = cnt == nd && !bad;
+    p.gmin = gmn;
+    p.ngroups = full ? (int64_t)((uint64_t)gmx - (uint64_t)gmn + 1ull) : 0;
     p.dcap = p.sp.F > 0 ? dim_items / ((uint64_t)pi.grid * p.sp.F) / 4 * 4 : 0;
     p.sp.ok = p.sp.ok && full && p.ngroups >= 1 && p.ngroups <= g_cap && p.ngroups < 0xFFFF && p.dcap >= 4;
     *out = p;
-    for (int i = 0; i < 8; ++i) st[i] = 0u;
-    st[5] = p.sp.ok ? 1u : 0u;
+    const uint32_t ok = p.sp.ok ? 1u : 0u;
+    for (int i = 0; i < 8; ++i) st[i] = i == 5 ? ok : 0u;
+    for (int i = 0; i < 8; ++i) host_st[i] = i == 5 ? ok : 0u;
+    __threadfence_system();
 }
 
 __device__ __forceinline__ void emit_matches(const uint32_t *e, const int64_t *v, const bool *live, int64_t amin,
@@ -1975,16 +2074,6 @@
         flags[g] = states[g] != 0;
 }
 
-struct OutCol {
-    void *values;
-    uint32_t *validity;
-    int32_t dtype;
-    int32_t _pad;
-};
-struct OutCols {
-    OutCol c[kMaxGroupKeys + kMaxAggs];
-};
-
 __device__ __forceinline__ void write_value(const OutCol &o, int64_t p, int64_t payload, bool valid) {
     if (o.validity && valid) atomicOr(&o.validity[p >> 5], 1u << (p & 31));
     switch (o.dtype) {
@@ -2039,12 +2128,16 @@
     }
 }
 
-__global__ __launch_bounds__(1024) void k_fused_finish(const uint64_t *__restrict__ states, int64_t G, KeyCols keys,
-                                                       const uint32_t *__restrict__ rep, AggSpecs specs, OutCols outs,
-                                                       uint64_t *__restrict__ total) {
-    __shared__ uint32_t pos[kSliceStateWords];
-    __shared__ uint32_t vbits[kMaxGroupKeys + kMaxAggs][kSliceStateWords / 32];
-    __shared__ uint32_t wsum[16];
+static_assert(kFinishVWords == kSliceStateWords / 32, "validity words");
+template <bool AGENT>
+__device__ __forceinline__ uint32_t fused_finish_body(const uint64_t *__restrict__ states, int64_t G, const KeyCols &keys,
+                                                      const uint32_t *__restrict__ rep, const AggSpecs &specs,
+                                                      const OutCols &outs, uint64_t *__restrict__ total, uint32_t *pos,
+                                                      uint32_t (*vbits)[kFinishVWords], uint32_t *wsum) {
+    auto state = [&](int64_t i) -> uint64_t {
+        if constexpr (AGENT) return ld_agent(states + i);
+        return states[i];
+    };
     const int t = threadIdx.x, lane = t & 63, wave = t >> 6;
     const int nout = keys.n + specs.n;
     const int64_t vwords = (G + 31) / 32;
@@ -2052,7 +2145,7 @@
         for (int64_t w = t; w < vwords; w += blockDim.x) vbits[c][w] = 0u;
     const int64_t per = (G + 1023) / 1024, g0 = (int64_t)t * per, g1 = g0 + per < G ? g0 + per : G;
     uint32_t c = 0;
-    for (int64_t g = g0; g < g1; ++g) c += states[g] != 0;
+    for (int64_t g = g0; g < g1; ++g) c += state(g) != 0;
     const uint32_t incl = wave_incl_scan(c);
     if (lane == 63) wsum[wave] = incl;
     __syncthreads();
@@ -2063,7 +2156,7 @@
     }
     for (int64_t g = g0; g < g1; ++g) {
         pos[g] = base;
-        base += states[g] != 0;
+        base += state(g) != 0;
     }
     if (t == 0) *total = all;
     __syncthreads();
@@ -2074,7 +2167,7 @@
         write_value(o, p, payload, true);
     };
     for (int64_t g = t; g < G; g += blockDim.x) {
-        const uint64_t rows = states[g];
+        const uint64_t rows = state(g);
         if (!rows) continue;
         const int64_t p = pos[g];
         for (int k = 0; k < keys.n; ++k) {
@@ -2083,8 +2176,8 @@
         }
         for (int a = 0; a < specs.n; ++a) {
             const AggSpec sp = specs.a[a];
-            const uint64_t cnt = sp.cnt_slot ? states[(int64_t)sp.cnt_slot * G + g] : rows;
-            const int64_t v = sp.kind == AK_COUNT ? 0 : (int64_t)states[(int64_t)sp.val_slot * G + g];
+            const uint64_t cnt = sp.cnt_slot ? state((int64_t)sp.cnt_slot * G + g) : rows;
+            const int64_t v = sp.kind == AK_COUNT ? 0 : (int64_t)state((int64_t)sp.val_slot * G + g);
             const int o = keys.n + a;
             const bool i32 = sp.in_type == QEH_DT_INT32;
             const bool flt = sp.in_type == QEH_DT_FLOAT32 || sp.in_type == QEH_DT_FLOAT64;
@@ -2104,6 +2197,16 @@
     for (int c = 0; c < nout; ++c)
         if (outs.c[c].validity)
             for (int64_t w = t; w < vwords; w += blockDim.x) outs.c[c].validity[w] = vbits[c][w];
+    return all;
+}
+
+__global__ __launch_bounds__(1024) void k_fused_finish(const uint64_t *__restrict__ states, int64_t G, KeyCols keys,
+                                                       const uint32_t *__restrict__ rep, AggSpecs specs, OutCols outs,
+                                                       uint64_t *__restrict__ total) {
+    __shared__ uint32_t pos[kSliceStateWords];
+    __shared__ uint32_t vbits[kMaxGroupKeys + kMaxAggs][kFinishVWords];
+    __shared__ uint32_t wsum[16];
+    fused_finish_body<false>(states, G, keys, rep, specs, outs, total, pos, vbits, wsum);
 }
 
 static int agg_output_type(int func, int in_type) {
@@ -3966,7 +4069,7 @@
                                          int64_t n_tiles, int64_t tail_rows, int grid, const SliceRegions &rg,
                                          const SlicePlan *dplan, const FusedPro &fp) {
     const bool nt = fast_nt_mode() == 1;
-    KernelTimer kta(ctx, "slice_partition");
+    KernelTimer kta(ctx, "slice_partition", nullptr, true);
     const HashTable t{};
 #define QEH_SE(NTV, NAV, NTB)                                                                                            \
     hipLaunchKernelGGL((k_slice_partition<NTV, NAV, NTB, 0, true>), dim3(grid), dim3(kSliceBlock), 0, ctx->stream, in,   \
@@ -3989,6 +4092,8 @@
                                        const AggSpecs &specs_in, int key_col, const qeh_column &bk, const qeh_column &gk,
                                        qeh_column *out_keys, qeh_column *out_aggs, int64_t *out_groups) {
     if (std::getenv("QEH_NO_FUSED") || std::getenv("QEH_NO_SLICES")) return kFusedNotEligible;
+    static const bool no_agg2 = std::getenv("QEH_NO_FUSED_AGG2") != nullptr;
+    static const bool fused_shards = std::getenv("QEH_FUSED_SHARDS") != nullptr;
     const size_t timing_mark = ctx->timing_pending.size();
     const bool bk_nulls = bk.validity && bk.null_count != 0, gk_nulls = gk.validity && gk.null_count != 0;
     if (bk.dtype != QEH_DT_INT64 || bk_nulls || (gk.dtype != QEH_DT_INT64 && gk.dtype != QEH_DT_INT32) || gk_nulls)
@@ -3998,7 +4103,7 @@
     FastIn in;
     int nterms, nacol;
     if (!fast_cols_eligible(cols, pp, key_col, specs_in, &in, &nterms, &nacol) || nacol > 2 ||
-        (nacol == 2 && std::getenv("QEH_NO_FUSED_AGG2")))
+        (nacol == 2 && no_agg2))
         return kFusedNotEligible;
     const int64_t tile_rows = nacol == 2 ? (int64_t)SliceShape<2, true>::TILE
                                          : (nacol ? SliceShape<1, true>::TILE : SliceShape<0, true>::TILE);
@@ -4009,14 +4114,14 @@
     const int64_t g_cap = std::min<int64_t>(kSliceStateWords / std::max(specs.n_slots, 1), 0xFFFE);
     const int64_t Gs = g_cap;
     specs.shards = 1;
-    if (std::getenv("QEH_FUSED_SHARDS"))
+    if (fused_shards)
         while (specs.shards < 64 && (size_t)specs.n_slots * Gs * 8 * specs.shards * 2 <= (8u << 20)) specs.shards *= 2;
     const int64_t n_all = n_tiles + (tail ? 1 : 0);
     const int grid = (int)std::min<int64_t>({(int64_t)ctx->props.multiProcessorCount, n_all,
                                              (int64_t)kMaxSliceGrid});
     const uint64_t tiles_per_wg = (uint64_t)((n_all + grid - 1) / grid);
 
-    DevBuf mm, plan, ditems, dcount, kbuf, vbuf, vbuf2, cbuf, states, errw, gkeys, rep;
+    DevBuf plan, ditems, dcount, kbuf, vbuf, vbuf2, cbuf, states, errw, gkeys, rep;
     SlicePlanIn pi{};
     pi.min_bytes = 6ull << 20;
     if (const char *e = std::getenv("QEH_SLICE_MIN_BYTES")) pi.min_bytes = std::strtoull(e, nullptr, 10);
@@ -4028,37 +4133,34 @@
     const uint64_t dim_items = (uint64_t)nd * 5 / 4 + (uint64_t)grid * kSliceMaxF * 64;
     if (dim_items >= (1ull << 32)) return kFusedNotEligible;
     const uint64_t nreg_max = (uint64_t)grid * kSliceMaxF;
-    QEH_TRY(mm.alloc(ctx, sizeof(MinMax) * 2 * (size_t)minmax_partials_max_blocks(ctx) + 16));
+    QEH_TRY(fused_sync_blocks(ctx));
     QEH_TRY(plan.alloc(ctx, sizeof(FusedPlan)));
+    QEH_TRY(states.alloc(ctx, (size_t)specs.shards * specs.n_slots * Gs * 8));
+    QEH_TRY(errw.alloc(ctx, 32));
+    uint32_t *st = errw.as<uint32_t>();
+    FusedPlan *dplan = plan.as<FusedPlan>();
+    FusedSync *sync = (FusedSync *)ctx->fused_sync;
+    {
+        KernelTimer kt(ctx, "fused_build");
+        const int gp = (int)std::max<int64_t>(1, std::min<int64_t>(ctx->props.multiProcessorCount, (nd + 8191) / 8192));
+        hipLaunchKernelGGL(k_fused_stats_plan, dim3(gp), dim3(kStatsBlock), 0, ctx->stream, make_colref(bk), make_colref(gk), nd,
+                           pi, g_cap, dim_items, dplan, st, ctx->pinned_status_dev, sync, states.as<uint64_t>(), Gs, specs);
+    }
+    QEH_HIP(hipGetLastError());
     QEH_TRY(ditems.alloc(ctx, dim_items * 4 + 64));
     QEH_TRY(dcount.alloc(ctx, nreg_max * 4 + 64));
     QEH_TRY(kbuf.alloc(ctx, pi.alloc_items * 2 + 64));
     if (nacol) QEH_TRY(vbuf.alloc(ctx, pi.alloc_items * 8 + 64));
     if (nacol > 1) QEH_TRY(vbuf2.alloc(ctx, pi.alloc_items * 8 + 64));
     QEH_TRY(cbuf.alloc(ctx, nreg_max * 4 + 64));
-    QEH_TRY(states.alloc(ctx, (size_t)specs.shards * specs.n_slots * Gs * 8));
-    QEH_TRY(errw.alloc(ctx, 32));
     QEH_TRY(gkeys.alloc(ctx, (size_t)Gs * 8));
     QEH_TRY(rep.alloc(ctx, (size_t)Gs * 4));
-    uint32_t *st = errw.as<uint32_t>();
     SliceRegions rg{};
     rg.key = kbuf.as<uint16_t>();
     rg.val = nacol ? vbuf.as<int64_t>() : nullptr;
     rg.val2 = nacol > 1 ? vbuf2.as<int64_t>() : nullptr;
     rg.count = cbuf.as<uint32_t>();
     rg.overflow = st + 1;
-    FusedPlan *dplan = plan.as<FusedPlan>();
-    {
-        KernelTimer kt(ctx, "fused_build");
-        const qeh_column both[2] = {bk, gk};
-        int nb = 0;
-        QEH_TRY(columns_minmax_partials(ctx, both, 2, mm.as<MinMax>(), &nb));
-        const int gp = (int)std::max<int64_t>(1, std::min<int64_t>(ctx->props.multiProcessorCount,
-                                                                   (specs.shards * specs.n_slots * Gs + 4095) / 4096));
-        hipLaunchKernelGGL(k_fused_plan, dim3(gp), dim3(1024), 0, ctx->stream, mm.as<MinMax>(), nb, pi, g_cap, nd, dim_items,
-                           dplan, st, states.as<uint64_t>(), Gs, specs);
-    }
-    QEH_HIP(hipGetLastError());
     FusedPro fp{};
     fp.dk = (const int64_t *)bk.values + bk.offset;
     fp.dg = make_colref(gk);
@@ -4072,46 +4174,17 @@
     fp.as32 = gk.dtype == QEH_DT_INT32 ? 1 : 0;
     fp.plan = dplan;
     launch_slice_partition_early(ctx, in, pp, nterms, nacol, n_tiles, tail, grid, rg, &dplan->sp, fp);
-    {
-        KernelTimer ktb(ctx, "slice_probe");
-        DimSlices dim{ditems.as<uint32_t>(), dcount.as<uint32_t>(), st + 4, dplan};
-        const bool pf = slice_probe_prefetch();
-        const int gridB = ctx->props.multiProcessorCount;
-        const HashTable t{};
-        static const bool pv = !(std::getenv("QEH_FUSED_PV") && std::atoi(std::getenv("QEH_FUSED_PV")) == 0);
-#define QEH_SD(NAV, PFV, PVV)                                                                                              \
-    hipLaunchKernelGGL((k_slice_probe<NAV, false, PFV, PVV, true>), dim3(gridB), dim3(kSliceBlock), 0, ctx->stream, rg,   \
-                       grid, 0, t, in, specs, Gs, states.as<uint64_t>(), dim)
-        if (nacol == 0) {
-            if (pf) QEH_SD(0, true, false);
-            else QEH_SD(0, false, false);
-        } else if (nacol == 2) {
-            if (pf) QEH_SD(2, true, false);
-            else QEH_SD(2, false, false);
-        } else if (pv) {
-            if (pf) QEH_SD(1, true, true);
-            else QEH_SD(1, false, true);
-        } else {
-            if (pf) QEH_SD(1, true, false);
-            else QEH_SD(1, false, false);
-        }
-#undef QEH_SD
-    }
-    QEH_HIP(hipGetLastError());
-    if (specs.shards > 1) {
-        const int64_t words = (int64_t)specs.n_slots * Gs;
-        hipLaunchKernelGGL(k_states_fold, dim3((unsigned)((words + 255) / 256)), dim3(256), 0, ctx->stream,
-                           states.as<uint64_t>(), Gs, specs);
-    }
     QEH_HIP(hipGetLastError());
     qeh_column kc{};
     kc.dtype = gk.dtype;
     kc.length = Gs;
     kc.values = gkeys.p;
-    KeyCols keys{};
-    keys.n = 1;
-    keys.c[0] = make_colref(kc);
-    OutCols oc{};
+    FusedFin fin{};
+    fin.keys.n = 1;
+    fin.keys.c[0] = make_colref(kc);
+    fin.rep = rep.as<uint32_t>();
+    fin.st = st;
+    fin.host_st = ctx->pinned_status_dev;
     int made = 0;
     auto cleanup = [&]() {
         for (int i = 0; i < made; ++i) qeh_column_release(ctx, i == 0 ? &out_keys[0] : &out_aggs[i - 1]);
@@ -4135,18 +4208,54 @@
             return s;
         }
         ++made;
-        oc.c[i].values = c->values;
-        oc.c[i].validity = (uint32_t *)c->validity;
-        oc.c[i].dtype = dt;
-    }
+        fin.outs.c[i].values = c->values;
+        fin.outs.c[i].validity = (uint32_t *)c->validity;
+        fin.outs.c[i].dtype = dt;
+    }
+    const bool in_b = specs.shards == 1;
+    if (in_b) fin.ticket = (uint32_t *)&sync->ticket_b.v;
     {
-        KernelTimer kt(ctx, "aggregate_finalize");
-        hipLaunchKernelGGL(k_fused_finish, dim3(1), dim3(1024), 0, ctx->stream, states.as<uint64_t>(), Gs, keys,
-                           rep.as<uint32_t>(), specs, oc, (uint64_t *)(st + 2));
+        KernelTimer ktb(ctx, "slice_probe", nullptr, true);
+        DimSlices dim{ditems.as<uint32_t>(), dcount.as<uint32_t>(), st + 4, dplan};
+        const bool pf = slice_probe_prefetch();
+        const int gridB = ctx->props.multiProcessorCount;
+        const HashTable t{};
+        static const bool pv = !(std::getenv("QEH_FUSED_PV") && std::atoi(std::getenv("QEH_FUSED_PV")) == 0);
+#define QEH_SD(NAV, PFV, PVV)                                                                                              \
+    hipLaunchKernelGGL((k_slice_probe<NAV, false, PFV, PVV, true>), dim3(gridB), dim3(kSliceBlock), 0, ctx->stream, rg,   \
+                       grid, 0, t, in, specs, Gs, states.as<uint64_t>(), dim, fin)
+        if (nacol == 0) {
+            if (pf) QEH_SD(0, true, false);
+            else QEH_SD(0, false, false);
+        } else if (nacol == 2) {
+            if (pf) QEH_SD(2, true, false);
+            else QEH_SD(2, false, false);
+        } else if (pv) {
+            if (pf) QEH_SD(1, true, true);
+            else QEH_SD(1, false, true);
+        } else {
+            if (pf) QEH_SD(1, true, false);
+            else QEH_SD(1, false, false);
+        }
+#undef QEH_SD
     }
     uint32_t sw[8];
     int s = hipGetLastError() == hipSuccess ? QEH_OK : fail(QEH_E_HIP, "fused join-aggregate: launch failed");
-    if (s == QEH_OK) s = read_small(ctx, sw, errw.p, 32);
+    if (s == QEH_OK && !in_b) {
+        const int64_t words = (int64_t)specs.n_slots * Gs;
+        hipLaunchKernelGGL(k_states_fold, dim3((unsigned)((words + 255) / 256)), dim3(256), 0, ctx->stream,
+                           states.as<uint64_t>(), Gs, specs);
+        {
+            KernelTimer kt(ctx, "aggregate_finalize");
+            hipLaunchKernelGGL(k_fused_finish, dim3(1), dim3(1024), 0, ctx->stream, states.as<uint64_t>(), Gs, fin.keys,
+                               fin.rep, specs, fin.outs, (uint64_t *)(st + 2));
+        }
+        if (hipGetLastError() != hipSuccess) s = fail(QEH_E_HIP, "fused join-aggregate: launch failed");
+        if (s == QEH_OK) s = read_small(ctx, sw, errw.p, 32);
+    } else if (s == QEH_OK) {
+        if (hipStreamSynchronize(ctx->stream) != hipSuccess) s = fail(QEH_E_HIP, "fused join-aggregate: stream failed");
+        else std::memcpy(sw, ctx->pinned_status, 32);
+    }
     if (s == QEH_OK && !sw[0] && (!sw[5] || sw[1] || sw[4])) s = kFusedNotEligible;
     if (s == kFusedNotEligible && !sw[5]) {
         for (size_t i = timing_mark; i < ctx->timing_pending.size(); ++i) ctx->timing_pending[i].name += "_declined";
diff --git a/query-engine_amd/csrc/qeh_internal.h b/query-engine_amd/csrc/qeh_internal.h
--- a/query-engine_amd/csrc/qeh_internal.h
+++ b/query-engine_amd/csrc/qeh_internal.h
@@ -53,6 +53,17 @@
 struct TimingRecord {
     std::string name;
     hipEvent_t start, stop;
+    bool shared_start = false;
+};
+
+struct FusedSync {
+    struct alignas(128) Word {
+        int64_t v;
+    };
+    Word mm[4];
+    Word invalid;
+    Word ticket_a;
+    Word ticket_b;
 };
 
 }
@@ -73,7 +84,12 @@
     void *pinned = nullptr;
     size_t pinned_bytes = 0;
     void *pinned_plan = nullptr;
+    void *fused_sync = nullptr;
+    uint32_t *pinned_status = nullptr;
+    uint32_t *pinned_status_dev = nullptr;
     bool timing = false;
+    hipEvent_t timing_last_stop = nullptr;
+    hipStream_t timing_last_stream = nullptr;
     std::vector<qeh::TimingRecord> timing_pending;
     std::vector<hipEvent_t> event_free;
     std::map<std::string, std::pair<double, int64_t>> timing_done;
@@ -145,9 +161,12 @@
     const char *name;
     hipStream_t stream;
     hipEvent_t a = nullptr, b = nullptr;
-    KernelTimer(qeh_ctx *c, const char *n, hipStream_t s = nullptr);
+    bool shared = false;
+    KernelTimer(qeh_ctx *c, const char *n, hipStream_t s = nullptr, bool chained = false);
     ~KernelTimer();
 };
+
+int fused_sync_blocks(qeh_ctx *ctx);
 
 hipStream_t aux_stream(qeh_ctx *ctx);
 
diff --git a/query-engine_amd/csrc/runtime.cpp b/query-engine_amd/csrc/runtime.cpp
--- a/query-engine_amd/csrc/runtime.cpp
+++ b/query-engine_amd/csrc/runtime.cpp
@@ -83,17 +83,25 @@
     return e;
 }
 
-KernelTimer::KernelTimer(qeh_ctx *c, const char *n, hipStream_t s) : ctx(c), name(n), stream(s ? s : c->stream) {
+KernelTimer::KernelTimer(qeh_ctx *c, const char *n, hipStream_t s, bool chained)
+    : ctx(c), name(n), stream(s ? s : c->stream) {
     if (!ctx->timing) return;
-    a = take_event(ctx);
+    if (chained && ctx->timing_last_stop && ctx->timing_last_stream == stream) {
+        a = ctx->timing_last_stop;
+        shared = true;
+    } else {
+        a = take_event(ctx);
+        hipEventRecord(a, stream);
+    }
     b = take_event(ctx);
-    hipEventRecord(a, stream);
 }
 
 KernelTimer::~KernelTimer() {
     if (!ctx->timing || !a) return;
     hipEventRecord(b, stream);
-    ctx->timing_pending.push_back({name, a, b});
+    ctx->timing_pending.push_back({name, a, b, shared});
+    ctx->timing_last_stop = b;
+    ctx->timing_last_stream = stream;
 }
 
 hipStream_t aux_stream(qeh_ctx *ctx) {
@@ -109,10 +117,11 @@
         auto &slot = ctx->timing_done[r.name];
         slot.first += ms;
         slot.second += 1;
-        ctx->event_free.push_back(r.start);
+        if (!r.shared_start) ctx->event_free.push_back(r.start);
         ctx->event_free.push_back(r.stop);
     }
     ctx->timing_pending.clear();
+    ctx->timing_last_stop = nullptr;
 }
 
 int read_small(qeh_ctx *ctx, void *host_dst, const void *dev_src, size_t bytes) {
@@ -127,6 +136,34 @@
     QEH_HIP(hipMemcpyAsync(ctx->pinned, dev_src, bytes, hipMemcpyDeviceToHost, ctx->stream));
     QEH_HIP(hipStreamSynchronize(ctx->stream));
     std::memcpy(host_dst, ctx->pinned, bytes);
+    return QEH_OK;
+}
+
+int fused_sync_blocks(qeh_ctx *ctx) {
+    if (ctx->fused_sync && ctx->pinned_status) return QEH_OK;
+    if (!ctx->pinned_status) {
+        void *h = nullptr, *d = nullptr;
+        QEH_HIP(hipHostMalloc(&h, 64, hipHostMallocMapped));
+        if (hipHostGetDevicePointer(&d, h, 0) != hipSuccess) {
+            hipHostFree(h);
+            return fail(QEH_E_HIP, "fused join-aggregate: no device address for the pinned status block");
+        }
+        std::memset(h, 0, 64);
+        ctx->pinned_status = (uint32_t *)h;
+        ctx->pinned_status_dev = (uint32_t *)d;
+    }
+    if (!ctx->fused_sync) {
+        FusedSync rest{};
+        rest.mm[0].v = rest.mm[2].v = INT64_MAX;
+        rest.mm[1].v = rest.mm[3].v = INT64_MIN;
+        void *d = nullptr;
+        QEH_HIP(hipMalloc(&d, sizeof rest));
+        if (hipMemcpy(d, &rest, sizeof rest, hipMemcpyHostToDevice) != hipSuccess) {
+            hipFree(d);
+            return fail(QEH_E_HIP, "fused join-aggregate: hand-off words not initialised");
+        }
+        ctx->fused_sync = d;
+    }
     return QEH_OK;
 }
 
@@ -222,7 +259,7 @@
     DeviceGuard dg(ctx->device);
     hipStreamSynchronize(ctx->stream);
     for (auto &r : ctx->timing_pending) {
-        hipEventDestroy(r.start);
+        if (!r.shared_start) hipEventDestroy(r.start);
         hipEventDestroy(r.stop);
     }
     for (auto e : ctx->event_free) hipEventDestroy(e);
@@ -231,6 +268,8 @@
     if (ctx->aux_stream) hipStreamSynchronize(ctx->aux_stream);
     if (ctx->pinned_plan) hipHostFree(ctx->pinned_plan);
     if (ctx->pinned) hipHostFree(ctx->pinned);
+    if (ctx->pinned_status) hipHostFree(ctx->pinned_status);
+    if (ctx->fused_sync) hipFree(ctx->fused_sync);
     ctx->source_cache.reset();
     delete ctx->pool;
     if (ctx->own_stream) hipStreamDestroy(ctx->own_stream);
```

Result: slower. 157.6 billion (-8.3%).
